# lucidrains/dreamer4

Hardware: AMD Instinct MI355X
Metric: imagined latent steps/sec (higher is better)
Workload: dtype f32; 1 GPU; cfg2 Moving-MNIST-latent shape: dim=512 depth=6 heads=8x64 latents=32x32 spatial=4 registers=8; generate(H+1=16 frames, num_steps=4, time cache) + learn_from_experience(ppo) + clip/AdamW both heads; global_batch=256, per_gpu_batch=256, horizon=15, num_steps=4, parallelism=dp1

## Files before the change

dreamer4_amd/_lib.py:

```python
from __future__ import annotations

import ctypes as C
import os

_HERE = os.path.dirname(os.path.abspath(__file__))
LIB_PATH = os.path.join(_HERE, 'libd4hip.so')

D4_MAX_ACTION_TYPES = 8

GEMM_RMS_ROWSCALE, GEMM_SILU, GEMM_SWIGLU, GEMM_TRANS_A, GEMM_TRANS_B, GEMM_ACCUMULATE = 1, 2, 4, 8, 16, 32


class Config(C.Structure):
    _fields_ = [
        ('dim', C.c_int32), ('dim_latent', C.c_int32), ('num_latent_tokens', C.c_int32), ('depth', C.c_int32),
        ('time_block_every', C.c_int32), ('attn_heads', C.c_int32), ('attn_dim_head', C.c_int32),
        ('attn_softclamp_value', C.c_float),
        ('num_spatial_tokens', C.c_int32), ('num_register_tokens', C.c_int32), ('max_steps', C.c_int32),
        ('num_tasks', C.c_int32), ('num_discrete_action_types', C.c_int32),
        ('num_discrete_actions', C.c_int32 * D4_MAX_ACTION_TYPES), ('num_continuous_actions', C.c_int32),
        ('multi_token_pred_len', C.c_int32),
        ('policy_head_mlp_depth', C.c_int32), ('value_head_mlp_depth', C.c_int32),
        ('terminal_mlp_depth', C.c_int32), ('predict_terminals', C.c_int32),
        ('reward_num_bins', C.c_int32), ('value_num_bins', C.c_int32), ('reward_encoder_type', C.c_int32), ('matmul_bf16', C.c_int32), ('head_mlp_recipe', C.c_int32), ('continuous_beta_param', C.c_int32),
# ... 100 lines not shown
    'd4_engine_destroy': (None, [_P]),
    'd4_engine_workspace_bytes': (C.c_size_t, [_P]),
    'd4_engine_set_workspace': (_I, [_P, _P, C.c_size_t]),
    'd4_engine_bind': (_I, [_P, C.c_char_p, _P, _P, _L]),
    'd4_engine_prepare': (_I, [_P, _P]),
    'd4_engine_cache_frames': (_I, [_P]),
    'd4_engine_cache_reset': (_I, [_P, _I]),
    'd4_engine_cache_export': (_I, [_P, _P, _I, _P]),
    'd4_engine_cache_import': (_I, [_P, _P, _I, _I, _P]),
    'd4_wm_forward': (_I, [_P, _P, _P, _I, _P, _P, _P, _I, _I, _I, _I, _P, _P, _P]),
    'd4_decoder_forward': (_I, [_P, _P, _P, _I, _I, _I, _P, _P]),
    'd4_ff_workspace_bytes': (C.c_size_t, [_I, _I, _I]),
    'd4_train_arith_set': (_I, [_I]),
    'd4_train_wide_set': (_I, [_I]),
    'd4_train_attn_products_set': (_I, [_I]),
    'd4_train_arith_get': (_I, []),
    'd4_train_scratch_bind': (_I, [_P, C.c_size_t]),
    'd4_ff_bf16_scratch_bytes': (C.c_size_t, [_I] * 3),
    'd4_attn_bf16_scratch_bytes': (C.c_size_t, [_I] * 4),
    'd4_cross_attn_bf16_scratch_bytes': (C.c_size_t, [_I] * 7),
    'd4_ff_forward': (_I, [_P] * 6 + [_I, _I, _I, _P, _P, C.c_size_t, _P]),
    'd4_ff_backward': (_I, [_P] * 6 + [_I, _I, _I] + [_P] * 6 + [_P, C.c_size_t, _P]),
    'd4_ff_backward_saved': (_I, [_P] * 6 + [_I, _I, _I] + [_P] * 6 + [_P, C.c_size_t, _P]),
    'd4_attn_workspace_bytes': (C.c_size_t, [_I] * 5),
    'd4_space_attn_forward': (_I, [_P] * 11 + [_I] * 5 + [_F, _I, _I, _P, _P, C.c_size_t, _P]),
    'd4_space_attn_backward': (_I, [_P] * 12 + [_I] * 5 + [_F, _I, _I] + [_P] * 11 + [_P, C.c_size_t, _P]),
    'd4_space_attn_backward_saved': (_I, [_P] * 12 + [_I] * 5 + [_F, _I, _I] + [_P] * 11 + [_P, C.c_size_t, _P]),
    'd4_time_attn_workspace_bytes': (C.c_size_t, [_I] * 6),
    'd4_time_attn_forward': (_I, [_P] * 12 + [_I] * 6 + [_F, _I, _P, _P, C.c_size_t, _P]),
    'd4_time_attn_backward': (_I, [_P] * 13 + [_I] * 6 + [_F, _I] + [_P] * 11 + [_P, C.c_size_t, _P]),
    'd4_time_attn_backward_saved': (_I, [_P] * 13 + [_I] * 6 + [_F, _I] + [_P] * 11 + [_P, C.c_size_t, _P]),
    'd4_cross_attn_workspace_bytes': (C.c_size_t, [_I] * 7),
    'd4_cross_attn_forward': (_I, [_P] * 10 + [_I] * 8 + [_F, _P, _P, C.c_size_t, _P]),
    'd4_cross_attn_backward': (_I, [_P] * 11 + [_I] * 8 + [_F] + [_P] * 10 + [_P, C.c_size_t, _P]),
    'd4_cross_attn_backward_saved': (_I, [_P] * 11 + [_I] * 8 + [_F] + [_P] * 10 + [_P, C.c_size_t, _P]),
    'd4_encoder_forward': (_I, [_P, _P, _I, _I, _P, _P]),
    'd4_euler_step': (_I, [_P, _P, _L, _F, _F, _P]),
    'd4_rollout': (_I, [_P, C.POINTER(RolloutIO), _P]),
    'd4_learn': (_I, [_P, C.POINTER(LearnIO), _P]),
    'd4_adamw_clip': (_I, [_P, _P, _P, _P, _L, _I, _F, _F, _F, _F, _F, _F, _F, _P, _P]),
    'd4_profile_bf16_enable': (_I, [_I]),
    'd4_profile_bf16_read': (_I, [C.POINTER(C.c_double), C.POINTER(C.c_double), C.POINTER(C.c_int64)]),
    'd4_profile_enable': (_I, [_I]),
    'd4_profile_read': (_I, [C.POINTER(C.c_double), C.POINTER(C.c_double), C.POINTER(C.c_int64), _I]),
    'd4_profile_classes': (_I, []),
    'd4_gemm_force_config': (_I, [_I]),
    'd4_debug_switch': (_I, [C.c_char_p, _I]),
    'd4_frame_fused_set': (_I, [_I]),
    'd4_profile_class_name': (C.c_char_p, [_I]),
    'd4_profile_glue_enable': (_I, [_I]),
    'd4_profile_glue_read': (_I, [C.POINTER(C.c_double), C.POINTER(C.c_double), C.POINTER(C.c_int64), _I]),
    'd4_profile_glue_classes': (_I, []),
    'd4_profile_glue_read_flops': (_I, [C.POINTER(C.c_double), _I]),
    'd4_measure_peaks': (_I, [_P, C.c_size_t, C.POINTER(C.c_double), C.POINTER(C.c_double), C.POINTER(C.c_double), _P]),
    'd4_profile_glue_class_name': (C.c_char_p, [_I]),
    'd4_debug_buffer': (_I, [_P, C.c_char_p, C.POINTER(_P)]),
    'd4_gemm': (_I, [_P, _I, _P, _I, _P, _I, _P, _P, _I, _I, _I, _I, _I, _F, _P]),
    'd4_gemm_tn': (_I, [_P, _I, _P, _I, _P, _I, _I, _I, _I, _P, C.c_int64, _I, _I, _P]),
    'd4_gemm_tn_bf16': (_I, [_P, _I, _P, _I, _P, _I, _I, _I, _I, _P, C.c_int64, _I, _P]),
    'd4_gemm_pair': (_I, [_P, _I, _P, _P, _I, _I, _I, _P, _I, _P, _P, _I, _I, _I, _I, _I, _F, _P]),
    'd4_gemm_batched': (_I, [_P, _I, _P, _I, _P, _I, _P, _P, _I, _I, _I, _I, _I, _F, _I, _L, _L, _L, _P]),
    'd4_gemm_bf16': (_I, [_P, _I, _P, _I, _P, _I, _P, _P, _I, _I, _I, _I, _I, _F, _P]),
    'd4_gemm_bf16a': (_I, [_P, _I, _P, _I, _P, _I, _P, _P, _P, _I, _I, _I, _I, _I, _F, _I, _P]),
    'd4_cvt_bf16': (_I, [_P, _P, _L, _P]),
    'd4_gemm_bf16a_compact': (_I, [_P, _I, _P, _I, _P, _I, _P, _P, _P, _I, _I, _I, _I, _I, _F, _P, _P, _I, _I, _I, _I, _I, _I, _P]),
    'd4_gemm_bf16a_batched': (_I, [_P, _I, _P, _I, _P, _I, _P, _P, _P, _I, _I, _I, _I, _I, _F, _I, _L, _L, _L, _I, _P]),
    'd4_cvt_rows_bf16': (_I, [_P, _L, _P, _L, _I, _I, _P]),
    'd4_split_bf16x3': (_I, [_P, _P, _L, _L, _P]),
    'd4_gemm_split': (_I, [_P, _I, _P, _L, _I, _P, _I, _P, _P, _I, _I, _I, _I, _I, _F, _I, _P]),
    'd4_split_f16x2': (_I, [_P, _P, _I, _I, _I, _L, _P, _P]),
    'd4_row_scale_exp': (_I, [_P, _L, _I, _I, _P, _P]),
    'd4_gemm_split2': (_I, [_P, _I, _P, _L, _I, _P, _P, _I, _P, _P, _I, _I, _I, _I, _I, _F, _I, _P, _P]),
    'd4_rmsnorm': (_I, [_P, _I, _P, _P, _I, _I, _I, _F, _P]),
    'd4_small_attn': (_I, [_P, _L, _L] * 4 + [_P] + [_P, _L, _L] * 3 + [_P] + [_I] * 4 + [_F] + [_I] * 6 + [_P]),
    'd4_small_attn_wide': (_I, [_P, _L, _L] * 4 + [_P] + [_P, _L, _L] * 3 + [_P] + [_I] * 4 + [_F] + [_I] * 6 + [_P]),
    'd4_small_attn_wide_bf16': (_I, [_P, _L, _L] * 4 + [_P] + [_P, _L, _L] * 3 + [_P] + [_I] * 4 + [_F] + [_I] * 6 + [_P]),
    'd4_pool_mix': (_I, [_P, _I, _P, _I, _P, _P, _I, _P, _I, _P, _P, _I, _I, _I, _F, _P, _P, _P, _P, _P]),
    'd4_pool_mix_deep': (_I, [_P, _I, _P, _I, _P, _P, _I, _P, _I, _P, _P, _I, _I, _I, _F, _P, _P, _P, _P, _P]),
    'd4_time_attn_decode': (_I, [_P, _I, _P, _I, _P, _P, _P, _P, _I, _P] + [_I] * 8 + [_P, _F, _I, _I, _P]),
    'd4_gemm_family_configs': (_I, [_I]),
    'd4_gemm_run': (_I, [C.POINTER(GemmDesc), _I, _I, _P]),
    'd4_gemm_run_rowmap': (_I, [C.POINTER(GemmDesc), _I, _I, _I, _I, _I, _I, _P]),
    'd4_gemm_run_pair': (_I, [C.POINTER(GemmDesc), C.POINTER(GemmDesc), _I, _I, _P]),
    'd4_tile16_weights': (_I, [_P, _I, _P, _I, _I, _P]),
    'd4_frame_attn_out': (_I, [_P, _L, _L] * 4 + [_P] + [_P, _L, _L] * 2 + [_P] + [_I] * 3 + [_F] + [_I] * 3 + [_P, _I, _P, _I, _P, _I, _P, _I, _I, _I, _I, _P]),
    'd4_attn_out_cols': (_I, [_P, _L, _L] * 4 + [_P] + [_P, _L, _L] * 2 + [_P] + [_I] * 3 + [_F] + [_I] * 3 + [_P, _I, _I, _P, _I, _P, _I, _P, _I, _I, _I, _I, _P]),
    'd4_frame_pool': (_I, [_P, _I, _P, _I, _P, _P, _I, _P, _I, _P, _I, _I, _I, _F, _P, _P, _I, _I, _P, _I, _P, _I, _P, _I, _I, _I, _I, _P]),
    'd4_frame_pool_tail': (_I, [_P, _P, _P, _I, _I, _I, _I, _P, _I, _P, _I, _P, _I, _I, _I, _I, _P]),
    'd4_lqap_in': (_I, [_P, _I, _P, _I, _P, _P, _P, _P] + [_I] * 5 + [_F, _P]),
    'd4_lqap_out': (_I, [_P, _I, _P, _P, _P, _P, _I, _P, _I] + [_I] * 5 + [_P]),
    'd4_debug_last_form': (C.c_char_p, [C.c_char_p]),
    'd4_debug_forms': (_I, [C.c_char_p, _I, C.POINTER(C.c_char_p)]),
    'd4_train_attn_core_plane_floats': (C.c_size_t, [_I] * 3),
    'd4_train_xattn_core_plane_floats': (C.c_size_t, [_I] * 4),
    'd4_train_attn_core': (_I, [_P, _I] + [_P] * 7 + [_I] * 4 + [_F, _I, _I, _I, _L, _L, _I, _P, _I, _P, C.c_size_t, _P]),
    'd4_train_xattn_core': (_I, [_P, _I, _P, _I] + [_P] * 6 + [_I] * 6 + [_F, _I, _P, C.c_size_t, _P]),
    'd4_train_attn_core_bf16_plane_floats': (C.c_size_t, [_I] * 4),
    'd4_train_xattn_core_bf16_plane_floats': (C.c_size_t, [_I] * 5),
    'd4_train_attn_core_bf16': (_I, [_P, _I] + [_P] * 7 + [_I] * 4 + [_F, _I, _I, _I, _L, _L, _I, _P, _I, _P, C.c_size_t, _P]),
    'd4_train_xattn_core_bf16': (_I, [_P, _I, _P, _I] + [_P] * 6 + [_I] * 6 + [_F, _I, _P, C.c_size_t, _P]),
    'd4_rmsnorm_backward': (_I, [_P, _P, _P, _P, _P, _P, _I, _I, _F, _P]),
    'd4_layernorm_rows': (_I, [_P, _I, _P, _P, _P, _I, _I, _I, _F, _I, _P]),
    'd4_assemble_tokens': (_I, [C.POINTER(AssembleDesc), _P]),
    'd4_gather_space_double_norm': (_I, [_P, _P, _P, _P, _I, _I, _I, _I, _I, _F, _P]),
    'd4_colsum': (_I, [_P, _I, _I, _I, _P, _P, C.c_size_t, _P]),
    'd4_colsum_batch': (_I, [_I, C.POINTER(_P), C.POINTER(C.c_int32), C.POINTER(C.c_int32), C.POINTER(C.c_int32), C.POINTER(_P), _P]),
    'd4_rmsnorm_bwd': (_I, [_P, _P, _P, _P, _P, _I, _I, _F, _P]),
    'd4_euler_step_rows': (_I, [_P, _I, _P, _I, _I, _I, _F, _F, _P]),
    'd4_splitk_reduce': (_I, [_P, _I, _I, _I, _P, _I, _P, _I, _P]),
    'd4_mean_tokens': (_I, [_P, _P, _I, _I, _I, _P]),
    'd4_hl_gauss_scalar_strided': (_I, [_P, _I, _P, _P, _I, _I, _I, _P]),
    'd4_unary_rows': (_I, [_I, _P, _P, _L, _P]),
    'd4_fold_rows': (_I, [_P, _P, _P, _I, _I, _I, _P]),
    'd4_swiglu_pack_rows': (_I, [_P, _P, _P, _P, _P, _I, _I, _I, _P]),
    'd4_build_latent_input': (_I, [_P, _P, _P, _P, _I, _I, _I, _I, _F, _P]),
    'd4_copy_rows': (_I, [_P, _I, _P, _I, _I, _I, _P]),
    'd4_pad_cols': (_I, [_P, _P, _I, _I, _I, _P]),
    'd4_video_patches': (_I, [_P, _P, _I, _I, _I, _I, _I, _I, _I, _P]),
    'd4_cache_transfer': (_I, [_P, _P] + [_I] * 9 + [_P]),
    'd4_cunembed': (_I, [_I, _P, _P, _I, _I, _I, _P]),
    'd4_coord_grid': (_I, [_P, _I, _I, _I, _P]),
    'd4_pack_tokens': (_I, [_I, _P, _P, _P, _P, _P, _I, _I, _I, _I, _I, _P]),
    'd4_prep_eval_inputs': (_I, [_P, _P, _P] + [_I] * 7 + [_P, _P, _I, _P]),
    'd4_layernorm_silu_bwd': (_I, [_P, _I, _P, _P, _P, _P, _P, _P, _I, _I, _F, _P]),
    'd4_silu_bwd': (_I, [_P, _P, _P, _L, _P]),
    'd4_swiglu': (_I, [_I, _P, _P, _P, _I, _I, _I, _P]),
    'd4_multi_copy': (_I, [_I, C.POINTER(_P), C.POINTER(_P), C.POINTER(C.c_int64), _P]),
    'd4_zero_pad_cols': (_I, [_P, _I, _I, _I, _I, _P]),
    'd4_cvt_pad_bf16': (_I, [_P, _L, _P, _L, _I, _I, _I, _P]),
    'd4_cvt_transpose_bf16': (_I, [_P, _I, _P, _I, _I, _I, _I, _P]),
    'd4_hl_gauss_scalar': (_I, [_P, _I, _P, _P, _I, _I, _P]),
    'd4_ppo_policy_loss': (_I, [_P, _I, _P, _P, _P, _P, _P, _I, _I, _I, _I, _F, _F, _P, _P, _P, _P]),
    'd4_gae': (_I, [_P, _P, _P, _P, _P, _F, _F, _I, _I, _P, _P]),
    'd4_gae_adv': (_I, [_P, _P, _P, _P, _P, _F, _F, _I, _I, _P, _P, _P, _P]),
    'd4_policy_loss': (_I, [C.POINTER(PolicyLossDesc), _P]),
    'd4_return_stats': (_I, [_P, _P, _P, _L, _P, C.c_double, _F, _F, _P, _P, _P]),
    'd4_value_loss': (_I, [C.POINTER(ValueLossDesc), _P]),
    'd4_categorical_sample_logp': (_I, [_P, _I, _P, _I, _P, _I, _I, _F, _P, _P, _P]),
    'd4_hl_gauss_ce': (_I, [_P, _I, _P, _P, _P, _I, _I, _F, _F, _F, _F, _I, _P, _P, _P, _P]),
    'd4_flow_noised_patches': (_I, [_P] * 4 + [_I] * 6 + [_P]),
    'd4_tok_rows_part_floats': (C.c_size_t, [_I, _I]),
    'd4_layernorm_rows_bwd': (_I, [_P, _I, _P, _P, _P, _P, _P, C.c_size_t, _I, _I, _F, _P]),
    'd4_mask_rows_fwd': (_I, [_P] * 4 + [_I, _I, _P]),
    'd4_mask_rows_bwd': (_I, [_P] * 5 + [C.c_size_t, _I, _I, _P]),
    'd4_recon_loss_fwd_bwd': (_I, [_P] * 4 + [_I] * 7 + [_P, _P, _P, C.c_size_t, _P]),
}

_lib = None


class D4Error(RuntimeError):
    pass


def load():
    global _lib
    if _lib is not None:
        return _lib
    if not os.path.isfile(LIB_PATH):
        raise D4Error(f'{LIB_PATH} is missing: run `python -m dreamer4_amd.build` (hipcc, gfx950). '
                      'There is no CPU fallback for the imagination path.')
    default_table = os.path.join(_HERE, 'gemm_tune_default.txt')
    if os.path.isfile(default_table):
        os.environ.setdefault('D4_GEMM_TUNE_DEFAULT', default_table)
    lib = C.CDLL(LIB_PATH)
    for name, (res, args) in SYMBOLS.items():
# ... 19 lines not shown
```

dreamer4_amd/csrc/engine.hip:

```cpp
#include "common.h"
#include "engine.h"
#include "prof.h"
#include <math.h>
#include <stdarg.h>
#include <stdio.h>
#include <stdlib.h>
#include <string.h>
#include <memory>

using namespace d4;

namespace d4 {

static constexpr float RMS_EPS = 1.1920928955078125e-07f;

static int round_up(int v, int m) { return (v + m - 1) / m * m; }

int engine_layout(d4_engine* e, bool assign) {
    const d4_config& c = e->c;
    size_t off = 0;
    auto alloc_bytes = [&](size_t bytes) -> char* {
        off = (off + 255) / 256 * 256;
        char* p = assign ? e->ws + off : nullptr;
        off += bytes;
// ... 666 lines not shown
            if ((rc = mir(e->layer_attn[l].to_out, (size_t)D, hd))) return rc;
        }
        for (int l = 0; l <= c.depth; ++l) {
            if ((rc = mir(e->ffp[l].w1, (size_t)2 * e->inner_pad, D))) return rc;
            if ((rc = mir(e->ffp[l].w2, (size_t)D, e->inner_pad))) return rc;
        }
        for (int p = 0; p < c.depth; ++p) {
            if ((rc = mir(e->pq_w[p], (size_t)(hp + e->php), D))) return rc;
            if ((rc = mir(e->pkv_w[p], (size_t)2 * hp, D))) return rc;
            if ((rc = mir(e->pools[p].to_out, (size_t)D, hp))) return rc;
        }
        for (int l = 0; l < (int)e->pkq_w.size(); ++l)
            if ((rc = mir(e->pkq_w[l], (size_t)(c.depth - l) * hp, D))) return rc;
        if ((rc = mir(e->cq_w, (size_t)(hd + h), D))) return rc;
        if ((rc = mir(e->ckv_w, (size_t)2 * hd, D))) return rc;
        if ((rc = mir(e->cross.to_out, (size_t)D, hd))) return rc;
        if (ns == n) {
            if ((rc = mir(e->lin_w, (size_t)D, dl))) return rc;
            if ((rc = mir(e->lout_w, (size_t)dl, D))) return rc;
        } else {
            if ((rc = mir(e->lin_kv_w, (size_t)2 * hd, dl))) return rc;
            if ((rc = mir(e->lq_in.to_out, (size_t)D, hd))) return rc;
            if ((rc = mir(e->lout_kv_w, (size_t)2 * hd, D))) return rc;
            if ((rc = mir(e->lout_w, (size_t)dl, hd))) return rc;
        }
    }

    e->l0_ready = e->ck_ready = false;
    if (e->c0_proj || e->ck) {
        const int nr = c.num_register_tokens, lo = 1 + ns, pin = 4096;
        t_bf16 = e->bf16 ? e : nullptr;
        auto planes = [e](GemmArgs g) {
            if (e->bf16)
                for (const auto& m : e->mirrors)
                    if (g.W >= m.src && g.W < m.src + m.n) { g.Wb = m.dst + (g.W - m.src); break; }
            if (g.Wb && e->split) { g.wplane = (int64_t)e->bf16_cap; if (!gemm_x3_applicable(g)) { g.Wb = nullptr; g.wplane = 0; } }
            return g;
        };
        rc = 0;
        if (e->c0_proj) {
            GemmArgs g{e->registers, D, e->proj_w[0], D, e->c0_proj, e->Nproj0, e->proj_b[0], nullptr, 0, nr, e->Nproj0, D, GEMM_RMS_ROWSCALE, RMS_EPS};
            g.rule_M = pin;
            if (gemm_rule_takes_x3sk(planes(g))) {
                rc = engine_gemm(g, s);
                for (int ly = 0; ly < 2 && !rc; ++ly) {
                    const int Sl = e->S - 1 + ly;
                    rc = copy_rows(e->c0_proj, 0, e->proj0r[ly] + (size_t)lo * e->Nproj0, Sl * e->Nproj0, e->Fr, nr * e->Nproj0, s);
                }
                e->l0_ready = !rc;
            }
        }
        if (!rc && e->ck && e->pkv_stride > 0) {
            bool ok = true;
            for (int p = 0; p < c.depth - 1; ++p) {
                GemmArgs g{e->registers, D, e->pkv_w[p], D, e->ck + (size_t)p * nr * hp, hp, nullptr, nullptr, 0, nr, hp, D, GEMM_RMS_ROWSCALE, RMS_EPS};
                g.rule_M = pin;
                ok = ok && gemm_rule_takes_v2(planes(g));
            }
            for (int p = 0; ok && p < c.depth - 1 && !rc; ++p) {
                GemmArgs g{e->registers, D, e->pkv_w[p], D, e->ck + (size_t)p * nr * hp, hp, nullptr, nullptr, 0, nr, hp, D, GEMM_RMS_ROWSCALE, RMS_EPS};
                g.rule_M = pin;
                rc = engine_gemm(g, s);
                for (int ly = 0; ly < 2 && !rc; ++ly) {
                    const int Sl = e->S - 1 + ly;
                    rc = copy_rows(e->ck + (size_t)p * nr * hp, 0, e->kvr[ly] + (size_t)p * e->kvr_stride[ly] + (size_t)lo * hp, Sl * hp, e->Fr, nr * hp, s);
                }
            }
            e->ck_ready = ok && !rc;
        }
        t_bf16 = nullptr;
        if (rc) return rc;
    }

    int32_t offs[D4_MAX_ACTION_TYPES] = {0}, sizes[D4_MAX_ACTION_TYPES] = {0};
    int o = 0;
    for (int a = 0; a < e->na; ++a) { offs[a] = o; sizes[a] = c.num_discrete_actions[a]; o += sizes[a]; }
    D4_HIP(hipMemcpyAsync(e->action_offsets, offs, sizeof(offs), hipMemcpyHostToDevice, s));
    D4_HIP(hipMemcpyAsync(e->action_sizes, sizes, sizeof(sizes), hipMemcpyHostToDevice, s));
    D4_HIP(hipStreamSynchronize(s));
    e->prepared = true;
    return 0;
}

static int ff_block(d4_engine* e, const FfPrep& fp, const float* out_b, const float* x, int ldx, float* y, int ldy,
                    int rows, hipStream_t s, float* y_compact = nullptr, int S = 0, int has_agent = 1) {
    int rc;
    GemmArgs g1{x, ldx, fp.w1, e->D, e->ffh, e->inner_pad, fp.b1, nullptr, 0, rows, 2 * e->inner_pad, e->D,
                GEMM_RMS_ROWSCALE | GEMM_SWIGLU, RMS_EPS, 2.0 * rows * (2.0 * e->inner) * e->D};
    if ((rc = engine_gemm(g1, s))) return rc;
    GemmArgs g2{e->ffh, e->inner_pad, fp.w2, e->inner_pad, y, ldy, out_b, x, ldx, rows, e->D, e->inner_pad, 0, RMS_EPS,
                2.0 * rows * (double)e->D * e->inner};
    if (y_compact) { g2.C2 = y_compact; g2.ldc2 = e->D; g2.c2_S = S; g2.c2_lo = t_keep_lo; g2.c2_hi = t_keep_hi; g2.c2_last = has_agent; }
    return engine_gemm(g2, s);
}

int g_pool_wide_keys = 1;
int g_rollout_clean_agent_row = 1;
int g_rollout_batched_heads = 1;
int g_lqap_in_fused = 1;
int g_lqap_out_fused = 1;
int g_last_layer_compact_q = 1;
int g_layer0_const_rows = 1;
int g_pool_const_keys = 1;
unsigned g_launch_count = 0;
static int pool_block(d4_engine* e, int p, const float* x, float* y, int L, int M, hipStream_t s, const float* hiddens = nullptr,
                      float* y_compact = nullptr, int S = 0, int has_agent = 1, int rule_M = 0, float* keys0 = nullptr) {
    if (!hiddens) hiddens = e->slabs;
    const d4_config& c = e->c;
    const int D = e->D, hp = e->hp;
    const AttnW& a = e->pools[p];
    int rc;
    const bool mix_path = c.pool_heads == 4 && D <= 1024;
    GemmArgs gq{x, D, e->pq_w[p], D, e->pool_q, e->ldpq, nullptr, nullptr, 0, M, mix_path ? hp : hp + e->php, D, GEMM_RMS_ROWSCALE, RMS_EPS};
    gq.rule_M = rule_M;
    if (mix_path) {
        const bool wide = g_pool_wide_keys && t_bf16 && e->kall_b && hiddens == e->slabs && p < c.depth - 1 && L == 2 * p + 3 && x == e->slabs + (size_t)(L - 1) * M * D;
        PoolMixArgs pm{};
        pm.q = e->pool_q; pm.ldq = e->ldpq; pm.k = e->pool_kv; pm.ldk = hp;
        if (wide) {
            const int j0 = p == 0 ? 0 : 2 * p + 1, ld = e->kall_ld;
            GemmArgs gw{hiddens + (size_t)j0 * M * D, D, e->pkq_w[p], D, nullptr, ld, nullptr, nullptr, 0, (L - j0) * M, (c.depth - p) * hp, D, GEMM_RMS_ROWSCALE, RMS_EPS};
            gw.algo_flops = 2.0 * M * hp * (double)D * ((double)(L - j0) * (c.depth - 1 - p) + 1.0);
            gw.Cb = e->kall_b + (size_t)j0 * M * ld + (size_t)p * hp;
            if ((rc = engine_gemm(gw, s))) return rc;
            pm.k = nullptr; pm.k_b = e->kall_b + (size_t)p * hp; pm.ldk = ld;
            pm.q = nullptr; pm.q_b = e->kall_b + (size_t)(L - 1) * M * ld + (size_t)(c.depth - 1) * hp; pm.ldq = ld;
        } else {
        GemmArgs gk{hiddens, D, e->pkv_w[p], D, e->pool_kv, hp, nullptr, nullptr, 0, L * M, hp, D, GEMM_RMS_ROWSCALE, RMS_EPS};
        gk.rule_M = L * rule_M;
        if (keys0) {
            gk.A = hiddens + (size_t)M * D; gk.C = keys0 + (size_t)M * hp; gk.M = (L - 1) * M; gk.rule_M = L * M;
            pm.k = keys0;
        }
        if ((rc = gemm_two(gq, gk, s))) return rc;
        if (t_bf16) pm.k_b = t_bf16->shadow_of(e->pool_kv);
        }
        pm.x = x; pm.ldx = D; pm.gate_w = e->pq_w[p] + (size_t)hp * D; pm.hid = hiddens; pm.D = D; pm.k_gamma = a.k_gamma;
        pm.u = e->pool_u; pm.M = M; pm.L = L; pm.heads = c.pool_heads; pm.eps = RMS_EPS; pm.rule_M = rule_M;
        if (t_bf16 && D > 512) pm.hid_b = t_bf16->shadow_of(hiddens);
        if (t_bf16) if (uint16_t* ub = t_bf16->shadow_of(e->pool_u)) { pm.u_b = ub; if (t_bf16->shadow_only(e->pool_u)) pm.u = nullptr; }
        const bool deep = L > 64 || g_pool_mix_deep;
        if (S > 0 && M % S == 0 && !e->pv_t.empty() && (!t_bf16 || t_bf16->fp32_planes()) && frame_pool_tail_applicable(M / S, S, D, c.pool_heads)) {
            const bool tail_only = deep || frame_fused_mode() == 2;
            if (!tail_only) return frame_pool(pm, e->pv_t[p], e->po_t[p], M / S, S, x, D, y, D, y_compact, D, t_keep_lo, t_keep_hi, has_agent, s);
            if ((rc = deep ? pool_mix_deep(pm, s) : pool_mix(pm, s))) return rc;
            return frame_pool_tail(e->pool_u, e->pv_t[p], e->po_t[p], M / S, S, D, c.pool_heads, x, D, y, D, y_compact, D, t_keep_lo, t_keep_hi, has_agent, s);
        }
        if ((rc = deep ? pool_mix_deep(pm, s) : pool_mix(pm, s))) return rc;
        GemmArgs gv{e->pool_u, c.pool_heads * D, e->pkv_w[p] + (size_t)hp * D, D, e->pool_att, hp, nullptr, nullptr, 0, M, 64, D, 0, RMS_EPS};
        gv.batch = c.pool_heads; gv.strideA = D; gv.strideW = (int64_t)64 * D; gv.strideC = 64; gv.rule_M = rule_M;
        if ((rc = engine_gemm(gv, s))) return rc;
    } else {
    const GemmArgs gkv{hiddens, D, e->pkv_w[p], D, e->pool_kv, 2 * hp, nullptr, nullptr, 0, L * M, 2 * hp, D, GEMM_RMS_ROWSCALE, RMS_EPS};
    if ((rc = gemm_two(gq, gkv, s))) return rc;
    SmallAttnArgs sa{};
    sa.q = e->pool_q; sa.q_group_stride = e->ldpq; sa.q_item_stride = 0;
    sa.k = e->pool_kv; sa.k_group_stride = 2 * hp; sa.k_item_stride = (int64_t)M * 2 * hp;
    sa.v = e->pool_kv + hp; sa.v_group_stride = 2 * hp; sa.v_item_stride = (int64_t)M * 2 * hp;
    sa.gate = e->pool_q + hp; sa.g_group_stride = e->ldpq; sa.g_item_stride = 0;
    sa.k_gamma = a.k_gamma;
    sa.out = e->pool_att; sa.o_group_stride = hp; sa.o_item_stride = 0;
    sa.groups = M; sa.heads = c.pool_heads; sa.nq = 1; sa.nk = L;
    sa.wide = (c.wide_frames & 2) ? 2 : (c.wide_frames & 1);
    sa.out_b = t_bf16 ? t_bf16->shadow_of(e->pool_att) : nullptr;
    if ((rc = small_attn(sa, s))) return rc;
    }
    if (y_compact) return gemm_c2(e->pool_att, hp, a.to_out, hp, y, D, M, D, hp, 0, nullptr, x, D, y_compact, S, t_keep_hi - t_keep_lo, has_agent, s);
    GemmArgs go{e->pool_att, hp, a.to_out, hp, y, D, nullptr, x, D, M, D, hp, 0, RMS_EPS};
    go.rule_M = rule_M;
    return engine_gemm(go, s);
}

void engine_drop_graphs(d4_engine* e) {
    for (auto& g : e->graphs) (void)hipGraphExecDestroy(g.exec);
    e->graphs.clear();
}

static int engine_forward_impl(d4_engine* e, const float* latents, int B, int Tq, int t0, int step_log2,
                               const int64_t* tasks, bool need_agent, hipStream_t s, const int* t0_dev, bool need_pred, bool agent_only);

bool engine_clean_agent_only(const d4_engine* e) {
    return !e->encoder && !e->decoder && (!e->bf16 || e->split) && e->c.pool_heads == 4 && e->D <= 1024;
}

int engine_forward(d4_engine* e, const float* latents, int B, int Tq, int t0, int step_log2,
                   const int64_t* tasks, bool need_agent, hipStream_t s, const int* t0_dev, bool need_pred) {
    t_bf16 = e->bf16 ? e : nullptr;
    need_pred = need_pred || !need_agent || e->encoder || e->decoder;
    const bool agent_only = !need_pred && engine_clean_agent_only(e);
    t_keep_lo = e->keep_lo;
    t_keep_hi = agent_only ? e->keep_lo : e->keep_hi;
    const int rc = engine_forward_impl(e, latents, B, Tq, t0, step_log2, tasks, need_agent, s, t0_dev, need_pred, agent_only);
    t_bf16 = nullptr;
    return rc;
}

static int engine_forward_impl(d4_engine* e, const float* latents, int B, int Tq, int t0, int step_log2,
                               const int64_t* tasks, bool need_agent, hipStream_t s, const int* t0_dev, bool need_pred, bool agent_only) {
    const d4_config& c = e->c;
    D4_REQUIRE(e->prepared, "engine not prepared");
    D4_REQUIRE(B >= 1 && B <= e->maxB, "batch %d exceeds max_batch %d", B, e->maxB);
    D4_REQUIRE(Tq >= 1 && Tq <= e->maxTq, "parallel frames %d exceed max_parallel_frames %d", Tq, e->maxTq);
    D4_REQUIRE(t0 + Tq <= e->Tcap || e->Lt == 0, "KV cache capacity %d exceeded (%d + %d frames)", e->Tcap, t0, Tq);
    const int has_agent = (need_agent && !e->encoder) ? 1 : 0;
    const int D = e->D, hd = e->hd, h = c.attn_heads, S = (need_agent || e->encoder) ? e->S : e->S - 1;
    const int n = c.num_latent_tokens, dl = c.dim_latent, ns = c.num_spatial_tokens;
    const int Fr = B * Tq, M = Fr * S;
    const bool denoise_only = !need_agent && !e->encoder && !e->decoder;
    const bool fp32_engine = !e->bf16 || e->split;
    auto tiled_family = [e](int M_, int N_, int K_, int flags, const float* W, int rule_M = 0) {
        GemmArgs g{};
        g.M = M_; g.N = N_; g.K = K_; g.lda = K_; g.ldw = K_; g.ldc = N_; g.flags = flags; g.rms_eps = RMS_EPS; g.rule_M = rule_M; g.W = W;
        if (e->bf16) {
            for (const auto& m : e->mirrors)
                if (W >= m.src && W < m.src + m.n) { g.Wb = m.dst + (W - m.src); break; }
            if (g.Wb && e->split) { g.wplane = (int64_t)e->bf16_cap; if (!gemm_x3_applicable(g)) { g.Wb = nullptr; g.wplane = 0; } }
// ... 93 lines not shown
        if ((rc = engine_gemm(gb, s))) return rc;
    }
    }
    if (t_bf16) if (uint16_t* sb = t_bf16->shadow_of(slab0)) { if ((rc = cvt_rows_bf16(slab0, D, sb, D, M, D, s))) return rc; }

    const float* x_in = slab0;
    const float* vres = P0 + 3 * hd + 2 * h;
    for (int l = 0; l < c.depth; ++l) {
        const AttnW& a = e->layer_attn[l];
        float* P = l == 0 ? P0 : e->proj;
        const int ldp = l == 0 ? e->Nproj0 : e->Nproj;
        const bool compact_q = g_last_layer_compact_q && fp32_engine && e->proj_wc && denoise_only && l == c.depth - 1 && !e->is_time[l] && c.depth >= 2 && S <= 16 && S >= 8 &&
                               c.attn_dim_head == 64 && !g_small_attn_wide && tiled_family(M, ldp, D, GEMM_RMS_ROWSCALE, e->proj_w[l]) &&
                               tiled_family(M, 2 * hd + h, D, GEMM_RMS_ROWSCALE, e->proj_wc) && tiled_family(Mc, hd + h, D, GEMM_RMS_ROWSCALE, e->proj_wc, M);
        if (compact_q) {
            GemmArgs ga{x_in, D, e->proj_wc, D, P, ldp, e->proj_bc, nullptr, 0, M, 2 * hd + h, D, GEMM_RMS_ROWSCALE, RMS_EPS};
            GemmArgs gb{e->xpool_c, D, e->proj_wc + (size_t)(2 * hd + h) * D, D, e->qc, e->ldqc, e->proj_bc + 2 * hd + h, nullptr, 0, Mc, hd + h, D, GEMM_RMS_ROWSCALE, RMS_EPS};
            gb.rule_M = M;
            if ((rc = gemm_two(ga, gb, s))) return rc;
        } else if (l == 0 && l0_const) {
            GemmArgs g0{e->slab0r, D, e->proj_w[0], D, P, ldp, e->proj_b[0], nullptr, 0, Fr * Sc, ldp, D, GEMM_RMS_ROWSCALE, RMS_EPS};
            g0.rule_M = M;
            g0.rm_Sc = (uint16_t)Sc; g0.rm_lo = (uint16_t)reg_lo; g0.rm_nr = (uint16_t)nr;
            if ((rc = engine_gemm(g0, s))) return rc;
        } else
        if ((rc = gemm_simple(x_in, D, e->proj_w[l], D, P, ldp, M, ldp, D, GEMM_RMS_ROWSCALE, e->proj_b[l], nullptr, 0, s))) return rc;
        bool fused_out = false;
        if (e->is_time[l]) {
            TimeAttnArgs ta{};
            ta.proj = P; ta.ldp = ldp; ta.vres = vres; ta.ldv = e->Nproj0; ta.k_gamma = a.k_gamma; ta.inv_freq = e->inv_freq;
            ta.cache = e->cache + (size_t)e->time_index[l] * 2 * e->maxB * e->S * h * e->Tcap * c.attn_dim_head;
            ta.dh = c.attn_dim_head;
            ta.out = e->att; ta.ldo = hd; ta.B = B; ta.S = S; ta.H = h; ta.Tq = Tq; ta.t0 = t0; ta.Tcap = e->Tcap;
            ta.softclamp = c.attn_softclamp_value;
            ta.cache_batch = e->maxB; ta.cache_S = e->S;
            ta.t0_dev = t0_dev;
            ta.out_b = t_bf16 ? t_bf16->shadow_of(e->att) : nullptr;
            if ((rc = time_attn_append(ta, s))) return rc;
        } else {
            SmallAttnArgs sa{};
            sa.dh = c.attn_dim_head;
            const int64_t gs = (int64_t)S * ldp;
            sa.q = P; sa.q_group_stride = gs; sa.q_item_stride = ldp;
            sa.k = P + hd; sa.k_group_stride = gs; sa.k_item_stride = ldp;
            sa.v = P + 2 * hd; sa.v_group_stride = gs; sa.v_item_stride = ldp;
            sa.gate = P + 3 * hd; sa.g_group_stride = gs; sa.g_item_stride = ldp;
            sa.mix = P + 3 * hd + h; sa.m_group_stride = gs; sa.m_item_stride = ldp;
            sa.vres = vres; sa.r_group_stride = (int64_t)S * e->Nproj0; sa.r_item_stride = e->Nproj0;
            sa.k_gamma = a.k_gamma;
            sa.out = e->att; sa.o_group_stride = (int64_t)S * hd; sa.o_item_stride = hd;
            sa.groups = Fr; sa.heads = h; sa.nq = S; sa.nk = S;
            sa.wide = (c.wide_frames & 2) ? 2 : (c.wide_frames & 1);
            sa.softclamp = c.attn_softclamp_value; sa.mask_special = e->encoder ? n : has_agent; sa.belief = 1;
            sa.out_b = t_bf16 ? t_bf16->shadow_of(e->att) : nullptr;
            if (denoise_only && l == c.depth - 1 && c.depth >= 2 && S <= 16 && S >= 8) {
                sa.q_lo = 1; sa.q_hi = 1 + ns; sa.q_last = 0;
                sa.out = e->att_c; sa.o_group_stride = (int64_t)nkeep * hd; sa.out_b = nullptr;
                if (compact_q) {
                    sa.k = P; sa.v = P + hd; sa.mix = P + 2 * hd;
                    sa.q = e->qc; sa.q_group_stride = (int64_t)nkeep * e->ldqc; sa.q_item_stride = e->ldqc;
                    sa.gate = e->qc + hd; sa.g_group_stride = (int64_t)nkeep * e->ldqc; sa.g_item_stride = e->ldqc;
                    sa.q_compact = 1;
                }
            }
            const bool tail_compact = denoise_only && l == c.depth - 1 && c.depth >= 2 && S <= 16 && S >= 8;
            if (!tail_compact && !e->wo_t.empty() && (!t_bf16 || t_bf16->fp32_planes()) && frame_attn_out_applicable(sa, D)) {
                if ((rc = frame_attn_out(sa, e->wo_t[l], D, x_in, D, slab(2 * l + 1), D, cslab(2 * l + 1), D, t_keep_lo, t_keep_hi, has_agent, s))) return rc;
                fused_out = true;
            } else if (!tail_compact && hd == 512 && (!t_bf16 || t_bf16->fp32_planes()) && attn_out_cols_applicable(sa, D)) {
                if ((rc = attn_out_cols(sa, a.to_out, hd, D, x_in, D, slab(2 * l + 1), D, cslab(2 * l + 1), D, t_keep_lo, t_keep_hi, has_agent, s))) return rc;
                fused_out = true;
            } else
            if ((rc = small_attn(sa, s))) return rc;
        }
        const bool compact_tail = denoise_only && l == c.depth - 1 && !e->is_time[l] && c.depth >= 2 && S <= 16 && S >= 8;
        if (compact_tail) {
            if ((rc = gemm_simple(e->att_c, hd, a.to_out, hd, cslab(2 * l + 1), D, Mc, D, hd, 0, nullptr, e->xpool_c, D, s))) return rc;
            if ((rc = ff_block(e, e->ffp[l], e->layer_ff[l].out_b, cslab(2 * l + 1), D, cslab(2 * l + 2), D, Mc, s))) return rc;
            break;
        }
        float* h1 = slab(2 * l + 1);
        float* h2 = slab(2 * l + 2);
        if (!fused_out && (rc = gemm_c2(e->att, hd, a.to_out, hd, h1, D, M, D, hd, 0, nullptr, x_in, D, cslab(2 * l + 1), S, t_keep_hi - t_keep_lo, has_agent, s))) return rc;
        if ((rc = ff_block(e, e->ffp[l], e->layer_ff[l].out_b, h1, D, h2, D, M, s, cslab(2 * l + 2), S, has_agent))) return rc;
        if (l != c.depth - 1) {
            float* xc = (denoise_only && l == c.depth - 2 && !e->is_time[c.depth - 1] && S <= 16 && S >= 8) ? e->xpool_c : nullptr;
            if ((rc = pool_block(e, l, h2, e->xpool, 2 * l + 3, M, s, nullptr, xc, S, has_agent, 0, keys0(l)))) return rc;
            x_in = e->xpool;
        }
    }

    float* xfc = e->xfc;
    const float* last = slab(2 * c.depth);
    if ((rc = copy_rows(cslab(2 * c.depth), D, xfc, D, Mc, D, s))) return rc;
    if (e->encoder) {
        const int P = e->P;
        const float* spec = cslab(2 * c.depth);
        if ((rc = gemm_simple(spec, D, e->cq_w, D, e->cq, e->ldcq, Mc, hd + h, D, GEMM_RMS_ROWSCALE, nullptr, nullptr, 0, s))) return rc;
        if ((rc = gemm_simple(last, D, e->ckv_w, D, e->ckv, 2 * hd, M, 2 * hd, D, GEMM_RMS_ROWSCALE, nullptr, nullptr, 0, s))) return rc;
        SmallAttnArgs sa{};
        sa.dh = c.attn_dim_head;
        sa.q = e->cq; sa.q_group_stride = (int64_t)n * e->ldcq; sa.q_item_stride = e->ldcq;
        sa.k = e->ckv; sa.k_group_stride = (int64_t)S * 2 * hd; sa.k_item_stride = 2 * hd;
        sa.v = e->ckv + hd; sa.v_group_stride = (int64_t)S * 2 * hd; sa.v_item_stride = 2 * hd;
        sa.gate = e->cq + hd; sa.g_group_stride = (int64_t)n * e->ldcq; sa.g_item_stride = e->ldcq;
        sa.k_gamma = e->cross.k_gamma;
        sa.out = e->catt; sa.o_group_stride = (int64_t)n * hd; sa.o_item_stride = hd;
        sa.groups = Fr; sa.heads = h; sa.nq = n; sa.nk = P;
        sa.wide = (c.wide_frames & 2) ? 2 : (c.wide_frames & 1);
        if ((rc = small_attn(sa, s))) return rc;
        if ((rc = gemm_simple(e->catt, hd, e->cross.to_out, hd, xfc, D, Mc, D, hd, 0, nullptr, spec, D, s))) return rc;
        if ((rc = ff_block(e, e->ffp[c.depth], e->sff.out_b, xfc, D, xfc, D, Mc, s))) return rc;
        if ((rc = pool_block(e, c.depth - 1, xfc, xfc, e->nslab, Mc, s, e->cslabs))) return rc;
        if ((rc = gemm_simple(xfc, D, e->t2p_wf, D, e->enc_out, c.dim_latent, Mc, c.dim_latent, D, GEMM_RMS_ROWSCALE, nullptr, nullptr, 0, s))) return rc;
        return tanh_rows(e->enc_out, e->enc_out, (int64_t)Mc * c.dim_latent, s);
    }
    if (e->decoder) {
        if ((rc = pool_block(e, c.depth - 1, xfc, xfc, e->nslab, Mc, s, e->cslabs))) return rc;
        return gemm_simple(xfc, D, e->t2p_wf, D, e->dec_out, e->dim_patch, Mc, e->dim_patch, D, GEMM_RMS_ROWSCALE, e->t2p_b, nullptr, 0, s);
    }
    if (need_agent) {
        const float* agent_in = last + (size_t)(S - 1) * D;
        float* agent_rows = xfc + (size_t)ck * D;
        const int lda = S * D, ldc = nkeep * D;
        {
            const GemmArgs gq{agent_in, lda, e->cq_w, D, e->cq, e->ldcq, nullptr, nullptr, 0, Fr, hd + h, D, GEMM_RMS_ROWSCALE, RMS_EPS};
            const GemmArgs gkv{last, D, e->ckv_w, D, e->ckv, 2 * hd, nullptr, nullptr, 0, M, 2 * hd, D, GEMM_RMS_ROWSCALE, RMS_EPS};
            if ((rc = gemm_two(gq, gkv, s))) return rc;
        }
        SmallAttnArgs sa{};
        sa.dh = c.attn_dim_head;
        sa.q = e->cq; sa.q_group_stride = e->ldcq; sa.q_item_stride = 0;
        sa.k = e->ckv; sa.k_group_stride = (int64_t)S * 2 * hd; sa.k_item_stride = 2 * hd;
        sa.v = e->ckv + hd; sa.v_group_stride = (int64_t)S * 2 * hd; sa.v_item_stride = 2 * hd;
        sa.gate = e->cq + hd; sa.g_group_stride = e->ldcq; sa.g_item_stride = 0;
        sa.k_gamma = e->cross.k_gamma;
        sa.out = e->catt; sa.o_group_stride = hd; sa.o_item_stride = 0;
        sa.groups = Fr; sa.heads = h; sa.nq = 1; sa.nk = S - 1;
        sa.wide = (c.wide_frames & 2) ? 2 : (c.wide_frames & 1);
        if ((rc = small_attn(sa, s))) return rc;
        if ((rc = gemm_simple(e->catt, hd, e->cross.to_out, hd, agent_rows, ldc, Fr, D, hd, 0, nullptr, agent_in, lda, s))) return rc;
        if ((rc = ff_block(e, e->ffp[c.depth], e->sff.out_b, agent_rows, ldc, agent_rows, ldc, Fr, s))) return rc;
    }
    if ((rc = pool_block(e, c.depth - 1, xfc, xfc, e->nslab, Mc, s, e->cslabs, nullptr, 0, 1, agent_only ? Fr * (ns + 1) : 0))) return rc;
    if (!need_pred) return 0;

    if (same_len) {
        if ((rc = copy_rows(xfc, nkeep * D, e->gs, ns * D, Fr, ns * D, s))) return rc;
        return gemm_simple(e->gs, D, e->lout_w, D, e->pred, dl, Fr * n, dl, D, GEMM_RMS_ROWSCALE, nullptr, nullptr, 0, s);
    }
    if ((rc = gather_space_double_norm(xfc, e->gs, e->latent_norm, e->lq_out.norm_ctx, Fr, nkeep, 0, D, ns, RMS_EPS, s))) return rc;
    if ((rc = gemm_simple(e->gs, D, e->lout_kv_w, D, e->okv, 2 * hd, Fr * ns, 2 * hd, D, 0, nullptr, nullptr, 0, s))) return rc;
    if (g_lqap_out_fused && fp32_engine && !g_small_attn_wide && lqap_out_applicable(h, c.attn_dim_head, n, ns, dl) && dl % 4 == 0 && frame_fused_frames_ok(Fr) &&
        tiled_family(Fr * n, dl, hd, 0, e->lout_w))
        return lqap_out(e->okv, 2 * hd, e->lout_q, e->lout_gate, e->lq_out.k_gamma, e->lout_w, hd, e->pred, dl, Fr, h, n, ns, dl, s);
    {
        SmallAttnArgs sa{};
        sa.dh = c.attn_dim_head;
        sa.q = e->lout_q; sa.q_group_stride = 0; sa.q_item_stride = hd;
        sa.k = e->okv; sa.k_group_stride = (int64_t)ns * 2 * hd; sa.k_item_stride = 2 * hd;
        sa.v = e->okv + hd; sa.v_group_stride = (int64_t)ns * 2 * hd; sa.v_item_stride = 2 * hd;
        sa.gate = e->lout_gate; sa.g_group_stride = 0; sa.g_item_stride = h;
        sa.k_gamma = e->lq_out.k_gamma;
        sa.out = e->oatt; sa.o_group_stride = (int64_t)n * hd; sa.o_item_stride = hd;
        sa.groups = Fr; sa.heads = h; sa.nq = n; sa.nk = ns;
        sa.wide = (c.wide_frames & 2) ? 2 : (c.wide_frames & 1);
        if ((rc = small_attn(sa, s))) return rc;
    }
    if ((rc = gemm_simple(e->oatt, hd, e->lout_w, hd, e->pred, dl, Fr * n, dl, hd, 0, nullptr, nullptr, 0, s))) return rc;
    return 0;
// ... 268 lines not shown
    int sl, rc;
    if ((rc = step_log2_of(step_size, &sl))) return rc;
    if ((rc = check_step_log2(e, sl))) return rc;
    D4_REQUIRE(batch <= e->maxB && frames <= e->maxTq, "batch/frames exceed engine capacity");
    const int Fr = batch * frames;
    D4_HIP(hipMemcpyAsync(e->sig, signal_levels, sizeof(int32_t) * Fr, hipMemcpyDeviceToDevice, s));
    if (e->na > 0) {
        if (prev_actions) D4_HIP(hipMemcpyAsync(e->pact, prev_actions, sizeof(int64_t) * Fr * e->na, hipMemcpyDeviceToDevice, s));
        else D4_HIP(hipMemsetAsync(e->pact, 0xFF, sizeof(int64_t) * Fr * e->na, s));
    }
    if (e->nc > 0) {
        if (prev_cont) D4_HIP(hipMemcpyAsync(e->pcont, prev_cont, sizeof(float) * Fr * e->nc, hipMemcpyDeviceToDevice, s));
        else if (e->na > 0) D4_HIP(hipMemsetAsync(e->pcont, 0, sizeof(float) * Fr * e->nc, s));
        else D4_HIP(hipMemsetAsync(e->pcont, 0xFF, sizeof(float) * Fr * e->nc, s));
    }
    const int t0 = use_cache ? e->cache_frames : 0;
    if ((rc = d4::engine_forward(e, latents, batch, frames, t0, sl, tasks, true, s))) return rc;
    if (commit_cache) e->cache_frames = t0 + frames;
    const int n_el = e->c.num_latent_tokens * e->c.dim_latent;
    if (pred && (rc = d4::copy_rows(e->pred, n_el, pred, n_el, Fr, n_el, s))) return rc;
    const int nkeep = e->c.num_spatial_tokens + 1;
    if (agent_embed && (rc = d4::copy_rows(e->xfc + (size_t)(nkeep - 1) * e->D, nkeep * e->D, agent_embed, e->D, Fr, e->D, s))) return rc;
    return 0;
}

int d4_decoder_forward(d4_engine* e, const float* latents, const float* noised_video, int time_index, int batch, int frames,
                       float* pred_video, void* stream) {
    D4_REQUIRE(e && latents && noised_video && pred_video, "null argument");
    D4_REQUIRE(e->decoder, "d4_decoder_forward needs an engine created with mode = D4_MODE_DECODER");
    D4_REQUIRE(batch >= 1 && batch <= e->maxB && frames >= 1 && frames <= e->maxTq, "batch / frames exceed the decoder engine's capacity (%d x %d)", e->maxB, e->maxTq);
    D4_REQUIRE(time_index >= 0 && time_index < e->c.decoder_flow_steps, "flow step %d outside [0, %d)", time_index, e->c.decoder_flow_steps);
    hipStream_t s = static_cast<hipStream_t>(stream);
    const d4_config& c = e->c;
    int rc;
    if ((rc = d4::video_to_patches(noised_video, e->dec_in, batch, c.channels, frames, e->nph, e->npw, c.patch_size, s))) return rc;
    if ((rc = d4::engine_forward(e, latents, batch, frames, 0, time_index, nullptr, false, s))) return rc;
    return d4::patches_to_video(e->dec_out, pred_video, batch, c.channels, frames, e->nph, e->npw, c.patch_size, s);
}

int d4_encoder_forward(d4_engine* e, const float* video, int batch, int frames, float* latents, void* stream) {
    D4_REQUIRE(e && video && latents, "null argument");
    D4_REQUIRE(e->encoder, "d4_encoder_forward needs an engine created with mode = D4_MODE_ENCODER");
    D4_REQUIRE(batch >= 1 && batch <= e->maxB && frames >= 1 && frames <= e->maxTq, "batch / frames exceed the encoder engine's capacity (%d x %d)", e->maxB, e->maxTq);
    hipStream_t s = static_cast<hipStream_t>(stream);
    const d4_config& c = e->c;
    int rc;
    if ((rc = d4::video_to_patches(video, e->dec_in, batch, c.channels, frames, e->nph, e->npw, c.patch_size, s))) return rc;
    if ((rc = d4::engine_forward(e, nullptr, batch, frames, 0, 0, nullptr, false, s))) return rc;
    const int nl = c.num_latent_tokens * c.dim_latent;
    return d4::copy_rows(e->enc_out, nl, latents, nl, batch * frames, nl, s);
}

int d4_euler_step(float* x, const float* pred, int64_t n, float one_minus_t, float dt, void* stream) {
    D4_REQUIRE(x && pred && n >= 0 && n < (int64_t)1 << 31, "euler_step: bad arguments");
    return d4::euler_step(x, (int)n, pred, (int)n, 1, (int)n, one_minus_t, dt, static_cast<hipStream_t>(stream));
}

int d4_rollout(d4_engine* e, const d4_rollout_io* io, void* stream) {
    D4_REQUIRE(e && io, "null argument");
    D4_REQUIRE(!e->decoder && !e->encoder, "d4_rollout needs a dynamics engine");
    hipStream_t s = static_cast<hipStream_t>(stream);
    const d4_config& c = e->c;
    const int B = io->batch, T = io->time_steps, P = io->prompt_frames, K = io->num_steps;
    D4_REQUIRE(B >= 1 && B <= e->maxB, "batch %d exceeds max_batch %d", B, e->maxB);
    D4_REQUIRE(K >= 1 && (K & (K - 1)) == 0 && K <= c.max_steps, "number of steps %d must be a power of 2 in (0, %d]  [D4:6357-6358]", K, c.max_steps);
    D4_REQUIRE(P >= 0 && P <= T, "bad prompt_frames");
    D4_REQUIRE(!io->sample_actions || e->na > 0 || e->nc > 0, "the model has no actions to sample  [D4:6626]");
    D4_REQUIRE(!io->sample_actions || e->na == 0 || (io->actions && io->gumbel_u && io->log_probs && io->action_logits), "sample_actions needs the action outputs and gumbel_u");
    D4_REQUIRE(!io->sample_actions || e->nc == 0 || (io->actions_cont && io->beta_noise && io->log_probs_cont && io->cont_params), "sample_actions needs the continuous action outputs and beta_noise");
    D4_REQUIRE(!io->sample_actions || io->values, "sample_actions needs the values output");
    D4_REQUIRE(!io->sample_terminals || (c.predict_terminals && io->bern_u), "sample_terminals needs predict_terminals and bern_u");
    D4_REQUIRE(io->use_time_cache || io->noise_context || T - P <= 1, "noise_context is required without the time cache");
    const int F = T - P;
    const int step_size = c.max_steps / K;
    int sl, rc;
    if ((rc = step_log2_of(step_size, &sl))) return rc;
    if ((rc = check_step_log2(e, sl))) return rc;
    const int n_el = c.num_latent_tokens * c.dim_latent;
    const int D = e->D, S = e->S, A = e->A, na = e->na, nc = e->nc;
    if (!io->use_time_cache) e->cache_frames = 0;
    const bool lean = d4::g_rollout_clean_agent_row != 0;
    const int lean_keep = (lean && d4::engine_clean_agent_only(e)) ? 1 : c.num_spatial_tokens + 1;
    const int variant = (lean ? 1 : 0) | (d4::g_lqap_in_fused ? 2 : 0) | (d4::g_lqap_out_fused ? 4 : 0) | (d4::g_last_layer_compact_q ? 8 : 0) |
                        (d4::g_layer0_const_rows ? 16 : 0) | (d4::g_pool_const_keys ? 32 : 0);
    const float* hist = nullptr;
    if (d4::g_rollout_batched_heads && F >= 1 && F <= e->head_rows) {
        if (io->agent_embed) hist = io->agent_embed;
        else if (F == 1) hist = e->agent_c;
        else if ((size_t)B * F <= e->hist_rows) hist = e->agent_hist;
    }
    const bool heads_after = hist != nullptr;

    for (int f = 0; f < F; ++f) {
        const int cur = P + f;
        int Tq, t0;
        bool commit;
        if (io->use_time_cache && (e->cache_frames > 0 || cur == 0)) { Tq = 1; t0 = e->cache_frames; commit = true; }
        else if (io->use_time_cache) { Tq = cur + 1; t0 = 0; commit = true; }
        else { Tq = cur + 1; t0 = 0; commit = false; }
        D4_REQUIRE(Tq <= e->maxTq, "a parallel pass over %d frames exceeds max_parallel_frames %d", Tq, e->maxTq);
        if ((rc = d4::copy_rows(io->noise_latent + (size_t)f * B * n_el, n_el, e->x_lat, n_el, B, n_el, s))) return rc;

        const bool graphable = Tq == 1 && B * S <= e->graph_max_rows && !d4::gemm_profile_active() && e->graph_max_rows > 0;
        if (graphable) {
            D4_REQUIRE(t0 + 1 <= e->Tcap || e->Lt == 0, "KV cache capacity %d exceeded (%d + 1 frames)", e->Tcap, t0);
            if ((rc = d4::set_frame_state(e->fstate, t0, s))) return rc;
            if ((rc = d4::prep_eval_inputs(e->sig, e->pact, io->actions, B, 1, na, cur, T, 0, c.max_steps - 1, s, nc > 0 ? e->pcont : nullptr, io->actions_cont, nc))) return rc;
            const int64_t* tasks = nullptr;
            if (io->tasks) {
                D4_HIP(hipMemcpyAsync(e->tasks_dev, io->tasks, sizeof(int64_t) * B, hipMemcpyDeviceToDevice, s));
                tasks = e->tasks_dev;
            }
            hipGraphExec_t exec = nullptr;
            const int bucket = e->Lt > 0 ? d4::time_history_bucket(t0) : 0;
            for (auto& g : e->graphs) if (g.B == B && g.K == K && g.sl == sl && g.tasks == (tasks != nullptr) && g.bucket == bucket && g.variant == variant) exec = g.exec;
            if (!exec) {
                if (!e->warm) {
                    e->warm = true;
                } else {
                    if (!e->capture_stream) D4_HIP(hipStreamCreateWithFlags(&e->capture_stream, hipStreamNonBlocking));
                    hipStream_t cs = e->capture_stream;
                    hipGraph_t graph;
                    D4_HIP(hipStreamBeginCapture(cs, hipStreamCaptureModeThreadLocal));
                    int crc = 0;
                    for (int step = 0; step <= K && !crc; ++step) {
                        const int sig_val = step * step_size < c.max_steps - 1 ? step * step_size : c.max_steps - 1;
                        d4::t_sig_uniform = sig_val;
                        crc = d4::engine_forward(e, e->x_lat, B, 1, t0, sl, tasks, step == K, cs, e->fstate, !(step == K && lean));
                        d4::t_sig_uniform = -1;
                        if (crc) break;
                        if (step == K) break;
                        const float tt = (float)sig_val / (float)c.max_steps;
                        crc = d4::euler_step(e->x_lat, n_el, e->pred, n_el, B, n_el, 1.f - tt, (float)step_size / (float)c.max_steps, cs);
                    }
                    hipError_t ce = hipStreamEndCapture(cs, &graph);
                    if (crc) { if (ce == hipSuccess) (void)hipGraphDestroy(graph); return crc; }
                    D4_HIP(ce);
                    D4_HIP(hipGraphInstantiate(&exec, graph, nullptr, nullptr, 0));
                    (void)hipGraphDestroy(graph);
                    e->graphs.push_back({B, K, sl, tasks != nullptr, bucket, variant, exec});
                }
            }
            if (exec) {
                D4_HIP(hipGraphLaunch(exec, s));
            } else {
                for (int step = 0; step <= K; ++step) {
                    const int sig_val = step * step_size < c.max_steps - 1 ? step * step_size : c.max_steps - 1;
                    d4::t_sig_uniform = sig_val;
                    rc = d4::engine_forward(e, e->x_lat, B, 1, t0, sl, tasks, step == K, s, e->fstate, !(step == K && lean));
                    d4::t_sig_uniform = -1;
                    if (rc) return rc;
                    if (step == K) break;
                    const float tt = (float)sig_val / (float)c.max_steps;
                    if ((rc = d4::euler_step(e->x_lat, n_el, e->pred, n_el, B, n_el, 1.f - tt, (float)step_size / (float)c.max_steps, s))) return rc;
                }
            }
            if (commit) e->cache_frames = t0 + 1;
        } else
        for (int step = 0; step <= K; ++step) {
            const bool last = step == K;
            const int sig_val = step * step_size < c.max_steps - 1 ? step * step_size : c.max_steps - 1;
            const float* lat = e->x_lat;
            if (Tq > 1) {
                if ((rc = d4::build_latent_input(e->lat_in, io->latents, io->ctx_hist, e->x_lat, B, Tq, n_el, T, io->context_signal_noise, s))) return rc;
                lat = e->lat_in;
            }
            if ((rc = d4::prep_eval_inputs(e->sig, e->pact, io->actions, B, Tq, na, cur + 1 - Tq, T, sig_val, c.max_steps - 1, s, nc > 0 ? e->pcont : nullptr, io->actions_cont, nc))) return rc;
// ... 4 lines not shown
                                     1.f - tt, (float)step_size / (float)c.max_steps, s))) return rc;
        }

        const int nkeep = lean_keep;
        const float* agent_row = e->xfc + ((size_t)(Tq - 1) * nkeep + (nkeep - 1)) * D;
        if ((rc = d4::copy_rows(agent_row, Tq * nkeep * D, e->agent_c, D, B, D, s))) return rc;
        if (io->agent_embed && (rc = d4::copy_rows(e->agent_c, D, io->agent_embed + (size_t)f * D, F * D, B, D, s))) return rc;
        if (hist == e->agent_hist && (rc = d4::copy_rows(e->agent_c, D, e->agent_hist + (size_t)f * D, F * D, B, D, s))) return rc;
        if (!heads_after) {
        if ((rc = d4::rmsnorm_rows(e->agent_c, D, e->reward_norm, e->hnorm, D, B, D, d4::RMS_EPS, s))) return rc;
        if ((rc = d4::gemm_simple(e->hnorm, D, e->reward_w, D, e->rlogits, c.reward_num_bins, B, c.reward_num_bins, D, 0, nullptr, nullptr, 0, s))) return rc;
        if ((rc = d4::hl_gauss_scalar(e->rlogits, c.reward_num_bins, e->reward_centers, io->rewards + cur, T, B, c.reward_num_bins, s))) return rc;
        }
        const float* term_logit = nullptr;
        if (io->sample_terminals) {
            if ((rc = d4::mean_tokens(e->x_lat, e->term_pool, B, c.num_latent_tokens, c.dim_latent, s))) return rc;
            if ((rc = d4::mlp_forward(e, e->terminal, e->term_pool, c.dim_latent, B, e->term_logit, 1, nullptr, s))) return rc;
            term_logit = e->term_logit;
        }
        if (io->sample_actions) {
            float* pe = e->hbuf[(e->policy.nl - 1) & 1];
            if ((rc = d4::mlp_forward(e, e->policy, e->agent_c, D, B, pe, 4 * D, nullptr, s))) return rc;
            float* logits = na > 0 ? io->action_logits + (size_t)f * A : nullptr;
            if (na > 0 && (rc = d4::gemm_simple(pe, 4 * D, e->action_unembed, c.multi_token_pred_len * 4 * D, logits, F * A, B, A, 4 * D, 0, nullptr, nullptr, 0, s))) return rc;
            float* cparams = nc > 0 ? io->cont_params + (size_t)f * nc * 2 : nullptr;
            if (nc > 0) {
                if ((rc = d4::cunembed_gather(e->cont_unembed, e->cu_w, nc, c.multi_token_pred_len, 4 * D, s))) return rc;
                if ((rc = d4::gemm_simple(pe, 4 * D, e->cu_w, 4 * D, cparams, F * nc * 2, B, 2 * nc, 4 * D, 0, nullptr, nullptr, 0, s))) return rc;
            }
            if (!heads_after) {
            float* vb = e->hbuf[(e->value.nl - 1) & 1];
            if ((rc = d4::mlp_forward(e, e->value, e->agent_c, D, B, vb, c.value_num_bins, nullptr, s))) return rc;
            if ((rc = d4::hl_gauss_scalar(vb, c.value_num_bins, e->value_centers, io->values + f, F, B, c.value_num_bins, s))) return rc;
            }
            d4::SampleArgs sa{};
            sa.logits = logits; sa.ld = F * A;
            sa.gumbel_u = na > 0 ? io->gumbel_u + (size_t)f * B * A : nullptr; sa.ld_u = A;
            sa.term_logit = term_logit; sa.bern_u = io->sample_terminals ? io->bern_u + (size_t)f * B : nullptr;
            sa.actions = na > 0 ? io->actions + (size_t)cur * na : nullptr; sa.act_stride = T * na;
            sa.log_probs = na > 0 ? io->log_probs + (size_t)f * na : nullptr; sa.lp_stride = F * na;
            sa.terminals = io->terminals; sa.lens = io->lens; sa.action_sizes = e->action_sizes;
            sa.B = B; sa.na = na; sa.frame_index = cur; sa.temperature = io->discrete_temperature;
            if (nc > 0) {
                sa.nc = nc; sa.cont_params = cparams; sa.ld_c = F * nc * 2;
                sa.beta_noise = io->beta_noise + (size_t)f * B * nc * 4 * 6;
                sa.actions_cont = io->actions_cont + (size_t)cur * nc; sa.actc_stride = T * nc;
                sa.log_probs_cont = io->log_probs_cont + (size_t)f * nc; sa.lpc_stride = F * nc;
                sa.cont_temperature = io->continuous_temperature; sa.beta_param = e->c.continuous_beta_param;
            }
            if ((rc = d4::sample_actions_terminals(sa, s))) return rc;
        } else if (term_logit) {
            d4::SampleArgs sa{};
            sa.term_logit = term_logit; sa.bern_u = io->bern_u + (size_t)f * B;
            sa.terminals = io->terminals; sa.lens = io->lens; sa.B = B; sa.na = 0; sa.frame_index = cur;
            if ((rc = d4::sample_actions_terminals(sa, s))) return rc;
        }
        if ((rc = d4::copy_rows(e->x_lat, n_el, io->latents + (size_t)cur * n_el, T * n_el, B, n_el, s))) return rc;
        if (io->ctx_hist && io->noise_context &&
            (rc = d4::copy_rows(io->noise_context + (size_t)f * B * n_el, n_el, io->ctx_hist + (size_t)cur * n_el, T * n_el, B, n_el, s))) return rc;
    }
    if (heads_after && (rc = d4::rollout_heads_batched(e, io, hist, B, F, P, T, s))) return rc;
    return 0;
}

int d4_profile_bf16_enable(int stride) { d4::gemm_bf16_profile_enable(stride); return 0; }
int d4_profile_bf16_read(double* ms, double* flops, int64_t* count) { return d4::gemm_bf16_profile_read(ms, flops, count); }
int d4_profile_enable(int on) { return d4::gemm_profile_enable(on); }
int d4_profile_read(double* ms, double* flops, int64_t* count, int nclass) { return d4::gemm_profile_read(ms, flops, count, nclass); }
int d4_profile_classes(void) { return d4::gemm_profile_classes(); }
int d4_profile_glue_enable(int mask) { return d4::glue_profile_enable(mask); }
int d4_profile_glue_read(double* ms, double* bytes, int64_t* count, int nclass) { return d4::glue_profile_read(ms, bytes, count, nclass); }
int d4_profile_glue_classes(void) { return d4::GL_N; }
int d4_profile_glue_read_flops(double* flops, int nclass) { return d4::glue_profile_read_flops(flops, nclass); }
const char* d4_profile_glue_class_name(int c) { return d4::glue_class_name(c); }
int d4_frame_fused_set(int mode) { return d4::frame_fused_set(mode); }

int d4_debug_switch(const char* name, int value) {
    int* sw = nullptr;
    if (name && !strcmp(name, "launch_count")) {
        const int old = (int)(d4::g_launch_count & 0x7fffffffu);
        d4::g_launch_count = (unsigned)value;
        return old;
    }
    if (name && !strcmp(name, "time_attn_fused_append")) sw = &d4::g_time_attn_fused_append;
    else if (name && !strcmp(name, "rollout_clean_agent_row")) sw = &d4::g_rollout_clean_agent_row;
    else if (name && !strcmp(name, "rollout_batched_heads")) sw = &d4::g_rollout_batched_heads;
    else if (name && !strcmp(name, "attn_out_cols")) sw = &d4::g_attn_out_cols;
    else if (name && !strcmp(name, "lqap_in_fused")) sw = &d4::g_lqap_in_fused;
    else if (name && !strcmp(name, "lqap_out_fused")) sw = &d4::g_lqap_out_fused;
    else if (name && !strcmp(name, "last_layer_compact_q")) sw = &d4::g_last_layer_compact_q;
    else if (name && !strcmp(name, "layer0_const_rows")) sw = &d4::g_layer0_const_rows;
    else if (name && !strcmp(name, "pool_const_keys")) sw = &d4::g_pool_const_keys;
    else if (name && !strcmp(name, "pool_wide_keys")) sw = &d4::g_pool_wide_keys;
    else if (name && !strcmp(name, "pool_mix_deep")) sw = &d4::g_pool_mix_deep;
    else if (name && !strcmp(name, "time_attn_tiled")) sw = &d4::g_time_attn_tiled;
    else if (name && !strcmp(name, "space_attn_tiled")) sw = &d4::g_space_attn_tiled;
    else if (name && !strcmp(name, "cross_attn_tiled")) sw = &d4::g_cross_attn_tiled;
    else if (name && !strcmp(name, "small_attn_wide")) sw = &d4::g_small_attn_wide;
    if (!sw) return -1;
    const int old = *sw;
    *sw = value;
    return old;
}
int d4_gemm_force_config(int id) {
    d4::gemm_bf16a_force_config(-1);
    d4::gemm_bf16_force_config(-1);
    const int n_main = d4::gemm_force_config(-1);
    if (id < 0) return n_main;
    if (id >= 500) { d4::gemm_bf16a_force_config(id - 500); return d4::gemm_bf16a_configs(); }
    if (id >= 400) { d4::gemm_force_config(id); return d4::gemm_h2_configs(); }
    if (id >= 300) { d4::gemm_force_config(id); return d4::gemm_x3_configs(); }
    if (id >= 200) return d4::gemm_bf16_force_config(id - 200);
    d4::gemm_force_config(id);
    return id >= 100 ? d4::gemm2_configs() : n_main;
}
const char* d4_profile_class_name(int c) { return d4::gemm_profile_class_name(c); }

int d4_debug_buffer(d4_engine* e, const char* name, float** ptr) {
    D4_REQUIRE(e && name && ptr, "null argument");
    struct { const char* n; float* p; } tbl[] = {
        {"slabs", e->slabs}, {"xpool", e->xpool}, {"xfc", e->xfc}, {"cslabs", e->cslabs}, {"proj0", e->proj0}, {"proj", e->proj}, {"att", e->att},
        {"ffh", e->ffh}, {"pool_q", e->pool_q}, {"pool_kv", e->pool_kv}, {"pool_att", e->pool_att}, {"cq", e->cq},
        {"ckv", e->ckv}, {"catt", e->catt}, {"lkv", e->lkv}, {"latt", e->latt}, {"space", e->space}, {"gs", e->gs},
        {"okv", e->okv}, {"oatt", e->oatt}, {"oproj", e->oproj}, {"pred", e->pred}, {"x_lat", e->x_lat},
        {"cache", e->cache}, {"lin_q", e->lin_q}, {"lin_gate", e->lin_gate}, {"lout_q", e->lout_q},
        {"qc", e->qc}, {"l_logits", e->l_logits}, {"l_dlogits", e->l_dlogits}, {"l_adv", e->l_adv}, {"l_returns", e->l_returns}, {"l_mask", e->l_mask},
    };
    for (auto& t : tbl) if (!strcmp(t.n, name)) {
        D4_REQUIRE(!e->shadow_only(t.p), "debug buffer '%s' exists only as a bf16 image in this engine (matmul_bf16 = 1)", name);
        *ptr = t.p; return 0;
    }
    D4_REQUIRE(false, "unknown debug buffer '%s'", name);
}

int d4_learn(d4_engine* e, const d4_learn_io* io, void* stream) {
    D4_REQUIRE(e && io, "null argument");
    return d4::learn(e, io, static_cast<hipStream_t>(stream));
}

int d4_gemm(const float* A, int lda, const float* W, int ldw, float* C, int ldc, const float* bias,
            const float* R, int ldr, int M, int N, int K, int flags, float rms_eps, void* stream) {
    d4::GemmArgs g{A, lda, W, ldw, C, ldc, bias, R, ldr, M, N, K, flags, rms_eps};
    return d4::gemm(g, static_cast<hipStream_t>(stream));
}

int d4_gemm_pair(const float* A1, int lda1, const float* W1, float* C1, int ldc1, int M1, int N1, const float* A2, int lda2, const float* W2, float* C2,
                 int ldc2, int M2, int N2, int K, int flags, float rms_eps, void* stream) {
    d4::GemmArgs a{A1, lda1, W1, K, C1, ldc1, nullptr, nullptr, 0, M1, N1, K, flags, rms_eps};
    d4::GemmArgs b{A2, lda2, W2, K, C2, ldc2, nullptr, nullptr, 0, M2, N2, K, flags, rms_eps};
    return d4::gemm_pair(a, b, static_cast<hipStream_t>(stream));
}

int d4_gemm_tn(const float* A, int lda, const float* B, int ldb, float* C, int ldc, int M, int N, int K, float* part, int64_t part_floats,
               int tile_n, int slices, void* stream) {
    return d4::gemm_tn(A, lda, B, ldb, C, ldc, M, N, K, part, (size_t)part_floats, static_cast<hipStream_t>(stream), tile_n, slices);
}

int d4_gemm_batched(const float* A, int lda, const float* W, int ldw, float* C, int ldc, const float* bias,
                    const float* R, int ldr, int M, int N, int K, int flags, float rms_eps, int batch,
                    int64_t strideA, int64_t strideW, int64_t strideC, void* stream) {
    d4::GemmArgs g{A, lda, W, ldw, C, ldc, bias, R, ldr, M, N, K, flags, rms_eps};
    g.batch = batch; g.strideA = strideA; g.strideW = strideW; g.strideC = strideC;
    return d4::gemm(g, static_cast<hipStream_t>(stream));
}

int d4_split_bf16x3(const float* src, uint16_t* dst, int64_t n, int64_t plane_stride, void* stream) {
    D4_REQUIRE(src && dst && n >= 0 && plane_stride >= n && (plane_stride % 8) == 0, "d4_split_bf16x3: bad arguments");
    return d4::split_bf16x3(src, dst, n, plane_stride, static_cast<hipStream_t>(stream));
}
int d4_gemm_split(const float* A, int lda, const uint16_t* W3, int64_t plane_stride, int ldw, float* C, int ldc, const float* bias,
                  const float* R, int ldr, int M, int N, int K, int flags, float rms_eps, int config, void* stream) {
    d4::GemmArgs g{A, lda, reinterpret_cast<const float*>(W3), ldw, C, ldc, bias, R, ldr, M, N, K, flags, rms_eps};
    g.Wb = W3; g.wplane = plane_stride;
    D4_REQUIRE(d4::gemm_x3_applicable(g), "d4_gemm_split: call not supported (M=%d N=%d K=%d flags=%d: K %% 32, ldw %% 8, plane_stride %% 8, 16-byte alignment)", M, N, K, flags);
    if (M == 0) return 0;
// ... 262 lines not shown
static d4::GemmArgs gemm_args_of(const d4_gemm_desc& d) {
    d4::GemmArgs g{d.A, d.lda, d.W, d.ldw, d.C, d.ldc, d.bias, d.R, d.ldr, d.M, d.N, d.K, d.flags, d.rms_eps};
    g.C2 = d.C2; g.ldc2 = d.ldc2; g.c2_S = d.c2_S; g.c2_lo = d.c2_lo; g.c2_hi = d.c2_hi; g.c2_last = d.c2_last;
    g.batch = d.batch > 0 ? d.batch : 1; g.strideA = d.strideA; g.strideW = d.strideW; g.strideC = d.strideC;
    g.Ab = d.Ab; g.Wb = d.Wb; g.Cb = d.Cb; g.C2b = d.C2b; g.wplane = d.wplane; g.wscale = d.wscale; g.strideWs = d.strideWs; g.aexp = d.aexp;
    return g;
}
static int gemm_desc_check(const char* who, const d4_gemm_desc* d) {
    D4_REQUIRE(d && d->M >= 1 && d->N >= 1 && d->K >= 1 && (d->C || d->Cb), "%s: null descriptor, no output or bad sizes", who);
    D4_REQUIRE(!(d->C2 || d->C2b) || (d->C2 && d->c2_S >= 1 && d->c2_lo >= 0 && d->c2_hi >= d->c2_lo && d->c2_hi <= d->c2_S && d->ldc2 >= d->N &&
                                      (d->c2_last == 0 || d->c2_last == 1) && !(d->flags & d4::GEMM_SWIGLU)),
               "%s: bad compaction arguments", who);
    return 0;
}
int d4_gemm_family_configs(int family) {
    switch (family) {
        case D4_GEMM_TILE: return d4::gemm_configs();
        case D4_GEMM_V2: return d4::gemm2_configs();
        case D4_GEMM_X3: return d4::gemm_x3_configs();
        case D4_GEMM_H2: return d4::gemm_h2_configs();
        case D4_GEMM_BF16: return d4::gemm_bf16_configs();
        case D4_GEMM_BF16A: return d4::gemm_bf16a_configs();
        case D4_GEMM_V2_KSPLIT: case D4_GEMM_X3SK: case D4_GEMM_SKINNY: return 1;
    }
    return -1;
}
static int gemm_run_args(const d4::GemmArgs& g, int family, int config, void* stream);
int d4_gemm_run(const d4_gemm_desc* d, int family, int config, void* stream) {
    if (int rc = gemm_desc_check("d4_gemm_run", d)) return rc;
    return gemm_run_args(gemm_args_of(*d), family, config, stream);
}
int d4_gemm_run_rowmap(const d4_gemm_desc* d, int family, int config, int rm_Sc, int rm_S, int rm_lo, int rm_nr, void* stream) {
    if (int rc = gemm_desc_check("d4_gemm_run_rowmap", d)) return rc;
    D4_REQUIRE(rm_Sc >= 1 && rm_nr >= 0 && rm_lo >= 0 && rm_lo <= rm_Sc && rm_S == rm_Sc + rm_nr && rm_S <= 65535, "d4_gemm_run_rowmap: bad row map (Sc=%d S=%d lo=%d nr=%d)", rm_Sc, rm_S, rm_lo, rm_nr);
    d4::GemmArgs g = gemm_args_of(*d);
    g.rm_Sc = (uint16_t)rm_Sc; g.rm_lo = (uint16_t)rm_lo; g.rm_nr = (uint16_t)rm_nr;
    return gemm_run_args(g, family, config, stream);
}
static int gemm_run_args(const d4::GemmArgs& g, int family, int config, void* stream) {
    hipStream_t s = static_cast<hipStream_t>(stream);
    const bool al16 = ((uintptr_t)g.A % 16) == 0 && ((uintptr_t)g.W % 16) == 0 && (g.lda % 4) == 0 && (g.ldw % 4) == 0;
#define D4_RUN_REFUSE(cond, why) D4_REQUIRE(cond, "d4_gemm_run: call not supported (family %d, configuration %d, M=%d N=%d K=%d flags=%d: " why ")", family, config, g.M, g.N, g.K, g.flags)
    switch (family) {
        case D4_GEMM_TILE: {
            D4_RUN_REFUSE(d4::gemm_config_valid(config, g), "the dispatcher does not run this configuration of the first family here - few-row shape, mirror weights or an epilogue the tile lacks");
            d4_gemm_force_config(config);
            const int rc = d4::gemm(g, s);
            d4_gemm_force_config(-1);
            return rc;
        }
        case D4_GEMM_V2:
            D4_RUN_REFUSE(al16 && !g.Wb && d4::gemm2_config_valid(config, g), "gemm2_config_valid: K %% 32, lda / ldw %% 4, no transposed operand, SiLU-GLU tiles");
            return d4::gemm2_launch(config, g, s);
        case D4_GEMM_V2_KSPLIT:
            D4_RUN_REFUSE(al16 && d4::gemm2_ksplit_applicable(g), "gemm2_ksplit_applicable: no batch, C2, row scale, bias-free flags other than SiLU; K >= 4 k-tiles");
            return d4::gemm2_ksplit_launch(g, s);
        case D4_GEMM_X3:
            D4_RUN_REFUSE(al16 && !g.wscale && d4::gemm_x3_config_valid(config, g), "gemm_x3_config_valid: three bf16 planes, K %% 32, ldw / plane %% 8, SiLU-GLU tiles");
            return d4::gemm_x3_launch(config, g, s);
        case D4_GEMM_X3SK:
            D4_RUN_REFUSE(al16 && !g.wscale && d4::gemm_x3sk_applicable(g), "gemm_x3sk_applicable: as gemm_x3, no batch");
            return d4::gemm_x3sk_launch(g, s);
        case D4_GEMM_H2:
            D4_RUN_REFUSE(al16 && d4::gemm_h2_config_valid(config, g), "gemm_h2_config_valid: two fp16 planes + row scales, K %% 32, ldw / plane %% 8, SiLU-GLU tiles");
            return d4::gemm_h2_launch(config, g, s);
        case D4_GEMM_SKINNY:
            D4_RUN_REFUSE(al16 && !g.Wb && d4::gemm_skinny_applicable(g) && (!(g.flags & d4::GEMM_SWIGLU) || g.N % 64 == 0),
                          "gemm_skinny_applicable: at most 256 rows and fewer than 64 tiles, K % 4, no transposed operand, C2 without batch");
            return d4::gemm_skinny(g, s);
        case D4_GEMM_BF16: {
            D4_RUN_REFUSE(((uintptr_t)g.A % 16) == 0 && !g.Ab && g.wplane == 0 && d4::gemm_bf16_config_valid(config, g), "gemm_bf16: bf16 weights, K %% 32, lda %% 4, ldw %% 8, SiLU-GLU tiles");
            d4::gemm_bf16_force_config(config);
            const int rc = d4::gemm_bf16(g, s);
            d4::gemm_bf16_force_config(-1);
            return rc;
        }
        case D4_GEMM_BF16A:
            D4_RUN_REFUSE(d4::gemm_bf16a_config_valid(config, g), "gemm_bf16a_config_valid: bf16 images of both operands, K %% 64, lda / ldw %% 8, SiLU-GLU tiles");
            return d4::gemm_bf16a_launch(config, g, s);
    }
    D4_REQUIRE(false, "d4_gemm_run: unknown family %d", family);
#undef D4_RUN_REFUSE
}
int d4_gemm_run_pair(const d4_gemm_desc* da, const d4_gemm_desc* db, int target, int config, void* stream) {
    if (int rc = gemm_desc_check("d4_gemm_run_pair", da)) return rc;
    if (int rc = gemm_desc_check("d4_gemm_run_pair", db)) return rc;
    const d4::GemmArgs a = gemm_args_of(*da), b = gemm_args_of(*db);
    hipStream_t s = static_cast<hipStream_t>(stream);
    auto al16 = [](const d4::GemmArgs& g) { return ((uintptr_t)g.A % 16) == 0 && ((uintptr_t)g.W % 16) == 0 && (g.lda % 4) == 0 && (g.ldw % 4) == 0; };
    switch (target) {
        case D4_PAIR_SKINNY:
            D4_REQUIRE(al16(a) && al16(b) && d4::gemm_skinny_pair_applicable(a, b),
                       "d4_gemm_run_pair: call not supported (gemm_skinny_pair_applicable: two few-row products of equal K, no SiLU-GLU, batch or mirror weights)");
            return d4::gemm_skinny_pair(a, b, s);
        case D4_PAIR_BF16A:
            D4_REQUIRE(d4::gemm_bf16a_pair_applicable(a, b),
                       "d4_gemm_run_pair: call not supported (gemm_bf16a_pair_applicable: equal K, flags == RMS, no bias / R / C2 / batch, a 64 x 64 or 128 x 64 tile by the rule)");
            return d4::gemm_bf16a_pair_launch(a, b, s);
        case D4_PAIR_V2:
            D4_REQUIRE(al16(a) && al16(b) && !a.Wb && !b.Wb && a.K == b.K && d4::gemm2_pair_config_ok(config) && d4::gemm2_pair_applicable(a, b) &&
                       d4::gemm2_config_valid(config, a) && d4::gemm2_config_valid(config, b),
                       "d4_gemm_run_pair: call not supported (gemm2 pair configuration %d: gemm2_pair_config_ok / gemm2_pair_applicable)", config);
            return d4::gemm2_pair_launch(config, a, b, s);
    }
    D4_REQUIRE(false, "d4_gemm_run_pair: unknown target %d", target);
}

int d4_tile16_weights(const float* W, int ldw, float* Wt, int N, int K, void* stream) {
    D4_REQUIRE(W && Wt && N >= 16 && K >= 4 && ldw >= K && ((uintptr_t)W % 16) == 0 && ((uintptr_t)Wt % 16) == 0, "d4_tile16_weights: bad arguments");
    return d4::tile16_weights(W, ldw, Wt, N, K, static_cast<hipStream_t>(stream));
}
static d4::SmallAttnArgs frame_attn_args(const float* q, int64_t q_group_stride, int64_t q_item_stride, const float* k, int64_t k_group_stride, int64_t k_item_stride,
                                         const float* v, int64_t v_group_stride, int64_t v_item_stride, const float* gate, int64_t g_group_stride, int64_t g_item_stride,
                                         const float* k_gamma, const float* vres, int64_t r_group_stride, int64_t r_item_stride, const float* mix, int64_t m_group_stride,
                                         int64_t m_item_stride, uint16_t* out_b, int frames, int heads, int S, float softclamp, int mask_special, int belief, int dh) {
    d4::SmallAttnArgs sa{};
    sa.q = q; sa.q_group_stride = q_group_stride; sa.q_item_stride = q_item_stride;
    sa.k = k; sa.k_group_stride = k_group_stride; sa.k_item_stride = k_item_stride;
    sa.v = v; sa.v_group_stride = v_group_stride; sa.v_item_stride = v_item_stride;
    sa.gate = gate; sa.g_group_stride = g_group_stride; sa.g_item_stride = g_item_stride;
    sa.k_gamma = k_gamma;
    sa.vres = vres; sa.r_group_stride = r_group_stride; sa.r_item_stride = r_item_stride;
    sa.mix = mix; sa.m_group_stride = m_group_stride; sa.m_item_stride = m_item_stride;
    sa.out_b = out_b;
    sa.groups = frames; sa.heads = heads; sa.nq = S; sa.nk = S;
    sa.softclamp = softclamp; sa.mask_special = mask_special; sa.belief = belief; sa.dh = dh;
    return sa;
}
static int frame_out_check(const char* who, const float* resid, const float* out, const float* c2, int S, int c2_lo, int c2_hi, int c2_last) {
    D4_REQUIRE(resid && out && ((uintptr_t)resid % 16) == 0 && ((uintptr_t)out % 16) == 0 && ((uintptr_t)c2 % 16) == 0, "%s: residual / output missing or not 16-byte aligned", who);
    D4_REQUIRE(!c2 || (c2_lo >= 0 && c2_hi >= c2_lo && c2_hi <= S && (c2_last == 0 || c2_last == 1)), "%s: bad compaction arguments", who);
    return 0;
}
int d4_frame_attn_out(const float* q, int64_t q_group_stride, int64_t q_item_stride, const float* k, int64_t k_group_stride, int64_t k_item_stride,
                      const float* v, int64_t v_group_stride, int64_t v_item_stride, const float* gate, int64_t g_group_stride, int64_t g_item_stride,
                      const float* k_gamma, const float* vres, int64_t r_group_stride, int64_t r_item_stride, const float* mix, int64_t m_group_stride,
                      int64_t m_item_stride, uint16_t* out_b, int frames, int heads, int S, float softclamp, int mask_special, int belief, int dh,
                      const float* wo_t, int D, const float* resid, int ldr, float* out, int ldo, float* c2, int ldc2, int c2_lo, int c2_hi, int c2_last,
                      void* stream) {
    const d4::SmallAttnArgs sa = frame_attn_args(q, q_group_stride, q_item_stride, k, k_group_stride, k_item_stride, v, v_group_stride, v_item_stride, gate, g_group_stride,
                                                 g_item_stride, k_gamma, vres, r_group_stride, r_item_stride, mix, m_group_stride, m_item_stride, out_b, frames, heads, S,
                                                 softclamp, mask_special, belief, dh);
    if (int rc = frame_out_check("d4_frame_attn_out", resid, out, c2, S, c2_lo, c2_hi, c2_last)) return rc;
    D4_REQUIRE(wo_t && ((uintptr_t)wo_t % 16) == 0 && ldr >= D && ldo >= D && (!c2 || ldc2 >= D), "d4_frame_attn_out: weight image missing / misaligned or a leading dimension below D");
    return d4::frame_attn_out(sa, wo_t, D, resid, ldr, out, ldo, c2, ldc2, c2_lo, c2_hi, c2_last, static_cast<hipStream_t>(stream));
}
int d4_attn_out_cols(const float* q, int64_t q_group_stride, int64_t q_item_stride, const float* k, int64_t k_group_stride, int64_t k_item_stride,
                     const float* v, int64_t v_group_stride, int64_t v_item_stride, const float* gate, int64_t g_group_stride, int64_t g_item_stride,
                     const float* k_gamma, const float* vres, int64_t r_group_stride, int64_t r_item_stride, const float* mix, int64_t m_group_stride,
                     int64_t m_item_stride, uint16_t* out_b, int frames, int heads, int S, float softclamp, int mask_special, int belief, int dh,
                     const float* W, int ldw, int D, const float* resid, int ldr, float* out, int ldo, float* c2, int ldc2, int c2_lo, int c2_hi, int c2_last,
                     void* stream) {
    const d4::SmallAttnArgs sa = frame_attn_args(q, q_group_stride, q_item_stride, k, k_group_stride, k_item_stride, v, v_group_stride, v_item_stride, gate, g_group_stride,
                                                 g_item_stride, k_gamma, vres, r_group_stride, r_item_stride, mix, m_group_stride, m_item_stride, out_b, frames, heads, S,
                                                 softclamp, mask_special, belief, dh);
    D4_REQUIRE(resid && out && (!c2 || (c2_lo >= 0 && c2_hi >= c2_lo && c2_hi <= S && (c2_last == 0 || c2_last == 1))), "d4_attn_out_cols: residual / output missing or bad compaction arguments");
    D4_REQUIRE(W && ldw >= heads * 64 && ldr >= D && ldo >= D && (!c2 || ldc2 >= D), "d4_attn_out_cols: weights missing or a leading dimension below its width");
    return d4::attn_out_cols(sa, W, ldw, D, resid, ldr, out, ldo, c2, ldc2, c2_lo, c2_hi, c2_last, static_cast<hipStream_t>(stream));
}
int d4_frame_pool(const float* q, int ldq, const float* x, int ldx, const float* gate_w, const float* k, int ldk, const float* hid, int D,
                  const float* k_gamma, int M, int L, int heads, float eps, const float* wv_t, const float* wo_t, int frames, int S, const float* resid,
                  int ldr, float* out, int ldo, float* c2, int ldc2, int c2_lo, int c2_hi, int c2_last, void* stream) {
    d4::PoolMixArgs pm{};
    pm.q = q; pm.ldq = ldq; pm.x = x; pm.ldx = ldx; pm.gate_w = gate_w; pm.k = k; pm.ldk = ldk; pm.hid = hid; pm.D = D; pm.k_gamma = k_gamma;
    pm.M = M; pm.L = L; pm.heads = heads; pm.eps = eps;
    if (int rc = frame_out_check("d4_frame_pool", resid, out, c2, S, c2_lo, c2_hi, c2_last)) return rc;
// ... 36 lines not shown
```

dreamer4_amd/csrc/gemm.hip:

```cpp
#include "common.h"
#include <string.h>
#include <hip/hip_ext.h>
#include "kernels.h"
#include <mutex>
#include <math.h>
#include <stdio.h>
#include <stdlib.h>
#include <map>
#include <tuple>
#include <type_traits>
#include <vector>

namespace d4 {


template <int BM, int BN, int WGM, int WGN, int BK, int KS, bool TA, bool TB, bool KTAIL>
__global__ __launch_bounds__(WGM * WGN * 64 * KS) void gemm_kernel(GemmArgs p) {
    constexpr int LDS_LD = BK + 4;
    constexpr int RF4 = BK / 4;
    constexpr int NT = WGM * WGN * 64 * KS;
    constexpr int TM = BM / WGM / 32;
    constexpr int TN = BN / WGN / 32;
    static_assert(TM >= 1 && TN >= 1, "tile");
    constexpr int A_F4 = BM * BK / 4 / NT;
// ... 580 lines not shown
    return (p.flags & GEMM_SWIGLU) ? 1 : 0;
}

static int autotune_v2(const GemmArgs& p, hipStream_t stream, int* best_out) {
    hipEvent_t e0 = prof_event(), e1 = prof_event();
    const int saved_mask = g_prof_mask;
    g_prof_mask = 0;
    int best = -1, rc = 0;
    float best_ms = 0.f;
    for (int c = 0; c < gemm2_configs() && !rc; ++c) {
        if (!gemm2_config_valid(c, p)) continue;
        if ((rc = gemm2_launch(c, p, stream))) break;
        float ms = 1e30f;
        for (int rep = 0; rep < 2 && !rc; ++rep) {
            (void)hipEventRecord(e0, stream);
            if ((rc = gemm2_launch(c, p, stream))) break;
            if ((rc = gemm2_launch(c, p, stream))) break;
            (void)hipEventRecord(e1, stream);
            if (hipEventSynchronize(e1) != hipSuccess) { rc = 1; break; }
            float t = 0.f;
            (void)hipEventElapsedTime(&t, e0, e1);
            ms = t < ms ? t : ms;
        }
        if (!rc && (best < 0 || ms < best_ms)) { best = c; best_ms = ms; }
    }
    g_prof_mask = saved_mask;
    g_event_pool.push_back(e0);
    g_event_pool.push_back(e1);
    if (rc) return rc;
    D4_REQUIRE(best >= 0, "gemm2: no configuration for M=%d N=%d K=%d flags=%d", p.M, p.N, p.K, p.flags);
    if (getenv("D4_GEMM_LOG"))
        fprintf(stderr, "[d4 gemm2] tuned M %6d N %5d K %5d batch %2d flags %3d -> %s (%.1f us)\n", p.M, p.N, p.K, p.batch, p.flags, gemm2_config_name(best), 500.f * best_ms);
    *best_out = best;
    return 0;
}

static bool use_v2(const GemmArgs& p) { return gemm2_applicable(p); }

static int gemm_v2(const GemmArgs& p, hipStream_t stream) {
    const bool tune_on = tune_mode() != 0;
    const int nb = p.batch > 0 ? p.batch : 1;
    const TuneKey key{p.M, p.N, p.K, p.flags, p.batch};
    tune_cache_load();
    auto it = g_tuned2.find(key);
    if (it != g_tuned2.end() && gemm2_config_valid(it->second, p)) return launch_v2(it->second, p, stream);
    const bool idempotent = !(p.flags & GEMM_ACCUMULATE) && p.R != p.C && p.A != p.C;
    hipStreamCaptureStatus cap = hipStreamCaptureStatusNone;
    (void)hipStreamIsCapturing(stream, &cap);
    if (!tune_on || !idempotent || cap != hipStreamCaptureStatusNone || 2.0 * p.M * p.N * p.K * nb < 1e8)
        return launch_v2(heuristic_v2(p), p, stream);
    if (tune_mode() == 2 && p.M <= 512) return launch_v2(heuristic_v2(p), p, stream);
    D4_TUNE_STRICT_CHECK(p, nb);
    int best = 0;
    if (int rc = autotune_v2(p, stream, &best)) return rc;
    g_tuned2[key] = best;
    tune_cache_append(key, 100 + best);
    return launch_v2(best, p, stream);
}

static int launch_v3(int c, const GemmArgs& p, hipStream_t stream) {
    const int cls = N_TILE_CFG + gemm2_configs() + c;
    const bool timed = ((g_prof_mask >> cls) & 1) && (g_prof_tick++ % g_prof_stride) == 0;
    if (!timed) return gemm_x3_launch(c, p, stream);
    ProfRec rec{};
    rec.a = prof_event(); rec.b = prof_event(); rec.cls = cls;
    rec.M = p.M; rec.N = p.N; rec.K = p.K; rec.flags = p.flags; rec.batch = p.batch;
    gemm_x3_config_tile(c, &rec.bm, &rec.bn);
    rec.flops = p.algo_flops > 0 ? p.algo_flops : 2.0 * p.M * p.N * p.K * (p.batch > 0 ? p.batch : 1);
    if (int rc = gemm_x3_launch(c, p, stream, rec.a, rec.b)) return rc;
    g_prof.push_back(rec);
    return 0;
}

static int launch_v3sk(const GemmArgs& p, hipStream_t stream) {
    const int cls = N_TILE_CFG + gemm2_configs() + gemm_x3_configs();
    const bool timed = ((g_prof_mask >> cls) & 1) && (g_prof_tick++ % g_prof_stride) == 0;
    if (!timed) return gemm_x3sk_launch(p, stream);
    ProfRec rec{};
    rec.a = prof_event(); rec.b = prof_event(); rec.cls = cls;
    rec.M = p.M; rec.N = p.N; rec.K = p.K; rec.flags = p.flags; rec.batch = p.batch;
    rec.bm = 128; rec.bn = 128;
    rec.flops = p.algo_flops > 0 ? p.algo_flops : 2.0 * p.M * p.N * p.K;
    if (int rc = gemm_x3sk_launch(p, stream, rec.a, rec.b)) return rc;
    g_prof.push_back(rec);
    return 0;
}

static int autotune_v3(const GemmArgs& p, hipStream_t stream, int* best_out) {
    hipEvent_t e0 = prof_event(), e1 = prof_event();
    const int saved_mask = g_prof_mask;
    g_prof_mask = 0;
    int best = -1, rc = 0;
    float best_ms = 0.f;
    for (int c = 0; c < gemm_x3_configs() && !rc; ++c) {
        if (!gemm_x3_config_valid(c, p)) continue;
        if ((rc = gemm_x3_launch(c, p, stream))) break;
        float ms = 1e30f;
        for (int rep = 0; rep < 2 && !rc; ++rep) {
            (void)hipEventRecord(e0, stream);
            if ((rc = gemm_x3_launch(c, p, stream))) break;
            if ((rc = gemm_x3_launch(c, p, stream))) break;
            (void)hipEventRecord(e1, stream);
            if (hipEventSynchronize(e1) != hipSuccess) { rc = 1; break; }
            float t = 0.f;
            (void)hipEventElapsedTime(&t, e0, e1);
            ms = t < ms ? t : ms;
        }
        if (!rc && (best < 0 || ms < best_ms)) { best = c; best_ms = ms; }
    }
    g_prof_mask = saved_mask;
    g_event_pool.push_back(e0);
    g_event_pool.push_back(e1);
    if (rc) return rc;
    D4_REQUIRE(best >= 0, "gemm_x3: no configuration for M=%d N=%d K=%d flags=%d", p.M, p.N, p.K, p.flags);
    if (getenv("D4_GEMM_LOG"))
        fprintf(stderr, "[d4 gemm_x3] tuned M %6d N %5d K %5d batch %2d flags %3d -> %s (%.1f us)\n", p.M, p.N, p.K, p.batch, p.flags, gemm_x3_config_name(best), 500.f * best_ms);
    *best_out = best;
    return 0;
}

static int gemm_v3(const GemmArgs& p, hipStream_t stream) {
    const bool tune_on = tune_mode() != 0;
    const int nb = p.batch > 0 ? p.batch : 1;
    if (g_forced_cfg >= 300 && gemm_x3_config_valid(g_forced_cfg - 300, p)) return launch_v3(g_forced_cfg - 300, p, stream);
    const TuneKey key{p.M, p.N, p.K, p.flags, p.batch};
    tune_cache_load();
    auto it = g_tuned3.find(key);
    if (it != g_tuned3.end() && gemm_x3_config_valid(it->second, p)) return launch_v3(it->second, p, stream);
    const bool idempotent = !(p.flags & GEMM_ACCUMULATE) && p.R != p.C && p.A != p.C;
    hipStreamCaptureStatus cap = hipStreamCaptureStatusNone;
    (void)hipStreamIsCapturing(stream, &cap);
    if (!tune_on || !idempotent || cap != hipStreamCaptureStatusNone || 2.0 * p.M * p.N * p.K * nb < 1e8)
        return launch_v3(gemm_x3_heuristic(p), p, stream);
    D4_TUNE_STRICT_CHECK(p, nb);
    int best = 0;
    if (int rc = autotune_v3(p, stream, &best)) return rc;
    g_tuned3[key] = best;
    tune_cache_append(key, 300 + best);
    return launch_v3(best, p, stream);
}

static int launch_v4(int c, const GemmArgs& p, hipStream_t stream) {
    const int cls = N_TILE_CFG + gemm2_configs() + gemm_x3_configs() + 1;
    const bool timed = ((g_prof_mask >> cls) & 1) && (g_prof_tick++ % g_prof_stride) == 0;
    if (!timed) return gemm_h2_launch(c, p, stream);
    ProfRec rec{};
    rec.a = prof_event(); rec.b = prof_event(); rec.cls = cls;
    rec.M = p.M; rec.N = p.N; rec.K = p.K; rec.flags = p.flags; rec.batch = p.batch;
    gemm_h2_config_tile(c, &rec.bm, &rec.bn);
    rec.flops = p.algo_flops > 0 ? p.algo_flops : 2.0 * p.M * p.N * p.K * (p.batch > 0 ? p.batch : 1);
    if (int rc = gemm_h2_launch(c, p, stream, rec.a, rec.b)) return rc;
    g_prof.push_back(rec);
    return 0;
}

static int autotune_v4(const GemmArgs& p, hipStream_t stream, int* best_out) {
    hipEvent_t e0 = prof_event(), e1 = prof_event();
    const int saved_mask = g_prof_mask;
    g_prof_mask = 0;
    int best = -1, rc = 0;
    float best_ms = 0.f;
    for (int c = 0; c < gemm_h2_configs() && !rc; ++c) {
        if (!gemm_h2_config_valid(c, p)) continue;
        if ((rc = gemm_h2_launch(c, p, stream))) break;
        float ms = 1e30f;
        for (int rep = 0; rep < 2 && !rc; ++rep) {
// ... 167 lines not shown
```

dreamer4_amd/csrc/gemm2.hip:

```cpp
#include "common.h"
#include <hip/hip_ext.h>
#include "kernels.h"
#include <stdlib.h>
#include <type_traits>

namespace d4 {

typedef __attribute__((address_space(3))) void* lds_void_ptr;

template <int N>
__device__ __forceinline__ void wait_vmcnt() {
    asm volatile("s_waitcnt vmcnt(%0)" ::"n"(N) : "memory");
}

template <int BK>
__device__ __forceinline__ int chunk_swizzle(int row) {
    if constexpr (BK == 32) return row & 7;
    else return (0x78 >> (((row >> 2) & 3) * 2)) & 3;
}

template <int WGM, int WGN, int TM, int TN, int NS, int BK, bool RMS, bool RMAP = false>
__device__ __forceinline__ void gemm2_body(GemmArgs& p, int bid, const int bz) {
    static_assert(BK == 16 || BK == 32, "k-tile");
    constexpr int CH = BK / 4;
    constexpr int RPP = 64 / CH;
    constexpr int H = BK / 16;
    constexpr int NW = WGM * WGN, NT = NW * 64;
    constexpr int BM = WGM * TM * 16, BN = WGN * TN * 16;
    constexpr int STAGE_ROWS = BM + BN;
    constexpr int STAGE_F = STAGE_ROWS * BK;
    constexpr int NSLOT = STAGE_ROWS / RPP;
    constexpr int LPW = (NSLOT + NW - 1) / NW;
    static_assert(NS >= 3 && NS <= 4 && 2 * LPW <= 63, "ring depth / vmcnt range");
    extern __shared__ __attribute__((aligned(16))) float smem[];

    const int tid = threadIdx.x, lane = tid & 63;
    const int wave = __builtin_amdgcn_readfirstlane(tid >> 6);
    const int wm = wave / WGN, wn = wave % WGN;

    const int nbn = (p.N + BN - 1) / BN, nbm = (p.M + BM - 1) / BM;
    {
        const int nblk = nbm * nbn, nx = 8;
        const int q = nblk / nx, r = nblk % nx, x = bid % nx, o = bid / nx;
        bid = (x < r ? x * (q + 1) : r * (q + 1) + (x - r) * q) + o;
    }
    const int bm0 = (bid / nbn) * BM, bn0 = (bid % nbn) * BN;
    p.A += bz * p.strideA; p.W += bz * p.strideW; p.C += bz * p.strideC;
    if (p.R) p.R += bz * p.strideC;

    const int rowsA = min(BM, p.M - bm0), rowsB = min(BN, p.N - bn0);
    auto uniform_rsrc = [](const float* base, int64_t bytes) {
        const uint64_t b = reinterpret_cast<uint64_t>(base);
        const uint32_t lo = __builtin_amdgcn_readfirstlane((uint32_t)b);
        const uint32_t hi = __builtin_amdgcn_readfirstlane((uint32_t)(b >> 32));
        const int nb = __builtin_amdgcn_readfirstlane((int)(bytes < 0x7FFFFFFF ? bytes : 0x7FFFFFFF));
        return __builtin_amdgcn_make_buffer_rsrc(reinterpret_cast<void*>(((uint64_t)hi << 32) | lo), 0, nb, 0x00020000);
    };
    const __amdgpu_buffer_rsrc_t rsA = uniform_rsrc(p.A + (int64_t)bm0 * p.lda, ((int64_t)(rowsA - 1) * p.lda + p.K) * 4);
    const __amdgpu_buffer_rsrc_t rsB = uniform_rsrc(p.W + (int64_t)bn0 * p.ldw, ((int64_t)(rowsB - 1) * p.ldw + p.K) * 4);

    uint32_t voff[LPW];
    const int prow = lane / CH;
    const int src_chunk = (lane % CH) ^ chunk_swizzle<BK>(prow);
#pragma unroll
    for (int i = 0; i < LPW; ++i) {
        const int slot = min(wave + NW * i, NSLOT - 1);
        const int r = slot * RPP + prow;
        voff[i] = (uint32_t)((slot * RPP < BM ? r * p.lda : (r - BM) * p.ldw) * 4 + src_chunk * 16);
    }
#define D4_ISSUE_STAGE(KT, BUF)                                                                                              \
    _Pragma("unroll") for (int i_ = 0; i_ < LPW; ++i_) {                                                                      \
        const int slot_ = min(wave + NW * i_, NSLOT - 1);                                                                     \
        float* dst_ = smem + (BUF) * STAGE_F + slot_ * 256;                                                                   \
        if (slot_ * RPP < BM) __builtin_amdgcn_raw_ptr_buffer_load_lds(rsA, (lds_void_ptr)dst_, 16, (uint32_t)voff[i_], (KT) * BK * 4, 0, 0); \
        else __builtin_amdgcn_raw_ptr_buffer_load_lds(rsB, (lds_void_ptr)dst_, 16, (uint32_t)voff[i_], (KT) * BK * 4, 0, 0);              \
    }

    f32x4 acc[TM][TN];
#pragma unroll
    for (int i = 0; i < TM; ++i)
#pragma unroll
        for (int j = 0; j < TN; ++j) acc[i][j] = f32x4{0.f, 0.f, 0.f, 0.f};

    const int kq = lane >> 4, frow = lane & 15;
    const int foff0 = frow * BK + ((kq ^ chunk_swizzle<BK>(frow)) << 2);
    const int a_base = wm * TM * 16 * BK, b_base = BM * BK + wn * TN * 16 * BK;

    constexpr int NPAR = 32 / BK;
    constexpr int SQI = RMS ? (BM * CH + NT - 1) / NT : 1;
    float ssq[SQI][NPAR];
#pragma unroll
    for (int i = 0; i < SQI; ++i)
#pragma unroll
        for (int h = 0; h < NPAR; ++h) ssq[i][h] = 0.f;

    const int nk = p.K / BK;
    auto wait_allow = [&](int stages) {
        if (stages >= 2) wait_vmcnt<2 * LPW>();
        else if (stages == 1) wait_vmcnt<LPW>();
        else wait_vmcnt<0>();
    };
    f32x4 af[2][TM], bf[2][TN];
    auto read_frags = [&](const float* st, auto set_tag, int second_half) {
        constexpr int SET = decltype(set_tag)::value;
        const int fo = second_half ? (foff0 ^ 16) : foff0;
#pragma unroll
        for (int i = 0; i < TM; ++i) af[SET][i] = *reinterpret_cast<const f32x4*>(st + a_base + i * 16 * BK + fo);
#pragma unroll
        for (int j = 0; j < TN; ++j) bf[SET][j] = *reinterpret_cast<const f32x4*>(st + b_base + j * 16 * BK + fo);
    };
    auto mfma_set = [&](auto set_tag) {
        constexpr int SET = decltype(set_tag)::value;
#pragma unroll
        for (int e = 0; e < 4; ++e)
#pragma unroll
            for (int i = 0; i < TM; ++i)
#pragma unroll
                for (int j = 0; j < TN; ++j)
                    acc[i][j] = __builtin_amdgcn_mfma_f32_16x16x4f32(bf[SET][j][e], af[SET][i][e], acc[i][j], 0, 0, 0);
    };
    using S0 = std::integral_constant<int, 0>;
    using S1 = std::integral_constant<int, 1>;

#pragma unroll
    for (int s = 0; s < NS - 1; ++s)
        if (s < nk) { D4_ISSUE_STAGE(s, s) }
    wait_allow(min(NS - 2, nk - 1));
    __builtin_amdgcn_s_barrier();
    read_frags(smem, S0{}, 0);

    auto k_tile = [&](int kt, auto par_tag) {
        constexpr int PAR = decltype(par_tag)::value;
        if (kt + 1 < nk) {
            wait_allow(min(kt + NS - 2, nk - 1) - (kt + 1));
            __builtin_amdgcn_s_barrier();
            if (kt + NS - 1 < nk) { D4_ISSUE_STAGE(kt + NS - 1, (kt + NS - 1) % NS) }
        }
        const float* st = smem + (kt % NS) * STAGE_F;
        const float* nxt = smem + ((kt + 1) % NS) * STAGE_F;
        if constexpr (RMS) {
#pragma unroll
            for (int i = 0; i < SQI; ++i) {
                const int idx = tid + i * NT;
                if (BM * CH % NT == 0 || idx < BM * CH) {
                    const f32x4 v = *reinterpret_cast<const f32x4*>(st + idx * 4);
                    ssq[i][PAR % NPAR] = ssq[i][PAR % NPAR] + __builtin_fmaf(v[3], v[3], __builtin_fmaf(v[2], v[2], __builtin_fmaf(v[1], v[1], v[0] * v[0])));
                }
            }
        }
        if constexpr (H == 2) {
            read_frags(st, S1{}, 1);
            mfma_set(S0{});
            if (kt + 1 < nk) read_frags(nxt, S0{}, 0);
            mfma_set(S1{});
        } else {
            using CUR = std::integral_constant<int, PAR>;
            using NXT = std::integral_constant<int, PAR ^ 1>;
            if (kt + 1 < nk) read_frags(nxt, NXT{}, 0);
            mfma_set(CUR{});
        }
    };
    for (int kt = 0; kt < nk; kt += 2) {
        k_tile(kt, S0{});
        if (kt + 1 < nk) k_tile(kt + 1, S1{});
    }

#undef D4_ISSUE_STAGE
    float* rowscale_s = smem + NS * STAGE_F;
    if constexpr (RMS) {
#pragma unroll
        for (int i = 0; i < SQI; ++i) {
            float s = ssq[i][0];
            s += dpp_f<0xB1>(s);
            s += dpp_f<0x4E>(s);
            if constexpr (NPAR == 1) {
                s += dpp_f<0x141>(s);
            } else {
                float s1 = ssq[i][1];
                s1 += dpp_f<0xB1>(s1);
                s1 += dpp_f<0x4E>(s1);
                s = s + s1;
            }
            const int idx = tid + i * NT;
            if ((idx % CH) == 0 && idx < BM * CH) rowscale_s[idx / CH] = rsqrtf(s / (float)p.K + p.rms_eps);
        }
        __syncthreads();
    }

    const bool swiglu = (p.flags & GEMM_SWIGLU) != 0;
    const bool vecC = (p.ldc % 4) == 0 && ((uintptr_t)p.C % 16) == 0;
    const bool vecR = p.R && (p.ldr % 4) == 0 && ((uintptr_t)p.R % 16) == 0;
    const bool vecC2 = p.C2 && (p.ldc2 % 4) == 0 && ((uintptr_t)p.C2 % 16) == 0;
#pragma unroll
    for (int i = 0; i < TM; ++i) {
        const int ml = wm * TM * 16 + i * 16 + frow;
        const int gm = bm0 + ml;
        if (gm >= p.M) continue;
        const float rs = RMS ? rowscale_s[ml] : 1.f;
        int64_t c2row = -1;
        if (p.C2) {
            const int ts = gm % p.c2_S, keep = p.c2_hi - p.c2_lo;
            const int rank = (ts >= p.c2_lo && ts < p.c2_hi) ? ts - p.c2_lo : ((p.c2_last && ts == p.c2_S - 1) ? keep : -1);
            if (rank >= 0) c2row = (int64_t)(gm / p.c2_S) * (keep + p.c2_last) + rank;
        }
        if (swiglu) {
            if constexpr (TN % 4 == 0) {
#pragma unroll
                for (int j = 0; j < TN; ++j) {
                    if ((j & 3) >= 2) continue;
                    const int gn = bn0 + wn * TN * 16 + j * 16 + kq * 4;
                    if (gn >= p.N) continue;
                    f32x4 o;
#pragma unroll
                    for (int e = 0; e < 4; ++e) {
                        float val = acc[i][j][e] * rs, gate = acc[i][j + 2][e] * rs;
                        if (p.bias) { val += p.bias[gn + e]; gate += p.bias[gn + e + 32]; }
                        o[e] = val * siluf(gate);
                    }
                    const int on = (gn / 64) * 32 + (gn % 64);
                    float* cp = p.C + (int64_t)gm * p.ldc + on;
                    if (vecC) *reinterpret_cast<f32x4*>(cp) = o;
                    else { cp[0] = o[0]; cp[1] = o[1]; cp[2] = o[2]; cp[3] = o[3]; }
                }
            }
            continue;
        }
#pragma unroll
        for (int j = 0; j < TN; ++j) {
            const int gn = bn0 + wn * TN * 16 + j * 16 + kq * 4;
            if (gn >= p.N) continue;
            const bool full = gn + 3 < p.N;
            f32x4 v;
#pragma unroll
            for (int e = 0; e < 4; ++e) v[e] = acc[i][j][e] * rs;
            if (p.bias) {
#pragma unroll
                for (int e = 0; e < 4; ++e) if (full || gn + e < p.N) v[e] += p.bias[gn + e];
            }
            if (p.flags & GEMM_SILU) {
#pragma unroll
                for (int e = 0; e < 4; ++e) v[e] = siluf(v[e]);
            }
            if (p.R) {
                const float* rp = p.R + (int64_t)gm * p.ldr + gn;
                if (vecR && full) { const f32x4 r4 = *reinterpret_cast<const f32x4*>(rp); v[0] += r4[0]; v[1] += r4[1]; v[2] += r4[2]; v[3] += r4[3]; }
                else {
#pragma unroll
                    for (int e = 0; e < 4; ++e) if (full || gn + e < p.N) v[e] += rp[e];
                }
            }
            int64_t crow = gm;
            if constexpr (RMAP) {
                const int fr = gm / p.rm_Sc, t = gm - fr * p.rm_Sc;
                crow = (int64_t)fr * (p.rm_Sc + p.rm_nr) + t + (t >= p.rm_lo ? p.rm_nr : 0);
            }
            float* cp = p.C + crow * p.ldc + gn;
            if (p.flags & GEMM_ACCUMULATE) {
#pragma unroll
                for (int e = 0; e < 4; ++e) if (full || gn + e < p.N) v[e] += cp[e];
            }
            if (vecC && full) *reinterpret_cast<f32x4*>(cp) = v;
            else {
#pragma unroll
                for (int e = 0; e < 4; ++e) if (full || gn + e < p.N) cp[e] = v[e];
            }
            if (c2row >= 0) {
                float* c2 = p.C2 + c2row * p.ldc2 + gn;
                if (vecC2 && full) *reinterpret_cast<f32x4*>(c2) = v;
                else {
#pragma unroll
                    for (int e = 0; e < 4; ++e) if (full || gn + e < p.N) c2[e] = v[e];
                }
            }
        }
    }
}

template <int WGM, int WGN, int TM, int TN, int NS, int BK, bool RMS>
__global__ __launch_bounds__(WGM* WGN * 64) void gemm2_kernel(GemmArgs p) {
    gemm2_body<WGM, WGN, TM, TN, NS, BK, RMS>(p, blockIdx.x, blockIdx.y);
}

template <int WGM, int WGN, int TM, int TN, int NS, int BK, bool RMS>
__global__ __launch_bounds__(WGM* WGN * 64) void gemm2_rowmap_kernel(GemmArgs p) {
    gemm2_body<WGM, WGN, TM, TN, NS, BK, RMS, true>(p, blockIdx.x, blockIdx.y);
}

template <int WGM, int WGN, int TM, int TN, int NS, int BK, bool RMS>
__global__ __launch_bounds__(WGM* WGN * 64) void gemm2_pair_kernel(GemmArgs a, GemmArgs b, int nblk_a) {
    const int bid = blockIdx.x;
    if (bid < nblk_a) gemm2_body<WGM, WGN, TM, TN, NS, BK, RMS>(a, bid, 0);
    else gemm2_body<WGM, WGN, TM, TN, NS, BK, RMS>(b, bid - nblk_a, 0);
}

constexpr int KS_GROUPS = 4, KS_NS = 3, KS_BM = 32, KS_BN = 64, KS_BK = 32;
constexpr int KS_STAGE_F = (KS_BM + KS_BN) * KS_BK;
constexpr int KS_RING_F = KS_NS * KS_STAGE_F;
constexpr int KS_LDP = KS_BN + 4;

__global__ __launch_bounds__(1024) void gemm2_ksplit_kernel(GemmArgs p) {
    constexpr int BK = KS_BK, CH = 8, RPP = 8, BM = KS_BM, BN = KS_BN, NS = KS_NS, LPW = 3, NSLOT = (BM + BN) / RPP;
    extern __shared__ __attribute__((aligned(16))) float smem[];
    const int tid = threadIdx.x, lane = tid & 63;
    const int wave = __builtin_amdgcn_readfirstlane(tid >> 6);
    const int grp = wave >> 2, w = wave & 3, wm = w >> 1, wn = w & 1;
    int bid = blockIdx.x;
    const int nbn = (p.N + BN - 1) / BN, nbm = (p.M + BM - 1) / BM;
    {
        const int nblk = nbm * nbn, nx = 8;
        const int q = nblk / nx, r = nblk % nx, x = bid % nx, o = bid / nx;
        bid = (x < r ? x * (q + 1) : r * (q + 1) + (x - r) * q) + o;
    }
    const int bm0 = (bid / nbn) * BM, bn0 = (bid % nbn) * BN;
    const int rowsA = min(BM, p.M - bm0), rowsB = min(BN, p.N - bn0);
    auto uniform_rsrc = [](const float* base, int64_t bytes) {
        const uint64_t b = reinterpret_cast<uint64_t>(base);
        const uint32_t lo = __builtin_amdgcn_readfirstlane((uint32_t)b);
        const uint32_t hi = __builtin_amdgcn_readfirstlane((uint32_t)(b >> 32));
        const int nb = __builtin_amdgcn_readfirstlane((int)(bytes < 0x7FFFFFFF ? bytes : 0x7FFFFFFF));
        return __builtin_amdgcn_make_buffer_rsrc(reinterpret_cast<void*>(((uint64_t)hi << 32) | lo), 0, nb, 0x00020000);
    };
    const __amdgpu_buffer_rsrc_t rsA = uniform_rsrc(p.A + (int64_t)bm0 * p.lda, ((int64_t)(rowsA - 1) * p.lda + p.K) * 4);
    const __amdgpu_buffer_rsrc_t rsB = uniform_rsrc(p.W + (int64_t)bn0 * p.ldw, ((int64_t)(rowsB - 1) * p.ldw + p.K) * 4);
    uint32_t voff[LPW];
    const int prow = lane / CH;
    const int src_chunk = (lane % CH) ^ chunk_swizzle<BK>(prow);
#pragma unroll
    for (int i = 0; i < LPW; ++i) {
        const int slot = w + 4 * i;
        const int r = slot * RPP + prow;
        voff[i] = (uint32_t)((slot * RPP < BM ? r * p.lda : (r - BM) * p.ldw) * 4 + src_chunk * 16);
    }
    float* ring = smem + grp * KS_RING_F;
    const int nkt = p.K / BK, nk = (nkt + KS_GROUPS - 1) / KS_GROUPS;
    const int mine = nkt / KS_GROUPS + (grp < nkt % KS_GROUPS ? 1 : 0);
    const int kt0 = grp * (nkt / KS_GROUPS) + min(grp, nkt % KS_GROUPS);
    const __amdgpu_buffer_rsrc_t rs0 = uniform_rsrc(p.A, 0);
#define D4_KS_ISSUE(KT, BUF)                                                                                                      \
    _Pragma("unroll") for (int i_ = 0; i_ < LPW; ++i_) {                                                                           \
        const int slot_ = w + 4 * i_;                                                                                               \
        float* dst_ = ring + (BUF) * KS_STAGE_F + slot_ * 256;                                                                      \
        const __amdgpu_buffer_rsrc_t rs_ = (KT) < mine ? (slot_ * RPP < BM ? rsA : rsB) : rs0;                                    \
        __builtin_amdgcn_raw_ptr_buffer_load_lds(rs_, (lds_void_ptr)dst_, 16, (uint32_t)voff[i_], (kt0 + (KT)) * BK * 4, 0, 0);           \
    }
    f32x4 acc[2] = {f32x4{0.f, 0.f, 0.f, 0.f}, f32x4{0.f, 0.f, 0.f, 0.f}};
    const int kq = lane >> 4, frow = lane & 15;
    const int foff0 = frow * BK + ((kq ^ chunk_swizzle<BK>(frow)) << 2);
    const int a_base = wm * 16 * BK, b_base = BM * BK + wn * 32 * BK;
    auto wait_allow = [&](int stages) {
        if (stages >= 2) wait_vmcnt<2 * LPW>();
        else if (stages == 1) wait_vmcnt<LPW>();
        else wait_vmcnt<0>();
    };
    f32x4 af[2], bf[2][2];
    auto read_frags = [&](const float* st, int set, int second_half) {
        const int fo = second_half ? (foff0 ^ 16) : foff0;
        af[set] = *reinterpret_cast<const f32x4*>(st + a_base + fo);
        bf[set][0] = *reinterpret_cast<const f32x4*>(st + b_base + fo);
        bf[set][1] = *reinterpret_cast<const f32x4*>(st + b_base + 16 * BK + fo);
// ... 188 lines not shown
```

dreamer4_amd/csrc/gemm_x3sk.hip:

```cpp
#include "common.h"
#include <hip/hip_ext.h>
#include "kernels.h"
#include <type_traits>

namespace d4 {

typedef __bf16 bf16x8 __attribute__((ext_vector_type(8)));


constexpr int SK_BM = 128, SK_BN = 128, SK_WGM = 4, SK_WGN = 2, SK_D = 3;
constexpr int SK_BK = 32, SK_LD = SK_BK + 8, SK_NT = SK_WGM * SK_WGN * 64;
constexpr int SK_G = SK_BK / 8;
constexpr int SK_APL = SK_BM * SK_LD, SK_BPL = SK_BN * SK_LD;
constexpr size_t SK_LDS = (size_t)(2 * 3 * (SK_BM + SK_BN) * SK_LD) * 2 + SK_BM * sizeof(float) + 16;
static_assert(SK_BM * SK_G == SK_NT && SK_BN * SK_G == SK_NT, "one 8-element group of each operand per thread and k-tile");

struct SkArgs {
    GemmArgs p;
    int P, F, R;
    int half;
};

__device__ __forceinline__ void split3(float a, __bf16& h1, __bf16& h2, __bf16& h3) {
    h1 = (__bf16)a;
    const float r = a - (float)h1;
    h2 = (__bf16)r;
    h3 = (__bf16)(r - (float)h2);
}


template <int TNV, bool RMAP>
__device__ __forceinline__ void sk_item(const SkArgs& s, const int bm0, const int bn0, __bf16* As, __bf16* Bs, float* rowscale_s) {
    const GemmArgs& p = s.p;
    const int kt0 = 0, kt1 = p.K / SK_BK;
    constexpr int BNV = 64 * TNV;
    const int tid = threadIdx.x, lane = tid & 63;
    const int wave = __builtin_amdgcn_readfirstlane(tid >> 6);
    const int wm = wave / SK_WGN, wn = wave % SK_WGN;
    const int lrow = lane & 31, lhalf = lane >> 5;
    const __bf16* Wb = reinterpret_cast<const __bf16*>(p.Wb);
    const int rowsA = min(SK_BM, p.M - bm0), rowsB = min(BNV, p.N - bn0);
    auto uniform_rsrc = [](const void* base, int64_t bytes) {
        const uint64_t bb = reinterpret_cast<uint64_t>(base);
        const uint32_t lo = __builtin_amdgcn_readfirstlane((uint32_t)bb);
        const uint32_t hi = __builtin_amdgcn_readfirstlane((uint32_t)(bb >> 32));
        const int nb = __builtin_amdgcn_readfirstlane((int)(bytes < 0x7FFFFFFF ? bytes : 0x7FFFFFFF));
        return __builtin_amdgcn_make_buffer_rsrc(reinterpret_cast<void*>(((uint64_t)hi << 32) | lo), 0, nb, 0x00020000);
    };
    const __amdgpu_buffer_rsrc_t rsA = uniform_rsrc(p.A + (int64_t)bm0 * p.lda, ((int64_t)(rowsA - 1) * p.lda + p.K) * 4);
    const int64_t wbytes = ((int64_t)(rowsB - 1) * p.ldw + p.K) * 2;
    const __amdgpu_buffer_rsrc_t rsB0 = uniform_rsrc(Wb + (int64_t)bn0 * p.ldw, wbytes);
    const __amdgpu_buffer_rsrc_t rsB1 = uniform_rsrc(Wb + p.wplane + (int64_t)bn0 * p.ldw, wbytes);
    const __amdgpu_buffer_rsrc_t rsB2 = uniform_rsrc(Wb + 2 * p.wplane + (int64_t)bn0 * p.ldw, wbytes);

    f32x4 ra[SK_D][2];
    f32x4 rb[SK_D][3];
    float ssq0 = 0.f, ssq1 = 0.f;
    using S0 = std::integral_constant<int, 0>;
    using S1 = std::integral_constant<int, 1>;
    using S2 = std::integral_constant<int, 2>;
    const int srow = tid / SK_G, scol = (tid % SK_G) * 8;
    const int browB = TNV == 2 ? srow : (srow & 63);
    const bool b_store = TNV == 2 || srow < 64;
    const uint32_t offA = (uint32_t)((srow * p.lda + scol) * 4), offB = (uint32_t)((browB * p.ldw + scol) * 2);
    auto load_tile = [&](auto set_tag, int k0) {
        constexpr int S = decltype(set_tag)::value;
        ra[S][0] = __builtin_bit_cast(f32x4, __builtin_amdgcn_raw_buffer_load_b128(rsA, offA + (uint32_t)k0 * 4, 0, 0));
        ra[S][1] = __builtin_bit_cast(f32x4, __builtin_amdgcn_raw_buffer_load_b128(rsA, offA + (uint32_t)k0 * 4 + 16, 0, 0));
        rb[S][0] = __builtin_bit_cast(f32x4, __builtin_amdgcn_raw_buffer_load_b128(rsB0, offB + (uint32_t)k0 * 2, 0, 0));
        rb[S][1] = __builtin_bit_cast(f32x4, __builtin_amdgcn_raw_buffer_load_b128(rsB1, offB + (uint32_t)k0 * 2, 0, 0));
        rb[S][2] = __builtin_bit_cast(f32x4, __builtin_amdgcn_raw_buffer_load_b128(rsB2, offB + (uint32_t)k0 * 2, 0, 0));
    };
    auto store_tile = [&](auto set_tag, int buf) {
        constexpr int S = decltype(set_tag)::value;
        __bf16* as = As + buf * 3 * SK_APL + srow * SK_LD + scol;
        __bf16* bs = Bs + buf * 3 * SK_BPL + browB * SK_LD + scol;
        if (b_store) {
            *reinterpret_cast<f32x4*>(bs) = rb[S][0];
            *reinterpret_cast<f32x4*>(bs + SK_BPL) = rb[S][1];
            *reinterpret_cast<f32x4*>(bs + 2 * SK_BPL) = rb[S][2];
        }
        const f32x4 v0 = ra[S][0], v1 = ra[S][1];
        bf16x8 o1, o2, o3;
#pragma unroll
        for (int e = 0; e < 4; ++e) {
// ... 87 lines not shown
        rsum = ssq0 + ssq1;
        rsum += dpp_f<0xB1>(rsum);
        rsum += dpp_f<0x4E>(rsum);
    }
    const bool row_lane = (tid % SK_G) == 0;

    if (rms) {
        if (row_lane) rowscale_s[srow] = rsqrtf(rsum / (float)p.K + p.rms_eps);
        __syncthreads();
    }

    const bool swiglu = (p.flags & GEMM_SWIGLU) != 0;
    if (TNV == 1 && swiglu) {
        float* xs = reinterpret_cast<float*>(As);
        const int gn = bn0 + lrow;
        if (wn == 1) {
#pragma unroll
            for (int e = 0; e < 16; ++e) {
                const int lr = wm * 32 + (e & 3) + 8 * (e >> 2) + 4 * lhalf;
                float gate = hi[0][e] * (rms ? rowscale_s[lr] : 1.f);
                if (p.bias) gate += p.bias[gn + 32];
                xs[lr * 33 + lrow] = siluf(gate);
            }
        }
        __syncthreads();
        if (wn == 0 && gn < p.N) {
#pragma unroll
            for (int e = 0; e < 16; ++e) {
                const int lr = wm * 32 + (e & 3) + 8 * (e >> 2) + 4 * lhalf;
                const int gm = bm0 + lr;
                if (gm >= p.M) continue;
                float val = hi[0][e] * (rms ? rowscale_s[lr] : 1.f);
                if (p.bias) val += p.bias[gn];
                const int on = (gn / 64) * 32 + (gn % 64);
                p.C[(int64_t)gm * p.ldc + on] = val * xs[lr * 33 + lrow];
            }
        }
        __syncthreads();
        return;
    }
#pragma unroll
    for (int e = 0; e < 16; ++e) {
        const int lr = wm * 32 + (e & 3) + 8 * (e >> 2) + 4 * lhalf;
        const int gm = bm0 + lr;
        if (gm >= p.M) continue;
        const float rs = rms ? rowscale_s[lr] : 1.f;
        if (swiglu) {
            if constexpr (TNV == 2) {
                const int gn = bn0 + wn * 64 + lrow;
                if (gn >= p.N) continue;
                float val = hi[0][e] * rs, gate = hi[1][e] * rs;
                if (p.bias) { val += p.bias[gn]; gate += p.bias[gn + 32]; }
                const int on = (gn / 64) * 32 + (gn % 64);
                p.C[(int64_t)gm * p.ldc + on] = val * siluf(gate);
            }
        } else {
#pragma unroll
            for (int j = 0; j < TNV; ++j) {
                const int gn = bn0 + wn * TNV * 32 + j * 32 + lrow;
                if (gn >= p.N) continue;
                float v = hi[j][e] * rs;
                if (p.bias) v += p.bias[gn];
                if (p.flags & GEMM_SILU) v = siluf(v);
                if (p.R) v += p.R[(int64_t)gm * p.ldr + gn];
                if constexpr (RMAP) {
                    const int fr = gm / p.rm_Sc, t = gm - fr * p.rm_Sc;
                    p.C[((int64_t)fr * (p.rm_Sc + p.rm_nr) + t + (t >= p.rm_lo ? p.rm_nr : 0)) * p.ldc + gn] = v;
                    continue;
                }
                if (p.flags & GEMM_ACCUMULATE) v += p.C[(int64_t)gm * p.ldc + gn];
                p.C[(int64_t)gm * p.ldc + gn] = v;
                if (p.C2) {
                    const int ts = gm % p.c2_S;
                    const int keep = p.c2_hi - p.c2_lo;
                    const int rank = (ts >= p.c2_lo && ts < p.c2_hi) ? ts - p.c2_lo : ((p.c2_last && ts == p.c2_S - 1) ? keep : -1);
                    if (rank >= 0) p.C2[((int64_t)(gm / p.c2_S) * (keep + p.c2_last) + rank) * p.ldc2 + gn] = v;
                }
            }
        }
    }
    __syncthreads();
}

template <bool RMAP>
__device__ __forceinline__ void sk_walk(const SkArgs s) {
    const GemmArgs& p = s.p;
    extern __shared__ __attribute__((aligned(16))) char smem_raw[];
    __bf16* As = reinterpret_cast<__bf16*>(smem_raw);
    __bf16* Bs = As + 2 * 3 * SK_APL;
    float* rowscale_s = reinterpret_cast<float*>(Bs + 2 * 3 * SK_BPL);

    const int b = blockIdx.x;
    const int nbn = (p.N + SK_BN - 1) / SK_BN, nbm = (p.M + SK_BM - 1) / SK_BM;
    const int nk_all = p.K / SK_BK;
    auto tile_of = [&](int tile, int& tm, int& tn) {
        int bid = tile;
        const int nblk = nbm * nbn, nx = 8;
        const int q = nblk / nx, r = nblk % nx, x = bid % nx, o = bid / nx;
        bid = (x < r ? x * (q + 1) : r * (q + 1) + (x - r) * q) + o;
        constexpr int RB = 4;
        const int band = bid / (RB * nbn), j = bid % (RB * nbn);
        const int rows = min(RB, nbm - band * RB);
        tm = band * RB + j % rows; tn = j / rows;
    };
    int tm, tn;
    if (s.half) {
        for (int i = 0; i < s.F; ++i) {
            tile_of(b + i * s.P, tm, tn);
            sk_item<2, RMAP>(s, tm * SK_BM, tn * SK_BN, As, Bs, rowscale_s);
        }
        const int R8 = (s.R + 7) & ~7;
        if (R8 + s.R <= s.P) {
            const int j = b < s.R ? b : b - R8, half = b < s.R ? 0 : 1;
            if (j >= 0 && j < s.R && (b < s.R || b >= R8)) {
                tile_of(s.F * s.P + j, tm, tn);
                const int bn0 = tn * SK_BN + half * 64;
                if (bn0 < p.N) sk_item<1, RMAP>(s, tm * SK_BM, bn0, As, Bs, rowscale_s);
            }
            return;
        }
        for (int h = b; h < 2 * s.R; h += s.P) {
            tile_of(s.F * s.P + h / 2, tm, tn);
            const int bn0 = tn * SK_BN + (h & 1) * 64;
            if (bn0 < p.N) sk_item<1, RMAP>(s, tm * SK_BM, bn0, As, Bs, rowscale_s);
        }
        return;
    }
    for (int i = 0; i < s.F + (b < s.R ? 1 : 0); ++i) {
        tile_of(b + i * s.P, tm, tn);
        sk_item<2, RMAP>(s, tm * SK_BM, tn * SK_BN, As, Bs, rowscale_s);
    }
}

__global__ __launch_bounds__(SK_NT, 2) void gemm_x3sk_kernel(SkArgs s) { sk_walk<false>(s); }
__global__ __launch_bounds__(SK_NT, 2) void gemm_x3sk_rowmap_kernel(SkArgs s) { sk_walk<true>(s); }

static std::atomic<int> g_sk_cus[64];

static int sk_cus() {
    int dev = 0;
    if (hipGetDevice(&dev) != hipSuccess) dev = 0;
    std::atomic<int>& c = g_sk_cus[dev & 63];
    int n = c.load(std::memory_order_relaxed);
    if (n == 0) {
        if (hipDeviceGetAttribute(&n, hipDeviceAttributeMultiprocessorCount, dev) != hipSuccess || n <= 0) n = 256;
        c.store(n, std::memory_order_relaxed);
    }
    return n;
}


const char* gemm_x3sk_name() { return "gemm_x3sk_kernel"; }

bool gemm_x3sk_applicable(const GemmArgs& p) {
    return gemm_x3_applicable(p) && p.batch <= 1 && p.M > 0 && (!(p.flags & GEMM_SWIGLU) || (p.N % 64) == 0);
}

bool gemm_x3sk_half_plan(const GemmArgs& p, int* F, int* R, int* P_out) {
    const int P = sk_cus();
    const int T = cdiv(p.M, SK_BM) * cdiv(p.N, SK_BN);
    const int f = T / P, r = T - f * P;
    *F = f; *R = r;
    if (P_out) *P_out = P;
    return r > 0 && 2 * r <= P;
}

bool gemm_x3sk_rule(const GemmArgs& p) {
    if (!gemm_x3sk_applicable(p) || p.M < 1024 || p.N < 512) return false;
    int F, R, P;
    return gemm_x3sk_half_plan(p, &F, &R, &P) && F >= 1 && F <= 3;
}

int gemm_x3sk_launch(const GemmArgs& p, hipStream_t stream, hipEvent_t ea, hipEvent_t eb) {
    D4_REQUIRE(gemm_x3sk_applicable(p), "gemm_x3sk: call not supported (M=%d N=%d K=%d flags=%d batch=%d)", p.M, p.N, p.K, p.flags, p.batch);
    SkArgs a;
    a.p = p;
    a.half = gemm_x3sk_half_plan(p, &a.F, &a.R, &a.P) ? 1 : 0;
    const int T = a.F * a.P + a.R;
    if (T < a.P && !a.half) a.P = T;
    D4_REQUIRE(gemm_rowmap_ok(p), "gemm_x3sk: bad output row map (Sc=%d lo=%d nr=%d) or an epilogue it does not cover (flags=%d)", p.rm_Sc, p.rm_lo, p.rm_nr, p.flags);
    const bool rmap = p.rm_Sc > 0;
    auto k = rmap ? gemm_x3sk_rowmap_kernel : gemm_x3sk_kernel;
    static DeviceOnce attr_set[2];
    if (attr_set[rmap].need()) {
        D4_HIP(hipFuncSetAttribute(reinterpret_cast<const void*>(k), hipFuncAttributeMaxDynamicSharedMemorySize, (int)SK_LDS));
        attr_set[rmap].done();
    }
    const dim3 grid(a.P), block(SK_NT);
    if (ea) hipExtLaunchKernelGGL(k, grid, block, (uint32_t)SK_LDS, stream, ea, eb, 0, a);
    else hipLaunchKernelGGL(k, grid, block, SK_LDS, stream, a);
    D4_LAUNCH_CHECK();
    return 0;
}

}
```

dreamer4_amd/csrc/kernels.h:

```cpp
#pragma once
#include <hip/hip_runtime.h>
#include <stdint.h>

namespace d4 {

enum : int {
    GEMM_RMS_ROWSCALE = 1,
    GEMM_SILU = 2,
    GEMM_SWIGLU = 4,
    GEMM_TRANS_A = 8,
    GEMM_TRANS_B = 16,
    GEMM_ACCUMULATE = 32,
};

struct GemmArgs {
    const float* A; int lda;
    const float* W; int ldw;
    float* C; int ldc;
    const float* bias;
    const float* R; int ldr;
    int M, N, K;
    int flags;
    float rms_eps;
    double algo_flops = 0;
    float* C2 = nullptr; int ldc2 = 0, c2_S = 0, c2_lo = 0, c2_hi = 0, c2_last = 1;
    int batch = 1; int64_t strideA = 0, strideW = 0, strideC = 0;
    const uint16_t* Wb = nullptr;
    const uint16_t* Ab = nullptr;
    uint16_t* Cb = nullptr;
    uint16_t* C2b = nullptr;
    int group_m = 0;
    uint16_t rm_Sc = 0, rm_lo = 0;
    int64_t wplane = 0;
    const float* wscale = nullptr;
    int64_t strideWs = 0;
    const int* aexp = nullptr;
    int rule_M = 0;
    uint16_t rm_nr = 0, rm_spare = 0;
};
static_assert(sizeof(GemmArgs) == 232, "GemmArgs is a kernel argument: the row map lives in its alignment gaps");
bool gemm_rowmap_ok(const GemmArgs& p);
int gemm_rowmap_refused(const GemmArgs& p, const char* who);
bool gemm_rule_takes_x3sk(const GemmArgs& p);

int gemm(const GemmArgs& p, hipStream_t stream);
bool gemm_rule_takes_v2(const GemmArgs& p);
bool gemm_bf16_applicable(const GemmArgs& p);
int gemm_bf16(const GemmArgs& p, hipStream_t stream);
int gemm_bf16_configs();
bool gemm_bf16_config_valid(int c, const GemmArgs& p);
int gemm_bf16_force_config(int id);
void gemm_bf16a_force_config(int id);
int cvt_f32_to_bf16(const float* src, uint16_t* dst, int64_t n, hipStream_t s);
int cvt_rows_bf16(const float* src, int64_t lds, uint16_t* dst, int64_t ldd, int rows, int cols, hipStream_t s);
int gemm_bf16a(const GemmArgs& p, hipStream_t stream);
bool gemm_bf16a_applicable(const GemmArgs& p);
bool gemm_bf16a_config_valid(int c, const GemmArgs& p);
int gemm_bf16a_configs();
int gemm_bf16a_rule(const GemmArgs& p);
int gemm_bf16a_launch(int c, const GemmArgs& p, hipStream_t stream, hipEvent_t ea = nullptr, hipEvent_t eb = nullptr);
int gemm_bf16p_launch(const GemmArgs& p, hipStream_t stream, hipEvent_t ea = nullptr, hipEvent_t eb = nullptr);
bool gemm_bf16a_pair_applicable(const GemmArgs& a, const GemmArgs& b);
int gemm_bf16a_pair_launch(const GemmArgs& a, const GemmArgs& b, hipStream_t stream, hipEvent_t ea = nullptr, hipEvent_t eb = nullptr);
int gemm_bf16a_pair(const GemmArgs& a, const GemmArgs& b, hipStream_t stream);
void gemm_bf16_profile_enable(int stride);
int gemm_bf16_profile_read(double* ms, double* flops, int64_t* count);
bool gemm_x3_applicable(const GemmArgs& p);
bool gemm_x3_config_valid(int c, const GemmArgs& p);
int gemm_x3_configs();
const char* gemm_x3_config_name(int c);
void gemm_x3_config_tile(int c, int* bm, int* bn);
int gemm_x3_heuristic(const GemmArgs& p);
int gemm_x3_launch(int c, const GemmArgs& p, hipStream_t stream, hipEvent_t ea = nullptr, hipEvent_t eb = nullptr);
int split_bf16x3(const float* src, uint16_t* dst, int64_t n, int64_t plane, hipStream_t s);
bool gemm_h2_applicable(const GemmArgs& p);
bool gemm_h2_config_valid(int c, const GemmArgs& p);
int gemm_h2_configs();
const char* gemm_h2_config_name(int c);
void gemm_h2_config_tile(int c, int* bm, int* bn);
int gemm_h2_heuristic(const GemmArgs& p);
bool gemm_h2_takes(const GemmArgs& p);
int gemm_h2_launch(int c, const GemmArgs& p, hipStream_t stream, hipEvent_t ea = nullptr, hipEvent_t eb = nullptr);
int split_f16x2_rows(const float* src, uint16_t* dst, int rows, int cols, int ld, int64_t plane, float* inv_scale, hipStream_t s);
int row_scale_exp(const float* A, int64_t lda, int rows, int K, int* out, hipStream_t s);
bool gemm_x3sk_applicable(const GemmArgs& p);
bool gemm_x3sk_rule(const GemmArgs& p);
const char* gemm_x3sk_name();
int gemm_x3sk_launch(const GemmArgs& p, hipStream_t stream, hipEvent_t ea = nullptr, hipEvent_t eb = nullptr);
bool gemm2_applicable(const GemmArgs& p);
bool gemm2_config_valid(int c, const GemmArgs& p);
int gemm2_configs();
const char* gemm2_config_name(int c);
void gemm2_config_tile(int c, int* bm, int* bn);
int gemm2_launch(int c, const GemmArgs& p, hipStream_t stream, hipEvent_t ea = nullptr, hipEvent_t eb = nullptr);
bool gemm2_ksplit_applicable(const GemmArgs& p);
bool gemm2_ksplit_rule(const GemmArgs& p);
int gemm2_ksplit_launch(const GemmArgs& p, hipStream_t stream, hipEvent_t ea = nullptr, hipEvent_t eb = nullptr);
bool gemm2_pair_config_ok(int c);
bool gemm2_pair_applicable(const GemmArgs& a, const GemmArgs& b);
int gemm2_pair_launch(int c, const GemmArgs& a, const GemmArgs& b, hipStream_t stream, hipEvent_t ea = nullptr, hipEvent_t eb = nullptr);
int gemm_pair(const GemmArgs& a, const GemmArgs& b, hipStream_t stream);
bool gemm_skinny_applicable(const GemmArgs& p);
int gemm_skinny(const GemmArgs& p, hipStream_t stream);
bool gemm_skinny_pair_applicable(const GemmArgs& a, const GemmArgs& b);
int gemm_skinny_pair(const GemmArgs& a, const GemmArgs& b, hipStream_t stream);
int gemm_profile_enable(int on);
bool gemm_profile_active();
int gemm_profile_read(double* ms, double* flops, int64_t* count, int nclass);
int gemm_profile_classes();
extern int g_time_attn_fused_append;
extern int g_pool_wide_keys;
extern int g_attn_out_cols;
extern int g_time_attn_tiled;
extern int g_space_attn_tiled;
extern int g_cross_attn_tiled;
extern int g_small_attn_wide;
int gemm_force_config(int id);
int gemm_configs();
bool gemm_config_valid(int c, const GemmArgs& p);
const char* gemm_profile_class_name(int c);

struct SmallAttnArgs {
    const float* q;      int64_t q_group_stride, q_item_stride;
    const float* k;      int64_t k_group_stride, k_item_stride;
    const float* v;      int64_t v_group_stride, v_item_stride;
    const float* gate;   int64_t g_group_stride, g_item_stride;
    const float* k_gamma;
    const float* vres;   int64_t r_group_stride, r_item_stride;
    const float* mix;    int64_t m_group_stride, m_item_stride;
    float* out;          int64_t o_group_stride, o_item_stride;
    int groups, heads, nq, nk;
    float softclamp;
    int mask_special;
    int belief;
    int q_lo = 0, q_hi = 0, q_last = 1;
    int q_compact = 0;
    int dh = 64;
    uint16_t* out_b = nullptr;
    int wide = 0;
};
int small_attn(const SmallAttnArgs& p, hipStream_t stream);
constexpr int WIDE_ATTN_MAX = 1024;
int wide_attn(const SmallAttnArgs& p, hipStream_t stream, const char** form);
int wide_attn_bf16_launch(const SmallAttnArgs& p, hipStream_t stream, const char** form);

struct PoolMixArgs {
    const float* q; int ldq;
    const float* x; int ldx;
    const float* gate_w;
    const float* k; int ldk;
    const float* hid; int D;
    const float* k_gamma;
    float* u;
    int M, L, heads;
    float eps;
    uint16_t* u_b = nullptr;
    const uint16_t* k_b = nullptr;
    const uint16_t* q_b = nullptr;
    const uint16_t* hid_b = nullptr;
    int rule_M = 0;
};
int pool_mix(const PoolMixArgs& p, hipStream_t stream);
constexpr int POOL_DEEP_MAX = 1024;
constexpr int POOL_DEEP_CHUNK = 64;
int pool_mix_deep(const PoolMixArgs& p, hipStream_t stream);
extern int g_pool_mix_deep;
void note_pool_deep_form(const char* name);

bool lqap_in_applicable(int heads, int dh, int n, int ns, int dl);
int lqap_in(const float* latents, int ldl, const float* w_kv, int ldw, const float* q, const float* gate, const float* k_gamma, float* out, int frames,
            int heads, int n, int ns, int dl, float eps, hipStream_t s);
// ... 156 lines not shown
```

include/d4hip.h:

```cpp
#ifndef D4HIP_H
#define D4HIP_H

#include <stddef.h>
#include <stdint.h>

#ifdef __cplusplus
extern "C" {
#endif

#define D4_MAX_ACTION_TYPES 8
#define D4_MODE_DYNAMICS 0
#define D4_MODE_DECODER 1
#define D4_MODE_ENCODER 2
#define D4_MLP_PRE_RMS 0
#define D4_MLP_POST_LAYER 1
#define D4_BETA_SOFTPLUS_P1 0
#define D4_BETA_EXP_P1 1

typedef struct d4_config {
    int32_t dim, dim_latent, num_latent_tokens, depth, time_block_every;
    int32_t attn_heads, attn_dim_head;
    float attn_softclamp_value;
    int32_t num_spatial_tokens, num_register_tokens, max_steps, num_tasks;
    int32_t num_discrete_action_types;
// ... 234 lines not shown
int d4_cross_attn_backward_saved(const float* q_tokens, const float* ctx, const float* dy, const float* norm_w, const float* norm_ctx_w, const float* wq,
                           const float* wk, const float* wv, const float* wo, const float* w_gates, const float* k_gamma, int groups, int nq, int nk,
                           int ctx_item_major, int dim, int dim_ctx, int heads, int dim_head, float softclamp,
                           float* d_q_tokens, float* d_ctx, float* d_norm_w, float* d_norm_ctx_w, float* d_wq, float* d_wk, float* d_wv, float* d_wo,
                           float* d_w_gates, float* d_k_gamma, float* workspace, size_t workspace_bytes, void* stream);
int d4_rmsnorm(const float* x, int ldx, const float* gamma, float* y, int ldy, int rows, int dim,
               float eps, void* stream);
int d4_small_attn(const float* q, int64_t q_group_stride, int64_t q_item_stride, const float* k, int64_t k_group_stride, int64_t k_item_stride,
                  const float* v, int64_t v_group_stride, int64_t v_item_stride, const float* gate, int64_t g_group_stride, int64_t g_item_stride,
                  const float* k_gamma, const float* vres, int64_t r_group_stride, int64_t r_item_stride, const float* mix, int64_t m_group_stride,
                  int64_t m_item_stride, float* out, int64_t o_group_stride, int64_t o_item_stride, uint16_t* out_b, int groups, int heads, int nq, int nk,
                  float softclamp, int mask_special, int belief, int q_lo, int q_hi, int q_last, int dh, void* stream);
int d4_small_attn_wide(const float* q, int64_t q_group_stride, int64_t q_item_stride, const float* k, int64_t k_group_stride, int64_t k_item_stride,
                  const float* v, int64_t v_group_stride, int64_t v_item_stride, const float* gate, int64_t g_group_stride, int64_t g_item_stride,
                  const float* k_gamma, const float* vres, int64_t r_group_stride, int64_t r_item_stride, const float* mix, int64_t m_group_stride,
                  int64_t m_item_stride, float* out, int64_t o_group_stride, int64_t o_item_stride, uint16_t* out_b, int groups, int heads, int nq, int nk,
                  float softclamp, int mask_special, int belief, int q_lo, int q_hi, int q_last, int dh, void* stream);
int d4_small_attn_wide_bf16(const float* q, int64_t q_group_stride, int64_t q_item_stride, const float* k, int64_t k_group_stride, int64_t k_item_stride,
                  const float* v, int64_t v_group_stride, int64_t v_item_stride, const float* gate, int64_t g_group_stride, int64_t g_item_stride,
                  const float* k_gamma, const float* vres, int64_t r_group_stride, int64_t r_item_stride, const float* mix, int64_t m_group_stride,
                  int64_t m_item_stride, float* out, int64_t o_group_stride, int64_t o_item_stride, uint16_t* out_b, int groups, int heads, int nq, int nk,
                  float softclamp, int mask_special, int belief, int q_lo, int q_hi, int q_last, int dh, void* stream);
int d4_pool_mix(const float* q, int ldq, const float* x, int ldx, const float* gate_w, const float* k, int ldk, const float* hid, int D,
                const float* k_gamma, float* u, int M, int L, int heads, float eps, uint16_t* u_b, const uint16_t* k_b, const uint16_t* q_b,
                const uint16_t* hid_b, void* stream);
int d4_pool_mix_deep(const float* q, int ldq, const float* x, int ldx, const float* gate_w, const float* k, int ldk, const float* hid, int D,
                     const float* k_gamma, float* u, int M, int L, int heads, float eps, uint16_t* u_b, const uint16_t* k_b, const uint16_t* q_b,
                     const uint16_t* hid_b, void* stream);
int d4_time_attn_decode(const float* proj, int ldp, const float* vres, int ldv, const float* k_gamma, const float* inv_freq, float* cache, float* out,
                        int ldo, uint16_t* out_b, int B, int S, int H, int Tq, int t0, int Tcap, int cache_batch, int cache_S, const int* t0_dev,
                        float softclamp, int dh, int mode, void* stream);
const char* d4_debug_last_form(const char* family);
int d4_debug_forms(const char* family, int i, const char** name);

size_t d4_train_attn_core_plane_floats(int rows, int heads, int dim_head);
size_t d4_train_xattn_core_plane_floats(int q_rows, int k_rows, int heads, int dim_head);
int d4_train_attn_core(const float* proj, int ldp, const float* rv, const float* gamma, const float* d_o3,
                       float* o3, float* dproj, float* d_rv, float* dgamma_part,
                       int groups, int items, int heads, int dim_head, float softclamp, int num_special, int belief,
                       int g_inner, int64_t g_outer_stride, int64_t item_stride, int causal, const float* inv_freq,
                       int core, float* planes, size_t plane_floats, void* stream);
int d4_train_xattn_core(const float* projq, int ldq, const float* projk, int ldk, const float* gamma, const float* d_o3,
                        float* o3, float* dprojq, float* dprojk, float* dgamma_part,
                        int groups, int nq, int nk, int heads, int dim_head, int item_major, float softclamp,
                        int core, float* planes, size_t plane_floats, void* stream);
size_t d4_train_attn_core_bf16_plane_floats(int groups, int items, int heads, int dim_head);
size_t d4_train_xattn_core_bf16_plane_floats(int groups, int nq, int nk, int heads, int dim_head);
int d4_train_attn_core_bf16(const float* proj, int ldp, const float* rv, const float* gamma, const float* d_o3,
                            float* o3, float* dproj, float* d_rv, float* dgamma_part,
                            int groups, int items, int heads, int dim_head, float softclamp, int num_special, int belief,
                            int g_inner, int64_t g_outer_stride, int64_t item_stride, int causal, const float* inv_freq,
                            int core, float* planes, size_t plane_floats, void* stream);
int d4_train_xattn_core_bf16(const float* projq, int ldq, const float* projk, int ldk, const float* gamma, const float* d_o3,
                             float* o3, float* dprojq, float* dprojk, float* dgamma_part,
                             int groups, int nq, int nk, int heads, int dim_head, int item_major, float softclamp,
                             int core, float* planes, size_t plane_floats, void* stream);

typedef struct d4_gemm_desc {
    const float* A; int32_t lda;
    const float* W; int32_t ldw;
    float* C; int32_t ldc;
    const float* bias;
    const float* R; int32_t ldr;
    int32_t M, N, K, flags;
    float rms_eps;
    float* C2; int32_t ldc2, c2_S, c2_lo, c2_hi, c2_last;
    int32_t batch; int64_t strideA, strideW, strideC;
    const uint16_t* Ab; const uint16_t* Wb; uint16_t* Cb; uint16_t* C2b;
    int64_t wplane; const float* wscale; int64_t strideWs; const int32_t* aexp;
} d4_gemm_desc;
#define D4_GEMM_TILE 0
#define D4_GEMM_V2 1
#define D4_GEMM_V2_KSPLIT 2
#define D4_GEMM_X3 3
#define D4_GEMM_X3SK 4
#define D4_GEMM_H2 5
#define D4_GEMM_SKINNY 6
#define D4_GEMM_BF16 7
#define D4_GEMM_BF16A 8
#define D4_GEMM_FAMILIES 9
int d4_gemm_family_configs(int family);
int d4_gemm_run(const d4_gemm_desc* d, int family, int config, void* stream);
int d4_gemm_run_rowmap(const d4_gemm_desc* d, int family, int config, int rm_Sc, int rm_S, int rm_lo, int rm_nr, void* stream);
#define D4_PAIR_SKINNY 0
#define D4_PAIR_BF16A 1
#define D4_PAIR_V2 2
int d4_gemm_run_pair(const d4_gemm_desc* a, const d4_gemm_desc* b, int target, int config, void* stream);
int d4_tile16_weights(const float* W, int ldw, float* Wt, int N, int K, void* stream);
int d4_frame_attn_out(const float* q, int64_t q_group_stride, int64_t q_item_stride, const float* k, int64_t k_group_stride, int64_t k_item_stride,
                      const float* v, int64_t v_group_stride, int64_t v_item_stride, const float* gate, int64_t g_group_stride, int64_t g_item_stride,
                      const float* k_gamma, const float* vres, int64_t r_group_stride, int64_t r_item_stride, const float* mix, int64_t m_group_stride,
                      int64_t m_item_stride, uint16_t* out_b, int frames, int heads, int S, float softclamp, int mask_special, int belief, int dh,
                      const float* wo_t, int D, const float* resid, int ldr, float* out, int ldo, float* c2, int ldc2, int c2_lo, int c2_hi, int c2_last,
                      void* stream);
int d4_attn_out_cols(const float* q, int64_t q_group_stride, int64_t q_item_stride, const float* k, int64_t k_group_stride, int64_t k_item_stride,
                     const float* v, int64_t v_group_stride, int64_t v_item_stride, const float* gate, int64_t g_group_stride, int64_t g_item_stride,
                     const float* k_gamma, const float* vres, int64_t r_group_stride, int64_t r_item_stride, const float* mix, int64_t m_group_stride,
                     int64_t m_item_stride, uint16_t* out_b, int frames, int heads, int S, float softclamp, int mask_special, int belief, int dh,
                     const float* W, int ldw, int D, const float* resid, int ldr, float* out, int ldo, float* c2, int ldc2, int c2_lo, int c2_hi, int c2_last,
                     void* stream);
int d4_frame_pool(const float* q, int ldq, const float* x, int ldx, const float* gate_w, const float* k, int ldk, const float* hid, int D,
                  const float* k_gamma, int M, int L, int heads, float eps, const float* wv_t, const float* wo_t, int frames, int S, const float* resid,
                  int ldr, float* out, int ldo, float* c2, int ldc2, int c2_lo, int c2_hi, int c2_last, void* stream);
int d4_frame_pool_tail(const float* u, const float* wv_t, const float* wo_t, int frames, int S, int D, int pool_heads, const float* resid, int ldr,
                       float* out, int ldo, float* c2, int ldc2, int c2_lo, int c2_hi, int c2_last, void* stream);
int d4_lqap_in(const float* latents, int ldl, const float* w_kv, int ldw, const float* q, const float* gate, const float* k_gamma, float* out, int frames,
               int heads, int n, int ns, int dl, float eps, void* stream);
int d4_lqap_out(const float* kv, int ldkv, const float* q, const float* gate, const float* k_gamma, const float* w_out, int ldw, float* pred, int ldp,
                int frames, int heads, int n, int ns, int dl, void* stream);

int d4_rmsnorm_backward(const float* x, const float* dy, const float* gamma, float* dx, float* d_gamma, float* scratch, int rows, int dim, float eps,
                        void* stream);
int d4_layernorm_rows(const float* x, int ldx, const float* g, const float* b, float* y, int ldy, int rows, int dim, float eps, int silu, void* stream);
typedef struct d4_assemble_desc {
    float* tokens;
    const float* space;
    const float* signal_embed;
    const float* step_embed;
    const float* registers;
    const float* agent_embed;
    const float* task_embed;
    const float* action_embed;
    const float* action_learned;
    const int32_t* signal_levels;
    int32_t signal_uniform;
    const int64_t* prev_actions;
    const float* prev_cont;
    const float* cont_embed;
    const int64_t* tasks;
    const int32_t* action_offsets;
    int32_t B, Tq, S, D, ns, nr, na, nc, step_log2;
    float* compact;
    int32_t has_agent;
} d4_assemble_desc;
int d4_assemble_tokens(const d4_assemble_desc* d, void* stream);
int d4_gather_space_double_norm(const float* tokens, float* out, const float* g0, const float* g1, int frames, int S, int first, int dim, int ns,
                                float eps, void* stream);
int d4_colsum(const float* x, int ld, int rows, int cols, float* out, float* scratch, size_t scratch_floats, void* stream);
int d4_colsum_batch(int n, const float* const* x, const int32_t* ld, const int32_t* rows, const int32_t* cols, float* const* out, void* stream);
int d4_rmsnorm_bwd(const float* x, const float* dxhat, const float* gamma, float* tg, float* dx, int rows, int dim, float eps, void* stream);
int d4_euler_step_rows(float* x, int ldx, const float* pred, int ldp, int B, int n_el, float one_minus_t, float dt, void* stream);
int d4_splitk_reduce(const float* part, int S, int M, int N, const float* bias, int silu, float* y, int ldy, void* stream);
int d4_mean_tokens(const float* x, float* out, int B, int n, int d, void* stream);
int d4_hl_gauss_scalar_strided(const float* logits, int ld, const float* centers, float* out, int out_stride, int rows, int bins, void* stream);
int d4_unary_rows(int op, const float* x, float* y, int64_t n, void* stream);
int d4_copy_rows(const float* src, int lds, float* dst, int ldd, int rows, int cols, void* stream);
int d4_fold_rows(const float* W, const float* gamma, float* out, int rows, int K, int ld_out, void* stream);
int d4_swiglu_pack_rows(const float* W, const float* bias, const float* gamma, float* Wp, float* bp, int inner, int inner_pad, int K, void* stream);
int d4_build_latent_input(float* out, const float* hist, const float* ctx_noise, const float* x, int B, int Tq, int n_el, int hist_t_stride, float w, void* stream);
int d4_pad_cols(const float* W, float* out, int rows, int cols, int cols_pad, void* stream);
int d4_video_patches(const float* src, float* dst, int B, int C, int T, int nh, int nw, int ps, int to_patches, void* stream);
int d4_cache_transfer(float* cache, float* ext, int Lt, int cache_batch, int B, int S, int H, int Tcap, int frames, int to_ext, int dh, void* stream);
int d4_cunembed(int op, const float* src, float* dst, int nc, int mtp, int d, void* stream);
int d4_coord_grid(float* out, int nh, int nw, int ld, void* stream);
int d4_pack_tokens(int which, float* tokens, float* compact, const float* pos, const float* img, const float* lat, int frames, int P, int n_lat, int n_total,
                   int D, void* stream);
int d4_prep_eval_inputs(int32_t* sig, int64_t* pact, const int64_t* actions_hist, int B, int Tq, int na, int frame_base, int hist_stride, int sig_val, int ctx_sig,
                        float* pcont, const float* cont_hist, int nc, void* stream);
int d4_layernorm_silu_bwd(const float* z, int ldz, const float* da, const float* g, const float* b, float* tg, float* tb, float* dz, int rows, int dim, float eps,
                          void* stream);
int d4_silu_bwd(const float* dy, const float* z, float* dz, int64_t n, void* stream);
int d4_swiglu(int bwd, const float* h, const float* du, float* out, int rows, int inner, int inner_pad, void* stream);
int d4_multi_copy(int count, float* const* dst, const float* const* src, const int64_t* n, void* stream);
int d4_zero_pad_cols(float* x, int rows, int ld, int c0, int c1, void* stream);
int d4_cvt_pad_bf16(const float* src, int64_t lds, uint16_t* dst, int64_t ldd, int rows, int cols, int cols_pad, void* stream);
int d4_cvt_transpose_bf16(const float* src, int lds, uint16_t* dst, int ldd, int rows, int cols, int rows_pad, void* stream);
// ... 71 lines not shown
```

Measured before the change: 23140 imagined steps/s.

## Fill idle workgroups of the FF-in stream-K GEMM with pool key tiles

```diff
diff --git a/dreamer4_amd/_lib.py b/dreamer4_amd/_lib.py
--- a/dreamer4_amd/_lib.py
+++ b/dreamer4_amd/_lib.py
@@ -206,6 +206,9 @@
     'd4_gemm_run': (_I, [C.POINTER(GemmDesc), _I, _I, _P]),
     'd4_gemm_run_rowmap': (_I, [C.POINTER(GemmDesc), _I, _I, _I, _I, _I, _I, _P]),
     'd4_gemm_run_pair': (_I, [C.POINTER(GemmDesc), C.POINTER(GemmDesc), _I, _I, _P]),
+    'd4_gemm_fill_capacity': (_I, [C.POINTER(GemmDesc)]),
+    'd4_gemm_run_fill': (_I, [C.POINTER(GemmDesc), C.POINTER(GemmDesc), _I, _P]),
+    'd4_gemm_run_fill_rowmap': (_I, [C.POINTER(GemmDesc), C.POINTER(GemmDesc), _I, _I, _I, _I, _I, _P]),
     'd4_tile16_weights': (_I, [_P, _I, _P, _I, _I, _P]),
     'd4_frame_attn_out': (_I, [_P, _L, _L] * 4 + [_P] + [_P, _L, _L] * 2 + [_P] + [_I] * 3 + [_F] + [_I] * 3 + [_P, _I, _P, _I, _P, _I, _P, _I, _I, _I, _I, _P]),
     'd4_attn_out_cols': (_I, [_P, _L, _L] * 4 + [_P] + [_P, _L, _L] * 2 + [_P] + [_I] * 3 + [_F] + [_I] * 3 + [_P, _I, _I, _P, _I, _P, _I, _P, _I, _I, _I, _I, _P]),
diff --git a/dreamer4_amd/csrc/engine.hip b/dreamer4_amd/csrc/engine.hip
--- a/dreamer4_amd/csrc/engine.hip
+++ b/dreamer4_amd/csrc/engine.hip
@@ -772,11 +772,25 @@
     return 0;
 }
 
+static GemmArgs ff_in_call(d4_engine* e, const FfPrep& fp, const float* x, int ldx, int rows) {
+    GemmArgs g1{x, ldx, fp.w1, e->D, e->ffh, e->inner_pad, fp.b1, nullptr, 0, rows, 2 * e->inner_pad, e->D,
+                GEMM_RMS_ROWSCALE | GEMM_SWIGLU, RMS_EPS, 2.0 * rows * (2.0 * e->inner) * e->D};
+    if (e->bf16 && e->split) {
+        for (const auto& m : e->mirrors)
+            if (g1.W >= m.src && g1.W < m.src + m.n) { g1.Wb = m.dst + (g1.W - m.src); break; }
+        if (g1.Wb) { g1.wplane = (int64_t)e->bf16_cap; if (!gemm_x3_applicable(g1)) { g1.Wb = nullptr; g1.wplane = 0; } }
+    }
+    return g1;
+}
+
 static int ff_block(d4_engine* e, const FfPrep& fp, const float* out_b, const float* x, int ldx, float* y, int ldy,
-                    int rows, hipStream_t s, float* y_compact = nullptr, int S = 0, int has_agent = 1) {
+                    int rows, hipStream_t s, float* y_compact = nullptr, int S = 0, int has_agent = 1, const GemmArgs* fill = nullptr) {
     int rc;
     GemmArgs g1{x, ldx, fp.w1, e->D, e->ffh, e->inner_pad, fp.b1, nullptr, 0, rows, 2 * e->inner_pad, e->D,
                 GEMM_RMS_ROWSCALE | GEMM_SWIGLU, RMS_EPS, 2.0 * rows * (2.0 * e->inner) * e->D};
+    if (fill) {
+        if ((rc = gemm_x3sk_fill(ff_in_call(e, fp, x, ldx, rows), *fill, gemm_x3sk_fill_tiles(*fill), s))) return rc;
+    } else
     if ((rc = engine_gemm(g1, s))) return rc;
     GemmArgs g2{e->ffh, e->inner_pad, fp.w2, e->inner_pad, y, ldy, out_b, x, ldx, rows, e->D, e->inner_pad, 0, RMS_EPS,
                 2.0 * rows * (double)e->D * e->inner};
@@ -792,9 +806,18 @@
 int g_last_layer_compact_q = 1;
 int g_layer0_const_rows = 1;
 int g_pool_const_keys = 1;
+int g_ff_fill_pool_keys = 1;
 unsigned g_launch_count = 0;
+static GemmArgs pool_key_call(d4_engine* e, int p, const float* hiddens, int L, int M, int rule_M, float* keys0) {
+    const int D = e->D, hp = e->hp;
+    GemmArgs gk{hiddens, D, e->pkv_w[p], D, e->pool_kv, hp, nullptr, nullptr, 0, L * M, hp, D, GEMM_RMS_ROWSCALE, RMS_EPS};
+    gk.rule_M = L * rule_M;
+    if (keys0) { gk.A = hiddens + (size_t)M * D; gk.C = keys0 + (size_t)M * hp; gk.M = (L - 1) * M; gk.rule_M = L * M; }
+    return gk;
+}
+
 static int pool_block(d4_engine* e, int p, const float* x, float* y, int L, int M, hipStream_t s, const float* hiddens = nullptr,
-                      float* y_compact = nullptr, int S = 0, int has_agent = 1, int rule_M = 0, float* keys0 = nullptr) {
+                      float* y_compact = nullptr, int S = 0, int has_agent = 1, int rule_M = 0, float* keys0 = nullptr, int keys_done = 0) {
     if (!hiddens) hiddens = e->slabs;
     const d4_config& c = e->c;
     const int D = e->D, hp = e->hp;
@@ -816,12 +839,9 @@
             pm.k = nullptr; pm.k_b = e->kall_b + (size_t)p * hp; pm.ldk = ld;
             pm.q = nullptr; pm.q_b = e->kall_b + (size_t)(L - 1) * M * ld + (size_t)(c.depth - 1) * hp; pm.ldq = ld;
         } else {
-        GemmArgs gk{hiddens, D, e->pkv_w[p], D, e->pool_kv, hp, nullptr, nullptr, 0, L * M, hp, D, GEMM_RMS_ROWSCALE, RMS_EPS};
-        gk.rule_M = L * rule_M;
-        if (keys0) {
-            gk.A = hiddens + (size_t)M * D; gk.C = keys0 + (size_t)M * hp; gk.M = (L - 1) * M; gk.rule_M = L * M;
-            pm.k = keys0;
-        }
+        GemmArgs gk = pool_key_call(e, p, hiddens, L, M, rule_M, keys0);
+        if (keys0) pm.k = keys0;
+        if (keys_done > 0) { gk.A += (size_t)keys_done * D; gk.C += (size_t)keys_done * hp; gk.M -= keys_done; gk.rule_M = L * M; }
         if ((rc = gemm_two(gq, gk, s))) return rc;
         if (t_bf16) pm.k_b = t_bf16->shadow_of(e->pool_kv);
         }
@@ -1081,10 +1101,28 @@
         float* h1 = slab(2 * l + 1);
         float* h2 = slab(2 * l + 2);
         if (!fused_out && (rc = gemm_c2(e->att, hd, a.to_out, hd, h1, D, M, D, hd, 0, nullptr, x_in, D, cslab(2 * l + 1), S, t_keep_hi - t_keep_lo, has_agent, s))) return rc;
-        if ((rc = ff_block(e, e->ffp[l], e->layer_ff[l].out_b, h1, D, h2, D, M, s, cslab(2 * l + 2), S, has_agent))) return rc;
+        GemmArgs kfill{};
+        int keys_done = 0;
+        if (g_ff_fill_pool_keys && dynamics && e->split && l < c.depth - 1 && c.pool_heads == 4 && D <= 1024 && !e->kall_b) {
+            const int L = 2 * l + 3;
+            const GemmArgs g1 = ff_in_call(e, e->ffp[l], h1, D, M);
+            const int cap = g1.Wb && gemm_rule_takes_x3sk(g1) ? gemm_x3sk_fill_capacity(g1) : 0;
+            const GemmArgs gk = pool_key_call(e, l, e->slabs, L, M, 0, keys0(l));
+            const int ready = (gk.M - M) / 128;
+            const int per_block = (e->hp + 63) / 64;
+            const int blocks = cap / per_block < ready ? cap / per_block : ready;
+            if (blocks > 0 && tiled_family(L * M, e->hp, D, GEMM_RMS_ROWSCALE, e->pkv_w[l]) &&
+                tiled_family(gk.M - 128 * blocks, e->hp, D, GEMM_RMS_ROWSCALE, e->pkv_w[l], L * M)) {
+                keys_done = 128 * blocks;
+                kfill = gk;
+                kfill.M = keys_done; kfill.rule_M = 0;
+                D4_REQUIRE(gemm_x3sk_fill_applicable(kfill), "ff_fill_pool_keys: the key problem of pool %d is no fill problem", l);
+            }
+        }
+        if ((rc = ff_block(e, e->ffp[l], e->layer_ff[l].out_b, h1, D, h2, D, M, s, cslab(2 * l + 2), S, has_agent, keys_done ? &kfill : nullptr))) return rc;
         if (l != c.depth - 1) {
             float* xc = (denoise_only && l == c.depth - 2 && !e->is_time[c.depth - 1] && S <= 16 && S >= 8) ? e->xpool_c : nullptr;
-            if ((rc = pool_block(e, l, h2, e->xpool, 2 * l + 3, M, s, nullptr, xc, S, has_agent, 0, keys0(l)))) return rc;
+            if ((rc = pool_block(e, l, h2, e->xpool, 2 * l + 3, M, s, nullptr, xc, S, has_agent, 0, keys0(l), keys_done))) return rc;
             x_in = e->xpool;
         }
     }
@@ -1519,7 +1557,7 @@
     const bool lean = d4::g_rollout_clean_agent_row != 0;
     const int lean_keep = (lean && d4::engine_clean_agent_only(e)) ? 1 : c.num_spatial_tokens + 1;
     const int variant = (lean ? 1 : 0) | (d4::g_lqap_in_fused ? 2 : 0) | (d4::g_lqap_out_fused ? 4 : 0) | (d4::g_last_layer_compact_q ? 8 : 0) |
-                        (d4::g_layer0_const_rows ? 16 : 0) | (d4::g_pool_const_keys ? 32 : 0);
+                        (d4::g_layer0_const_rows ? 16 : 0) | (d4::g_pool_const_keys ? 32 : 0) | (d4::g_ff_fill_pool_keys ? 64 : 0);
     const float* hist = nullptr;
     if (d4::g_rollout_batched_heads && F >= 1 && F <= e->head_rows) {
         if (io->agent_embed) hist = io->agent_embed;
@@ -1690,6 +1728,11 @@
         d4::g_launch_count = (unsigned)value;
         return old;
     }
+    if (name && !strcmp(name, "ff_fill_launches")) {
+        const int old = (int)(d4::g_fill_launches & 0x7fffffffu);
+        d4::g_fill_launches = (unsigned)value;
+        return old;
+    }
     if (name && !strcmp(name, "time_attn_fused_append")) sw = &d4::g_time_attn_fused_append;
     else if (name && !strcmp(name, "rollout_clean_agent_row")) sw = &d4::g_rollout_clean_agent_row;
     else if (name && !strcmp(name, "rollout_batched_heads")) sw = &d4::g_rollout_batched_heads;
@@ -1699,6 +1742,7 @@
     else if (name && !strcmp(name, "last_layer_compact_q")) sw = &d4::g_last_layer_compact_q;
     else if (name && !strcmp(name, "layer0_const_rows")) sw = &d4::g_layer0_const_rows;
     else if (name && !strcmp(name, "pool_const_keys")) sw = &d4::g_pool_const_keys;
+    else if (name && !strcmp(name, "ff_fill_pool_keys")) sw = &d4::g_ff_fill_pool_keys;
     else if (name && !strcmp(name, "pool_wide_keys")) sw = &d4::g_pool_wide_keys;
     else if (name && !strcmp(name, "pool_mix_deep")) sw = &d4::g_pool_mix_deep;
     else if (name && !strcmp(name, "time_attn_tiled")) sw = &d4::g_time_attn_tiled;
@@ -2127,6 +2171,26 @@
     D4_REQUIRE(false, "d4_gemm_run: unknown family %d", family);
 #undef D4_RUN_REFUSE
 }
+int d4_gemm_fill_capacity(const d4_gemm_desc* main) {
+    if (!main || main->M < 1 || main->N < 1 || main->K < 1) return 0;
+    return d4::gemm_x3sk_fill_capacity(gemm_args_of(*main));
+}
+int d4_gemm_run_fill(const d4_gemm_desc* main, const d4_gemm_desc* fill, int fill_tiles, void* stream) {
+    if (int rc = gemm_desc_check("d4_gemm_run_fill", main)) return rc;
+    D4_REQUIRE(fill_tiles == 0 || fill, "d4_gemm_run_fill: fill tiles without a fill descriptor");
+    if (fill_tiles != 0) if (int rc = gemm_desc_check("d4_gemm_run_fill", fill)) return rc;
+    const d4::GemmArgs g = gemm_args_of(*main);
+    D4_REQUIRE(((uintptr_t)g.A % 16) == 0 && (g.lda % 4) == 0 && !g.wscale, "d4_gemm_run_fill: main operands must be 16-byte aligned split-operand planes");
+    return d4::gemm_x3sk_fill(g, fill ? gemm_args_of(*fill) : d4::GemmArgs{}, fill_tiles, static_cast<hipStream_t>(stream));
+}
+int d4_gemm_run_fill_rowmap(const d4_gemm_desc* main, const d4_gemm_desc* fill, int fill_tiles, int rm_Sc, int rm_S, int rm_lo, int rm_nr, void* stream) {
+    if (int rc = gemm_desc_check("d4_gemm_run_fill_rowmap", main)) return rc;
+    if (int rc = gemm_desc_check("d4_gemm_run_fill_rowmap", fill)) return rc;
+    D4_REQUIRE(rm_Sc >= 1 && rm_nr >= 0 && rm_lo >= 0 && rm_lo <= rm_Sc && rm_S == rm_Sc + rm_nr && rm_S <= 65535, "d4_gemm_run_fill_rowmap: bad row map (Sc=%d S=%d lo=%d nr=%d)", rm_Sc, rm_S, rm_lo, rm_nr);
+    d4::GemmArgs f = gemm_args_of(*fill);
+    f.rm_Sc = (uint16_t)rm_Sc; f.rm_lo = (uint16_t)rm_lo; f.rm_nr = (uint16_t)rm_nr;
+    return d4::gemm_x3sk_fill(gemm_args_of(*main), f, fill_tiles, static_cast<hipStream_t>(stream));
+}
 int d4_gemm_run_pair(const d4_gemm_desc* da, const d4_gemm_desc* db, int target, int config, void* stream) {
     if (int rc = gemm_desc_check("d4_gemm_run_pair", da)) return rc;
     if (int rc = gemm_desc_check("d4_gemm_run_pair", db)) return rc;
diff --git a/dreamer4_amd/csrc/gemm.hip b/dreamer4_amd/csrc/gemm.hip
--- a/dreamer4_amd/csrc/gemm.hip
+++ b/dreamer4_amd/csrc/gemm.hip
@@ -686,6 +686,22 @@
     rec.bm = 128; rec.bn = 128;
     rec.flops = p.algo_flops > 0 ? p.algo_flops : 2.0 * p.M * p.N * p.K;
     if (int rc = gemm_x3sk_launch(p, stream, rec.a, rec.b)) return rc;
+    g_prof.push_back(rec);
+    return 0;
+}
+
+int gemm_x3sk_fill(const GemmArgs& p, const GemmArgs& fill, int fill_tiles, hipStream_t stream) {
+    std::lock_guard<std::recursive_mutex> lock(gemm_mutex());
+    const int cls = N_TILE_CFG + gemm2_configs() + gemm_x3_configs();
+    const bool timed = ((g_prof_mask >> cls) & 1) && (g_prof_tick++ % g_prof_stride) == 0;
+    if (!timed) return gemm_x3sk_fill_launch(p, fill, fill_tiles, stream);
+    ProfRec rec{};
+    rec.a = prof_event(); rec.b = prof_event(); rec.cls = cls;
+    rec.M = p.M; rec.N = p.N; rec.K = p.K; rec.flags = p.flags; rec.batch = p.batch;
+    rec.bm = 128; rec.bn = 128;
+    rec.flops = p.algo_flops > 0 ? p.algo_flops : 2.0 * p.M * p.N * p.K;
+    if (fill_tiles > 0) rec.flops += 2.0 * fill.M * fill.N * fill.K * fill_tiles / (double)gemm_x3sk_fill_tiles(fill);
+    if (int rc = gemm_x3sk_fill_launch(p, fill, fill_tiles, stream, rec.a, rec.b)) return rc;
     g_prof.push_back(rec);
     return 0;
 }
diff --git a/dreamer4_amd/csrc/gemm2.hip b/dreamer4_amd/csrc/gemm2.hip
--- a/dreamer4_amd/csrc/gemm2.hip
+++ b/dreamer4_amd/csrc/gemm2.hip
@@ -1,280 +1,11 @@
 #include "common.h"
 #include <hip/hip_ext.h>
 #include "kernels.h"
+#include "gemm2_body.h"
 #include <stdlib.h>
 #include <type_traits>
 
 namespace d4 {
-
-typedef __attribute__((address_space(3))) void* lds_void_ptr;
-
-template <int N>
-__device__ __forceinline__ void wait_vmcnt() {
-    asm volatile("s_waitcnt vmcnt(%0)" ::"n"(N) : "memory");
-}
-
-template <int BK>
-__device__ __forceinline__ int chunk_swizzle(int row) {
-    if constexpr (BK == 32) return row & 7;
-    else return (0x78 >> (((row >> 2) & 3) * 2)) & 3;
-}
-
-template <int WGM, int WGN, int TM, int TN, int NS, int BK, bool RMS, bool RMAP = false>
-__device__ __forceinline__ void gemm2_body(GemmArgs& p, int bid, const int bz) {
-    static_assert(BK == 16 || BK == 32, "k-tile");
-    constexpr int CH = BK / 4;
-    constexpr int RPP = 64 / CH;
-    constexpr int H = BK / 16;
-    constexpr int NW = WGM * WGN, NT = NW * 64;
-    constexpr int BM = WGM * TM * 16, BN = WGN * TN * 16;
-    constexpr int STAGE_ROWS = BM + BN;
-    constexpr int STAGE_F = STAGE_ROWS * BK;
-    constexpr int NSLOT = STAGE_ROWS / RPP;
-    constexpr int LPW = (NSLOT + NW - 1) / NW;
-    static_assert(NS >= 3 && NS <= 4 && 2 * LPW <= 63, "ring depth / vmcnt range");
-    extern __shared__ __attribute__((aligned(16))) float smem[];
-
-    const int tid = threadIdx.x, lane = tid & 63;
-    const int wave = __builtin_amdgcn_readfirstlane(tid >> 6);
-    const int wm = wave / WGN, wn = wave % WGN;
-
-    const int nbn = (p.N + BN - 1) / BN, nbm = (p.M + BM - 1) / BM;
-    {
-        const int nblk = nbm * nbn, nx = 8;
-        const int q = nblk / nx, r = nblk % nx, x = bid % nx, o = bid / nx;
-        bid = (x < r ? x * (q + 1) : r * (q + 1) + (x - r) * q) + o;
-    }
-    const int bm0 = (bid / nbn) * BM, bn0 = (bid % nbn) * BN;
-    p.A += bz * p.strideA; p.W += bz * p.strideW; p.C += bz * p.strideC;
-    if (p.R) p.R += bz * p.strideC;
-
-    const int rowsA = min(BM, p.M - bm0), rowsB = min(BN, p.N - bn0);
-    auto uniform_rsrc = [](const float* base, int64_t bytes) {
-        const uint64_t b = reinterpret_cast<uint64_t>(base);
-        const uint32_t lo = __builtin_amdgcn_readfirstlane((uint32_t)b);
-        const uint32_t hi = __builtin_amdgcn_readfirstlane((uint32_t)(b >> 32));
-        const int nb = __builtin_amdgcn_readfirstlane((int)(bytes < 0x7FFFFFFF ? bytes : 0x7FFFFFFF));
-        return __builtin_amdgcn_make_buffer_rsrc(reinterpret_cast<void*>(((uint64_t)hi << 32) | lo), 0, nb, 0x00020000);
-    };
-    const __amdgpu_buffer_rsrc_t rsA = uniform_rsrc(p.A + (int64_t)bm0 * p.lda, ((int64_t)(rowsA - 1) * p.lda + p.K) * 4);
-    const __amdgpu_buffer_rsrc_t rsB = uniform_rsrc(p.W + (int64_t)bn0 * p.ldw, ((int64_t)(rowsB - 1) * p.ldw + p.K) * 4);
-
-    uint32_t voff[LPW];
-    const int prow = lane / CH;
-    const int src_chunk = (lane % CH) ^ chunk_swizzle<BK>(prow);
-#pragma unroll
-    for (int i = 0; i < LPW; ++i) {
-        const int slot = min(wave + NW * i, NSLOT - 1);
-        const int r = slot * RPP + prow;
-        voff[i] = (uint32_t)((slot * RPP < BM ? r * p.lda : (r - BM) * p.ldw) * 4 + src_chunk * 16);
-    }
-#define D4_ISSUE_STAGE(KT, BUF)                                                                                              \
-    _Pragma("unroll") for (int i_ = 0; i_ < LPW; ++i_) {                                                                      \
-        const int slot_ = min(wave + NW * i_, NSLOT - 1);                                                                     \
-        float* dst_ = smem + (BUF) * STAGE_F + slot_ * 256;                                                                   \
-        if (slot_ * RPP < BM) __builtin_amdgcn_raw_ptr_buffer_load_lds(rsA, (lds_void_ptr)dst_, 16, (uint32_t)voff[i_], (KT) * BK * 4, 0, 0); \
-        else __builtin_amdgcn_raw_ptr_buffer_load_lds(rsB, (lds_void_ptr)dst_, 16, (uint32_t)voff[i_], (KT) * BK * 4, 0, 0);              \
-    }
-
-    f32x4 acc[TM][TN];
-#pragma unroll
-    for (int i = 0; i < TM; ++i)
-#pragma unroll
-        for (int j = 0; j < TN; ++j) acc[i][j] = f32x4{0.f, 0.f, 0.f, 0.f};
-
-    const int kq = lane >> 4, frow = lane & 15;
-    const int foff0 = frow * BK + ((kq ^ chunk_swizzle<BK>(frow)) << 2);
-    const int a_base = wm * TM * 16 * BK, b_base = BM * BK + wn * TN * 16 * BK;
-
-    constexpr int NPAR = 32 / BK;
-    constexpr int SQI = RMS ? (BM * CH + NT - 1) / NT : 1;
-    float ssq[SQI][NPAR];
-#pragma unroll
-    for (int i = 0; i < SQI; ++i)
-#pragma unroll
-        for (int h = 0; h < NPAR; ++h) ssq[i][h] = 0.f;
-
-    const int nk = p.K / BK;
-    auto wait_allow = [&](int stages) {
-        if (stages >= 2) wait_vmcnt<2 * LPW>();
-        else if (stages == 1) wait_vmcnt<LPW>();
-        else wait_vmcnt<0>();
-    };
-    f32x4 af[2][TM], bf[2][TN];
-    auto read_frags = [&](const float* st, auto set_tag, int second_half) {
-        constexpr int SET = decltype(set_tag)::value;
-        const int fo = second_half ? (foff0 ^ 16) : foff0;
-#pragma unroll
-        for (int i = 0; i < TM; ++i) af[SET][i] = *reinterpret_cast<const f32x4*>(st + a_base + i * 16 * BK + fo);
-#pragma unroll
-        for (int j = 0; j < TN; ++j) bf[SET][j] = *reinterpret_cast<const f32x4*>(st + b_base + j * 16 * BK + fo);
-    };
-    auto mfma_set = [&](auto set_tag) {
-        constexpr int SET = decltype(set_tag)::value;
-#pragma unroll
-        for (int e = 0; e < 4; ++e)
-#pragma unroll
-            for (int i = 0; i < TM; ++i)
-#pragma unroll
-                for (int j = 0; j < TN; ++j)
-                    acc[i][j] = __builtin_amdgcn_mfma_f32_16x16x4f32(bf[SET][j][e], af[SET][i][e], acc[i][j], 0, 0, 0);
-    };
-    using S0 = std::integral_constant<int, 0>;
-    using S1 = std::integral_constant<int, 1>;
-
-#pragma unroll
-    for (int s = 0; s < NS - 1; ++s)
-        if (s < nk) { D4_ISSUE_STAGE(s, s) }
-    wait_allow(min(NS - 2, nk - 1));
-    __builtin_amdgcn_s_barrier();
-    read_frags(smem, S0{}, 0);
-
-    auto k_tile = [&](int kt, auto par_tag) {
-        constexpr int PAR = decltype(par_tag)::value;
-        if (kt + 1 < nk) {
-            wait_allow(min(kt + NS - 2, nk - 1) - (kt + 1));
-            __builtin_amdgcn_s_barrier();
-            if (kt + NS - 1 < nk) { D4_ISSUE_STAGE(kt + NS - 1, (kt + NS - 1) % NS) }
-        }
-        const float* st = smem + (kt % NS) * STAGE_F;
-        const float* nxt = smem + ((kt + 1) % NS) * STAGE_F;
-        if constexpr (RMS) {
-#pragma unroll
-            for (int i = 0; i < SQI; ++i) {
-                const int idx = tid + i * NT;
-                if (BM * CH % NT == 0 || idx < BM * CH) {
-                    const f32x4 v = *reinterpret_cast<const f32x4*>(st + idx * 4);
-                    ssq[i][PAR % NPAR] = ssq[i][PAR % NPAR] + __builtin_fmaf(v[3], v[3], __builtin_fmaf(v[2], v[2], __builtin_fmaf(v[1], v[1], v[0] * v[0])));
-                }
-            }
-        }
-        if constexpr (H == 2) {
-            read_frags(st, S1{}, 1);
-            mfma_set(S0{});
-            if (kt + 1 < nk) read_frags(nxt, S0{}, 0);
-            mfma_set(S1{});
-        } else {
-            using CUR = std::integral_constant<int, PAR>;
-            using NXT = std::integral_constant<int, PAR ^ 1>;
-            if (kt + 1 < nk) read_frags(nxt, NXT{}, 0);
-            mfma_set(CUR{});
-        }
-    };
-    for (int kt = 0; kt < nk; kt += 2) {
-        k_tile(kt, S0{});
-        if (kt + 1 < nk) k_tile(kt + 1, S1{});
-    }
-
-#undef D4_ISSUE_STAGE
-    float* rowscale_s = smem + NS * STAGE_F;
-    if constexpr (RMS) {
-#pragma unroll
-        for (int i = 0; i < SQI; ++i) {
-            float s = ssq[i][0];
-            s += dpp_f<0xB1>(s);
-            s += dpp_f<0x4E>(s);
-            if constexpr (NPAR == 1) {
-                s += dpp_f<0x141>(s);
-            } else {
-                float s1 = ssq[i][1];
-                s1 += dpp_f<0xB1>(s1);
-                s1 += dpp_f<0x4E>(s1);
-                s = s + s1;
-            }
-            const int idx = tid + i * NT;
-            if ((idx % CH) == 0 && idx < BM * CH) rowscale_s[idx / CH] = rsqrtf(s / (float)p.K + p.rms_eps);
-        }
-        __syncthreads();
-    }
-
-    const bool swiglu = (p.flags & GEMM_SWIGLU) != 0;
-    const bool vecC = (p.ldc % 4) == 0 && ((uintptr_t)p.C % 16) == 0;
-    const bool vecR = p.R && (p.ldr % 4) == 0 && ((uintptr_t)p.R % 16) == 0;
-    const bool vecC2 = p.C2 && (p.ldc2 % 4) == 0 && ((uintptr_t)p.C2 % 16) == 0;
-#pragma unroll
-    for (int i = 0; i < TM; ++i) {
-        const int ml = wm * TM * 16 + i * 16 + frow;
-        const int gm = bm0 + ml;
-        if (gm >= p.M) continue;
-        const float rs = RMS ? rowscale_s[ml] : 1.f;
-        int64_t c2row = -1;
-        if (p.C2) {
-            const int ts = gm % p.c2_S, keep = p.c2_hi - p.c2_lo;
-            const int rank = (ts >= p.c2_lo && ts < p.c2_hi) ? ts - p.c2_lo : ((p.c2_last && ts == p.c2_S - 1) ? keep : -1);
-            if (rank >= 0) c2row = (int64_t)(gm / p.c2_S) * (keep + p.c2_last) + rank;
-        }
-        if (swiglu) {
-            if constexpr (TN % 4 == 0) {
-#pragma unroll
-                for (int j = 0; j < TN; ++j) {
-                    if ((j & 3) >= 2) continue;
-                    const int gn = bn0 + wn * TN * 16 + j * 16 + kq * 4;
-                    if (gn >= p.N) continue;
-                    f32x4 o;
-#pragma unroll
-                    for (int e = 0; e < 4; ++e) {
-                        float val = acc[i][j][e] * rs, gate = acc[i][j + 2][e] * rs;
-                        if (p.bias) { val += p.bias[gn + e]; gate += p.bias[gn + e + 32]; }
-                        o[e] = val * siluf(gate);
-                    }
-                    const int on = (gn / 64) * 32 + (gn % 64);
-                    float* cp = p.C + (int64_t)gm * p.ldc + on;
-                    if (vecC) *reinterpret_cast<f32x4*>(cp) = o;
-                    else { cp[0] = o[0]; cp[1] = o[1]; cp[2] = o[2]; cp[3] = o[3]; }
-                }
-            }
-            continue;
-        }
-#pragma unroll
-        for (int j = 0; j < TN; ++j) {
-            const int gn = bn0 + wn * TN * 16 + j * 16 + kq * 4;
-            if (gn >= p.N) continue;
-            const bool full = gn + 3 < p.N;
-            f32x4 v;
-#pragma unroll
-            for (int e = 0; e < 4; ++e) v[e] = acc[i][j][e] * rs;
-            if (p.bias) {
-#pragma unroll
-                for (int e = 0; e < 4; ++e) if (full || gn + e < p.N) v[e] += p.bias[gn + e];
-            }
-            if (p.flags & GEMM_SILU) {
-#pragma unroll
-                for (int e = 0; e < 4; ++e) v[e] = siluf(v[e]);
-            }
-            if (p.R) {
-                const float* rp = p.R + (int64_t)gm * p.ldr + gn;
-                if (vecR && full) { const f32x4 r4 = *reinterpret_cast<const f32x4*>(rp); v[0] += r4[0]; v[1] += r4[1]; v[2] += r4[2]; v[3] += r4[3]; }
-                else {
-#pragma unroll
-                    for (int e = 0; e < 4; ++e) if (full || gn + e < p.N) v[e] += rp[e];
-                }
-            }
-            int64_t crow = gm;
-            if constexpr (RMAP) {
-                const int fr = gm / p.rm_Sc, t = gm - fr * p.rm_Sc;
-                crow = (int64_t)fr * (p.rm_Sc + p.rm_nr) + t + (t >= p.rm_lo ? p.rm_nr : 0);
-            }
-            float* cp = p.C + crow * p.ldc + gn;
-            if (p.flags & GEMM_ACCUMULATE) {
-#pragma unroll
-                for (int e = 0; e < 4; ++e) if (full || gn + e < p.N) v[e] += cp[e];
-            }
-            if (vecC && full) *reinterpret_cast<f32x4*>(cp) = v;
-            else {
-#pragma unroll
-                for (int e = 0; e < 4; ++e) if (full || gn + e < p.N) cp[e] = v[e];
-            }
-            if (c2row >= 0) {
-                float* c2 = p.C2 + c2row * p.ldc2 + gn;
-                if (vecC2 && full) *reinterpret_cast<f32x4*>(c2) = v;
-                else {
-#pragma unroll
-                    for (int e = 0; e < 4; ++e) if (full || gn + e < p.N) c2[e] = v[e];
-                }
-            }
-        }
-    }
-}
 
 template <int WGM, int WGN, int TM, int TN, int NS, int BK, bool RMS>
 __global__ __launch_bounds__(WGM* WGN * 64) void gemm2_kernel(GemmArgs p) {
diff --git a/dreamer4_amd/csrc/gemm2_body.h b/dreamer4_amd/csrc/gemm2_body.h
--- /dev/null
+++ b/dreamer4_amd/csrc/gemm2_body.h
@@ -0,0 +1,278 @@
+#pragma once
+#include "common.h"
+#include "kernels.h"
+#include <type_traits>
+
+namespace d4 {
+
+typedef __attribute__((address_space(3))) void* lds_void_ptr;
+
+template <int N>
+__device__ __forceinline__ void wait_vmcnt() {
+    asm volatile("s_waitcnt vmcnt(%0)" ::"n"(N) : "memory");
+}
+
+template <int BK>
+__device__ __forceinline__ int chunk_swizzle(int row) {
+    if constexpr (BK == 32) return row & 7;
+    else return (0x78 >> (((row >> 2) & 3) * 2)) & 3;
+}
+
+template <int WGM, int WGN, int TM, int TN, int NS, int BK, bool RMS, bool RMAP = false>
+__device__ __forceinline__ void gemm2_body(GemmArgs& p, int bid, const int bz) {
+    static_assert(BK == 16 || BK == 32, "k-tile");
+    constexpr int CH = BK / 4;
+    constexpr int RPP = 64 / CH;
+    constexpr int H = BK / 16;
+    constexpr int NW = WGM * WGN, NT = NW * 64;
+    constexpr int BM = WGM * TM * 16, BN = WGN * TN * 16;
+    constexpr int STAGE_ROWS = BM + BN;
+    constexpr int STAGE_F = STAGE_ROWS * BK;
+    constexpr int NSLOT = STAGE_ROWS / RPP;
+    constexpr int LPW = (NSLOT + NW - 1) / NW;
+    static_assert(NS >= 3 && NS <= 4 && 2 * LPW <= 63, "ring depth / vmcnt range");
+    extern __shared__ __attribute__((aligned(16))) float smem[];
+
+    const int tid = threadIdx.x, lane = tid & 63;
+    const int wave = __builtin_amdgcn_readfirstlane(tid >> 6);
+    const int wm = wave / WGN, wn = wave % WGN;
+
+    const int nbn = (p.N + BN - 1) / BN, nbm = (p.M + BM - 1) / BM;
+    {
+        const int nblk = nbm * nbn, nx = 8;
+        const int q = nblk / nx, r = nblk % nx, x = bid % nx, o = bid / nx;
+        bid = (x < r ? x * (q + 1) : r * (q + 1) + (x - r) * q) + o;
+    }
+    const int bm0 = (bid / nbn) * BM, bn0 = (bid % nbn) * BN;
+    p.A += bz * p.strideA; p.W += bz * p.strideW; p.C += bz * p.strideC;
+    if (p.R) p.R += bz * p.strideC;
+
+    const int rowsA = min(BM, p.M - bm0), rowsB = min(BN, p.N - bn0);
+    auto uniform_rsrc = [](const float* base, int64_t bytes) {
+        const uint64_t b = reinterpret_cast<uint64_t>(base);
+        const uint32_t lo = __builtin_amdgcn_readfirstlane((uint32_t)b);
+        const uint32_t hi = __builtin_amdgcn_readfirstlane((uint32_t)(b >> 32));
+        const int nb = __builtin_amdgcn_readfirstlane((int)(bytes < 0x7FFFFFFF ? bytes : 0x7FFFFFFF));
+        return __builtin_amdgcn_make_buffer_rsrc(reinterpret_cast<void*>(((uint64_t)hi << 32) | lo), 0, nb, 0x00020000);
+    };
+    const __amdgpu_buffer_rsrc_t rsA = uniform_rsrc(p.A + (int64_t)bm0 * p.lda, ((int64_t)(rowsA - 1) * p.lda + p.K) * 4);
+    const __amdgpu_buffer_rsrc_t rsB = uniform_rsrc(p.W + (int64_t)bn0 * p.ldw, ((int64_t)(rowsB - 1) * p.ldw + p.K) * 4);
+
+    uint32_t voff[LPW];
+    const int prow = lane / CH;
+    const int src_chunk = (lane % CH) ^ chunk_swizzle<BK>(prow);
+#pragma unroll
+    for (int i = 0; i < LPW; ++i) {
+        const int slot = min(wave + NW * i, NSLOT - 1);
+        const int r = slot * RPP + prow;
+        voff[i] = (uint32_t)((slot * RPP < BM ? r * p.lda : (r - BM) * p.ldw) * 4 + src_chunk * 16);
+    }
+#define D4_ISSUE_STAGE(KT, BUF)                                                                                              \
+    _Pragma("unroll") for (int i_ = 0; i_ < LPW; ++i_) {                                                                      \
+        const int slot_ = min(wave + NW * i_, NSLOT - 1);                                                                     \
+        float* dst_ = smem + (BUF) * STAGE_F + slot_ * 256;                                                                   \
+        if (slot_ * RPP < BM) __builtin_amdgcn_raw_ptr_buffer_load_lds(rsA, (lds_void_ptr)dst_, 16, (uint32_t)voff[i_], (KT) * BK * 4, 0, 0); \
+        else __builtin_amdgcn_raw_ptr_buffer_load_lds(rsB, (lds_void_ptr)dst_, 16, (uint32_t)voff[i_], (KT) * BK * 4, 0, 0);              \
+    }
+
+    f32x4 acc[TM][TN];
+#pragma unroll
+    for (int i = 0; i < TM; ++i)
+#pragma unroll
+        for (int j = 0; j < TN; ++j) acc[i][j] = f32x4{0.f, 0.f, 0.f, 0.f};
+
+    const int kq = lane >> 4, frow = lane & 15;
+    const int foff0 = frow * BK + ((kq ^ chunk_swizzle<BK>(frow)) << 2);
+    const int a_base = wm * TM * 16 * BK, b_base = BM * BK + wn * TN * 16 * BK;
+
+    constexpr int NPAR = 32 / BK;
+    constexpr int SQI = RMS ? (BM * CH + NT - 1) / NT : 1;
+    float ssq[SQI][NPAR];
+#pragma unroll
+    for (int i = 0; i < SQI; ++i)
+#pragma unroll
+        for (int h = 0; h < NPAR; ++h) ssq[i][h] = 0.f;
+
+    const int nk = p.K / BK;
+    auto wait_allow = [&](int stages) {
+        if (stages >= 2) wait_vmcnt<2 * LPW>();
+        else if (stages == 1) wait_vmcnt<LPW>();
+        else wait_vmcnt<0>();
+    };
+    f32x4 af[2][TM], bf[2][TN];
+    auto read_frags = [&](const float* st, auto set_tag, int second_half) {
+        constexpr int SET = decltype(set_tag)::value;
+        const int fo = second_half ? (foff0 ^ 16) : foff0;
+#pragma unroll
+        for (int i = 0; i < TM; ++i) af[SET][i] = *reinterpret_cast<const f32x4*>(st + a_base + i * 16 * BK + fo);
+#pragma unroll
+        for (int j = 0; j < TN; ++j) bf[SET][j] = *reinterpret_cast<const f32x4*>(st + b_base + j * 16 * BK + fo);
+    };
+    auto mfma_set = [&](auto set_tag) {
+        constexpr int SET = decltype(set_tag)::value;
+#pragma unroll
+        for (int e = 0; e < 4; ++e)
+#pragma unroll
+            for (int i = 0; i < TM; ++i)
+#pragma unroll
+                for (int j = 0; j < TN; ++j)
+                    acc[i][j] = __builtin_amdgcn_mfma_f32_16x16x4f32(bf[SET][j][e], af[SET][i][e], acc[i][j], 0, 0, 0);
+    };
+    using S0 = std::integral_constant<int, 0>;
+    using S1 = std::integral_constant<int, 1>;
+
+#pragma unroll
+    for (int s = 0; s < NS - 1; ++s)
+        if (s < nk) { D4_ISSUE_STAGE(s, s) }
+    wait_allow(min(NS - 2, nk - 1));
+    __builtin_amdgcn_s_barrier();
+    read_frags(smem, S0{}, 0);
+
+    auto k_tile = [&](int kt, auto par_tag) {
+        constexpr int PAR = decltype(par_tag)::value;
+        if (kt + 1 < nk) {
+            wait_allow(min(kt + NS - 2, nk - 1) - (kt + 1));
+            __builtin_amdgcn_s_barrier();
+            if (kt + NS - 1 < nk) { D4_ISSUE_STAGE(kt + NS - 1, (kt + NS - 1) % NS) }
+        }
+        const float* st = smem + (kt % NS) * STAGE_F;
+        const float* nxt = smem + ((kt + 1) % NS) * STAGE_F;
+        if constexpr (RMS) {
+#pragma unroll
+            for (int i = 0; i < SQI; ++i) {
+                const int idx = tid + i * NT;
+                if (BM * CH % NT == 0 || idx < BM * CH) {
+                    const f32x4 v = *reinterpret_cast<const f32x4*>(st + idx * 4);
+                    ssq[i][PAR % NPAR] = ssq[i][PAR % NPAR] + __builtin_fmaf(v[3], v[3], __builtin_fmaf(v[2], v[2], __builtin_fmaf(v[1], v[1], v[0] * v[0])));
+                }
+            }
+        }
+        if constexpr (H == 2) {
+            read_frags(st, S1{}, 1);
+            mfma_set(S0{});
+            if (kt + 1 < nk) read_frags(nxt, S0{}, 0);
+            mfma_set(S1{});
+        } else {
+            using CUR = std::integral_constant<int, PAR>;
+            using NXT = std::integral_constant<int, PAR ^ 1>;
+            if (kt + 1 < nk) read_frags(nxt, NXT{}, 0);
+            mfma_set(CUR{});
+        }
+    };
+    for (int kt = 0; kt < nk; kt += 2) {
+        k_tile(kt, S0{});
+        if (kt + 1 < nk) k_tile(kt + 1, S1{});
+    }
+
+#undef D4_ISSUE_STAGE
+    float* rowscale_s = smem + NS * STAGE_F;
+    if constexpr (RMS) {
+#pragma unroll
+        for (int i = 0; i < SQI; ++i) {
+            float s = ssq[i][0];
+            s += dpp_f<0xB1>(s);
+            s += dpp_f<0x4E>(s);
+            if constexpr (NPAR == 1) {
+                s += dpp_f<0x141>(s);
+            } else {
+                float s1 = ssq[i][1];
+                s1 += dpp_f<0xB1>(s1);
+                s1 += dpp_f<0x4E>(s1);
+                s = s + s1;
+            }
+            const int idx = tid + i * NT;
+            if ((idx % CH) == 0 && idx < BM * CH) rowscale_s[idx / CH] = rsqrtf(s / (float)p.K + p.rms_eps);
+        }
+        __syncthreads();
+    }
+
+    const bool swiglu = (p.flags & GEMM_SWIGLU) != 0;
+    const bool vecC = (p.ldc % 4) == 0 && ((uintptr_t)p.C % 16) == 0;
+    const bool vecR = p.R && (p.ldr % 4) == 0 && ((uintptr_t)p.R % 16) == 0;
+    const bool vecC2 = p.C2 && (p.ldc2 % 4) == 0 && ((uintptr_t)p.C2 % 16) == 0;
+#pragma unroll
+    for (int i = 0; i < TM; ++i) {
+        const int ml = wm * TM * 16 + i * 16 + frow;
+        const int gm = bm0 + ml;
+        if (gm >= p.M) continue;
+        const float rs = RMS ? rowscale_s[ml] : 1.f;
+        int64_t c2row = -1;
+        if (p.C2) {
+            const int ts = gm % p.c2_S, keep = p.c2_hi - p.c2_lo;
+            const int rank = (ts >= p.c2_lo && ts < p.c2_hi) ? ts - p.c2_lo : ((p.c2_last && ts == p.c2_S - 1) ? keep : -1);
+            if (rank >= 0) c2row = (int64_t)(gm / p.c2_S) * (keep + p.c2_last) + rank;
+        }
+        if (swiglu) {
+            if constexpr (TN % 4 == 0) {
+#pragma unroll
+                for (int j = 0; j < TN; ++j) {
+                    if ((j & 3) >= 2) continue;
+                    const int gn = bn0 + wn * TN * 16 + j * 16 + kq * 4;
+                    if (gn >= p.N) continue;
+                    f32x4 o;
+#pragma unroll
+                    for (int e = 0; e < 4; ++e) {
+                        float val = acc[i][j][e] * rs, gate = acc[i][j + 2][e] * rs;
+                        if (p.bias) { val += p.bias[gn + e]; gate += p.bias[gn + e + 32]; }
+                        o[e] = val * siluf(gate);
+                    }
+                    const int on = (gn / 64) * 32 + (gn % 64);
+                    float* cp = p.C + (int64_t)gm * p.ldc + on;
+                    if (vecC) *reinterpret_cast<f32x4*>(cp) = o;
+                    else { cp[0] = o[0]; cp[1] = o[1]; cp[2] = o[2]; cp[3] = o[3]; }
+                }
+            }
+            continue;
+        }
+#pragma unroll
+        for (int j = 0; j < TN; ++j) {
+            const int gn = bn0 + wn * TN * 16 + j * 16 + kq * 4;
+            if (gn >= p.N) continue;
+            const bool full = gn + 3 < p.N;
+            f32x4 v;
+#pragma unroll
+            for (int e = 0; e < 4; ++e) v[e] = acc[i][j][e] * rs;
+            if (p.bias) {
+#pragma unroll
+                for (int e = 0; e < 4; ++e) if (full || gn + e < p.N) v[e] += p.bias[gn + e];
+            }
+            if (p.flags & GEMM_SILU) {
+#pragma unroll
+                for (int e = 0; e < 4; ++e) v[e] = siluf(v[e]);
+            }
+            if (p.R) {
+                const float* rp = p.R + (int64_t)gm * p.ldr + gn;
+                if (vecR && full) { const f32x4 r4 = *reinterpret_cast<const f32x4*>(rp); v[0] += r4[0]; v[1] += r4[1]; v[2] += r4[2]; v[3] += r4[3]; }
+                else {
+#pragma unroll
+                    for (int e = 0; e < 4; ++e) if (full || gn + e < p.N) v[e] += rp[e];
+                }
+            }
+            int64_t crow = gm;
+            if constexpr (RMAP) {
+                const int fr = gm / p.rm_Sc, t = gm - fr * p.rm_Sc;
+                crow = (int64_t)fr * (p.rm_Sc + p.rm_nr) + t + (t >= p.rm_lo ? p.rm_nr : 0);
+            }
+            float* cp = p.C + crow * p.ldc + gn;
+            if (p.flags & GEMM_ACCUMULATE) {
+#pragma unroll
+                for (int e = 0; e < 4; ++e) if (full || gn + e < p.N) v[e] += cp[e];
+            }
+            if (vecC && full) *reinterpret_cast<f32x4*>(cp) = v;
+            else {
+#pragma unroll
+                for (int e = 0; e < 4; ++e) if (full || gn + e < p.N) cp[e] = v[e];
+            }
+            if (c2row >= 0) {
+                float* c2 = p.C2 + c2row * p.ldc2 + gn;
+                if (vecC2 && full) *reinterpret_cast<f32x4*>(c2) = v;
+                else {
+#pragma unroll
+                    for (int e = 0; e < 4; ++e) if (full || gn + e < p.N) c2[e] = v[e];
+                }
+            }
+        }
+    }
+}
+
+}
diff --git a/dreamer4_amd/csrc/gemm_x3sk.hip b/dreamer4_amd/csrc/gemm_x3sk.hip
--- a/dreamer4_amd/csrc/gemm_x3sk.hip
+++ b/dreamer4_amd/csrc/gemm_x3sk.hip
@@ -1,6 +1,7 @@
 #include "common.h"
 #include <hip/hip_ext.h>
 #include "kernels.h"
+#include "gemm2_body.h"
 #include <type_traits>
 
 namespace d4 {
@@ -254,7 +255,7 @@
     __syncthreads();
 }
 
-template <bool RMAP>
+template <bool RMAP, bool WHOLE = false>
 __device__ __forceinline__ void sk_walk(const SkArgs s) {
     const GemmArgs& p = s.p;
     extern __shared__ __attribute__((aligned(16))) char smem_raw[];
@@ -276,7 +277,7 @@
         tm = band * RB + j % rows; tn = j / rows;
     };
     int tm, tn;
-    if (s.half) {
+    if (!WHOLE && s.half) {
         for (int i = 0; i < s.F; ++i) {
             tile_of(b + i * s.P, tm, tn);
             sk_item<2, RMAP>(s, tm * SK_BM, tn * SK_BN, As, Bs, rowscale_s);
@@ -306,6 +307,18 @@
 
 __global__ __launch_bounds__(SK_NT, 2) void gemm_x3sk_kernel(SkArgs s) { sk_walk<false>(s); }
 __global__ __launch_bounds__(SK_NT, 2) void gemm_x3sk_rowmap_kernel(SkArgs s) { sk_walk<true>(s); }
+
+constexpr int SKF_BM = 128, SKF_BN = 64;
+constexpr size_t SKF_LDS = (size_t)(3 * (SKF_BM + SKF_BN) * 32 + SKF_BM) * sizeof(float);
+static_assert(SKF_LDS <= SK_LDS, "a fill tile runs in the LDS of the workgroup it fills");
+template <bool FILL_RMS>
+__global__ __launch_bounds__(SK_NT, 2) void gemm_x3sk_fill_kernel(SkArgs s, GemmArgs fill, int fill_tiles) {
+    const int b = blockIdx.x;
+    sk_walk<false, true>(s);
+    if (b < s.R || b - s.R >= fill_tiles) return;
+    __syncthreads();
+    gemm2_body<4, 2, 2, 2, 3, 32, FILL_RMS>(fill, b - s.R, 0);
+}
 
 static std::atomic<int> g_sk_cus[64];
 
@@ -365,4 +378,53 @@
     return 0;
 }
 
-}
+int gemm_x3sk_fill_capacity(const GemmArgs& main) {
+    if (!gemm_x3sk_applicable(main)) return 0;
+    int F, R, P;
+    (void)gemm_x3sk_half_plan(main, &F, &R, &P);
+    return F >= 1 && R > 0 ? P - R : 0;
+}
+
+unsigned g_fill_launches = 0;
+
+int gemm_x3sk_fill_tiles(const GemmArgs& fill) { return cdiv(fill.M, SKF_BM) * cdiv(fill.N, SKF_BN); }
+
+bool gemm_x3sk_fill_applicable(const GemmArgs& fill) {
+    return gemm2_applicable(fill) && fill.batch <= 1 && fill.rm_Sc == 0 && fill.C && !fill.C2 && !fill.R && !fill.Cb && !fill.C2b && !(fill.flags & ~GEMM_RMS_ROWSCALE) &&
+           ((uintptr_t)fill.A % 16) == 0 && ((uintptr_t)fill.W % 16) == 0;
+}
+
+int gemm_x3sk_fill_launch(const GemmArgs& main, const GemmArgs& fill, int fill_tiles, hipStream_t stream, hipEvent_t ea, hipEvent_t eb) {
+    D4_REQUIRE(gemm_x3sk_applicable(main) && main.rm_Sc == 0, "gemm_x3sk fill: main call not supported (M=%d N=%d K=%d flags=%d batch=%d row map %d)", main.M, main.N,
+               main.K, main.flags, main.batch, (int)main.rm_Sc);
+    SkArgs a;
+    a.p = main;
+    (void)gemm_x3sk_half_plan(main, &a.F, &a.R, &a.P);
+    a.half = 0;
+    D4_REQUIRE(a.F >= 1, "gemm_x3sk fill: the main call (M=%d N=%d: %d tiles on %d workgroups) has no whole round, it is not persistent", main.M, main.N, a.R, a.P);
+    const int cap = a.R > 0 ? a.P - a.R : 0;
+    D4_REQUIRE(fill_tiles >= 0 && fill_tiles <= cap, "gemm_x3sk fill: %d fill tiles exceed the capacity of %d idle workgroups", fill_tiles, cap);
+    GemmArgs f{};
+    bool rms = false;
+    if (fill_tiles > 0) {
+        D4_REQUIRE(gemm_x3sk_fill_applicable(fill), "gemm_x3sk fill: fill problem not supported (M=%d N=%d K=%d flags=%d batch=%d row map %d: an f32-input product of "
+                   "K %% 32 == 0, no batch, row map, second output or epilogue other than row scale / bias)", fill.M, fill.N, fill.K, fill.flags, fill.batch, (int)fill.rm_Sc);
+        D4_REQUIRE(fill_tiles <= gemm_x3sk_fill_tiles(fill), "gemm_x3sk fill: %d fill tiles, the fill problem (M=%d N=%d) has %d", fill_tiles, fill.M, fill.N, gemm_x3sk_fill_tiles(fill));
+        f = fill;
+        rms = (fill.flags & GEMM_RMS_ROWSCALE) != 0;
+    }
+    auto k = rms ? gemm_x3sk_fill_kernel<true> : gemm_x3sk_fill_kernel<false>;
+    static DeviceOnce attr_set[2];
+    if (attr_set[rms].need()) {
+        D4_HIP(hipFuncSetAttribute(reinterpret_cast<const void*>(k), hipFuncAttributeMaxDynamicSharedMemorySize, (int)SK_LDS));
+        attr_set[rms].done();
+    }
+    const dim3 grid(a.P), block(SK_NT);
+    if (ea) hipExtLaunchKernelGGL(k, grid, block, (uint32_t)SK_LDS, stream, ea, eb, 0, a, f, fill_tiles);
+    else hipLaunchKernelGGL(k, grid, block, SK_LDS, stream, a, f, fill_tiles);
+    D4_LAUNCH_CHECK();
+    if (fill_tiles > 0) ++g_fill_launches;
+    return 0;
+}
+
+}
diff --git a/dreamer4_amd/csrc/kernels.h b/dreamer4_amd/csrc/kernels.h
--- a/dreamer4_amd/csrc/kernels.h
+++ b/dreamer4_amd/csrc/kernels.h
@@ -87,6 +87,12 @@
 bool gemm_x3sk_rule(const GemmArgs& p);
 const char* gemm_x3sk_name();
 int gemm_x3sk_launch(const GemmArgs& p, hipStream_t stream, hipEvent_t ea = nullptr, hipEvent_t eb = nullptr);
+int gemm_x3sk_fill_capacity(const GemmArgs& main);
+int gemm_x3sk_fill_tiles(const GemmArgs& fill);
+bool gemm_x3sk_fill_applicable(const GemmArgs& fill);
+int gemm_x3sk_fill_launch(const GemmArgs& main, const GemmArgs& fill, int fill_tiles, hipStream_t stream, hipEvent_t ea = nullptr, hipEvent_t eb = nullptr);
+extern unsigned g_fill_launches;
+int gemm_x3sk_fill(const GemmArgs& main, const GemmArgs& fill, int fill_tiles, hipStream_t stream);
 bool gemm2_applicable(const GemmArgs& p);
 bool gemm2_config_valid(int c, const GemmArgs& p);
 int gemm2_configs();
diff --git a/include/d4hip.h b/include/d4hip.h
--- a/include/d4hip.h
+++ b/include/d4hip.h
@@ -340,6 +340,9 @@
 int d4_gemm_family_configs(int family);
 int d4_gemm_run(const d4_gemm_desc* d, int family, int config, void* stream);
 int d4_gemm_run_rowmap(const d4_gemm_desc* d, int family, int config, int rm_Sc, int rm_S, int rm_lo, int rm_nr, void* stream);
+int d4_gemm_fill_capacity(const d4_gemm_desc* main_call);
+int d4_gemm_run_fill(const d4_gemm_desc* main_call, const d4_gemm_desc* fill, int fill_tiles, void* stream);
+int d4_gemm_run_fill_rowmap(const d4_gemm_desc* main_call, const d4_gemm_desc* fill, int fill_tiles, int rm_Sc, int rm_S, int rm_lo, int rm_nr, void* stream);
 #define D4_PAIR_SKINNY 0
 #define D4_PAIR_BF16A 1
 #define D4_PAIR_V2 2
```

Result: faster. 23470 imagined steps/s (median of 6 runs) (+1.4%).
